# kondratevakate/mri-epilepsy-diagnosis

Measured on AMD Instinct MI355X. Metric: MRI volumes/sec (fwd+bwd) 3D U-Net @160x192x160, higher is better.
Workload: dtype f32; 1 GPU; unet.UNet(c0=8, 3 enc blocks, BN+PReLU, trilinear) fwd+softmax-Dice+bwd+AdamW, batch 2 x 1x160x192x160 fp32 per GPU (BASELINE configs[1]); global_batch=2, parallelism=dp1, launch=eager

## Files before the change

### include/mri3d.h

```cpp
#ifndef MRI3D_H
#define MRI3D_H

#include <stddef.h>
#include <stdint.h>

#ifdef __cplusplus
extern "C" {
#endif

typedef void* mri3d_stream_t;

enum { MRI3D_OK = 0, MRI3D_EINVAL = -1, MRI3D_ENOTSUP = -2, MRI3D_ELAUNCH = -3, MRI3D_EWORKSPACE = -4 };
enum { MRI3D_F32 = 0, MRI3D_BF16 = 1 };
enum { MRI3D_ACT_NONE = 0, MRI3D_ACT_RELU = 1, MRI3D_ACT_LEAKY = 2, MRI3D_ACT_PRELU = 3 };
enum { MRI3D_UP_NEAREST = 0, MRI3D_UP_TRILINEAR = 1 };
enum { MRI3D_PASS_FWD = 0, MRI3D_PASS_DGRAD = 1, MRI3D_PASS_WGRAD = 2 };

int mri3d_version(void);
const char* mri3d_last_error(void);

typedef struct Mri3dConvGeom {
    int32_t n;
    int32_t di, hi, wi, ci;
    int32_t dout, ho, wo, co;
    int32_t kd, kh, kw;
    int32_t sd, sh, sw;
    int32_t pd, ph, pw;
    int32_t dd, dh, dw;
    int32_t x_ld, y_ld;
    int32_t dtype;
} Mri3dConvGeom;

size_t mri3d_conv3d_workspace_bytes(const Mri3dConvGeom* g, int pass);

int mri3d_conv3d_fwd(const Mri3dConvGeom* g, const void* x, const void* w, const void* bias, void* y,
                     void* workspace, size_t ws_bytes, mri3d_stream_t stream);
int32_t mri3d_conv3d_fwd_stats_blocks(const Mri3dConvGeom* g);
int mri3d_conv3d_fwd_stats(const Mri3dConvGeom* g, const void* x, const void* w, const void* bias, void* y,
                           double* stat_partials, void* workspace, size_t ws_bytes, mri3d_stream_t stream);
int mri3d_conv3d_dgrad(const Mri3dConvGeom* g, const void* dy, const void* w, const void* bias, void* dx,
                       void* workspace, size_t ws_bytes, mri3d_stream_t stream);
int mri3d_conv3d_wgrad(const Mri3dConvGeom* g, const void* x, const void* dy, void* dw, void* dbias,
                       void* workspace, size_t ws_bytes, mri3d_stream_t stream);

int mri3d_conv3d_route(const Mri3dConvGeom* g, int32_t pass, int32_t stats, int32_t bias, int32_t split, int32_t second_ld,
                       int32_t align_x, int32_t align_y, char* name, size_t name_bytes);

int32_t mri3d_conv3d_cat_supported(const Mri3dConvGeom* g, int32_t split, int32_t second_ld, int32_t pass);
int32_t mri3d_conv3d_fwd_cat_stats_blocks(const Mri3dConvGeom* g, int32_t split, int32_t second_ld);
int mri3d_conv3d_fwd_cat(const Mri3dConvGeom* g, const void* x, const void* x2, int32_t split, int32_t x2_ld, const void* w,
                         const void* bias, void* y, double* stat_partials, void* workspace, size_t ws_bytes,
                         mri3d_stream_t stream);
int mri3d_conv3d_dgrad_cat(const Mri3dConvGeom* g, const void* dy, const void* w, void* dx, void* dx2, int32_t split,
                           int32_t dx2_ld, void* workspace, size_t ws_bytes, mri3d_stream_t stream);
int mri3d_conv3d_wgrad_cat(const Mri3dConvGeom* g, const void* x, const void* x2, int32_t split, int32_t x2_ld, const void* dy,
                           void* dw, void* dbias, void* workspace, size_t ws_bytes, mri3d_stream_t stream);

int32_t mri3d_conv3d_march_supported(const Mri3dConvGeom* g, int32_t pass);
int32_t mri3d_conv3d_march_stats_blocks(const Mri3dConvGeom* g);
int mri3d_conv3d_fwd_march(const Mri3dConvGeom* g, const void* x, const void* x2, int32_t split, int32_t x2_ld, const void* w,
                           const void* bias, void* y, double* stat_partials, void* workspace, size_t ws_bytes,
                           mri3d_stream_t stream);
int mri3d_conv3d_dgrad_march(const Mri3dConvGeom* g, const void* dy, const void* w, void* dx, void* dx2, int32_t split,
                             int32_t dx2_ld, void* workspace, size_t ws_bytes, mri3d_stream_t stream);

typedef struct Mri3dMarchPlanInfo {
    int32_t chunks, blocks, wgh, wgw, gch, gcw, nseg, seglen, nbuf, grid, whole_chunks, dispatcher;
    int64_t smem_bytes, wp_bytes;
} Mri3dMarchPlanInfo;
int32_t mri3d_conv3d_march_plan_query(const Mri3dConvGeom* g, int32_t pass, int32_t stats, Mri3dMarchPlanInfo* out);

int32_t mri3d_upconv3d_supported(const Mri3dConvGeom* g, int32_t scale);
size_t mri3d_upconv3d_workspace_bytes(const Mri3dConvGeom* g, int32_t scale);
int mri3d_upconv3d_fwd(const Mri3dConvGeom* g, int32_t scale, const void* x, const float* w, const float* bias, void* y,
                       mri3d_stream_t stream);
int mri3d_upconv3d_dgrad(const Mri3dConvGeom* g, int32_t scale, const void* dy, const float* w, void* dx, mri3d_stream_t stream);
int mri3d_upconv3d_wgrad(const Mri3dConvGeom* g, int32_t scale, const void* x, const void* dy, float* dw, float* dbias,
                         void* workspace, size_t ws_bytes, mri3d_stream_t stream);

int32_t mri3d_convpair_supported(const Mri3dConvGeom* first, const Mri3dConvGeom* second);
size_t mri3d_convpair_workspace_bytes(const Mri3dConvGeom* first, const Mri3dConvGeom* second);
int mri3d_convpair_wgrad_first(const Mri3dConvGeom* first, const Mri3dConvGeom* second, const void* x, const void* dy2, const float* w2,
                               float* dw1, float* dbias1, void* workspace, size_t ws_bytes, mri3d_stream_t stream);

typedef struct Mri3dFusedConvPlanInfo {
    int32_t hch, grid, gtrips, trips, per, passes, chunks;
    int64_t slabs, rows;
} Mri3dFusedConvPlanInfo;
int32_t mri3d_upconv3d_plan_query(const Mri3dConvGeom* g, int32_t scale, int32_t pass, Mri3dFusedConvPlanInfo* out);
int32_t mri3d_convpair_plan_query(const Mri3dConvGeom* first, const Mri3dConvGeom* second, Mri3dFusedConvPlanInfo* out);

typedef struct Mri3dNormGeom {
    int32_t n;
    int64_t vox;
    int32_t c;
    int32_t x_ld;
    int32_t y_ld;
    int32_t instance;
    int32_t act;
// ... 31 lines not shown
size_t mri3d_norm_act_pw_workspace_bytes(const Mri3dNormGeom* g, int32_t co);
int mri3d_norm_act_pw_fwd(const Mri3dNormGeom* g, int32_t co, const void* x, const float* mean, const float* invstd,
                          const float* gamma, const float* beta, const float* alpha, const float* w, const float* bias,
                          void* out, mri3d_stream_t stream);
int mri3d_norm_act_pw_bwd(const Mri3dNormGeom* g, int32_t co, int training, const void* x, const void* dout,
                          const float* mean, const float* invstd, const float* gamma, const float* beta, const float* alpha,
                          const float* w, void* dx, float* dgamma, float* dbeta, float* dalpha, float* dw, float* dbias,
                          void* workspace, size_t ws_bytes, mri3d_stream_t stream);

typedef struct Mri3dPoolGeom {
    int32_t n, di, hi, wi, dout, ho, wo, c;
    int32_t kd, kh, kw, sd, sh, sw, pd, ph, pw;
    int32_t x_ld, y_ld;
    int32_t dtype;
} Mri3dPoolGeom;
int mri3d_maxpool3d_fwd(const Mri3dPoolGeom* g, const void* x, void* y, uint8_t* idx, mri3d_stream_t stream);
int mri3d_maxpool3d_bwd(const Mri3dPoolGeom* g, const void* dy, const uint8_t* idx, void* dx, mri3d_stream_t stream);
int mri3d_maxpool3d_bwd_add(const Mri3dPoolGeom* g, const void* dy, const uint8_t* idx, const void* addend,
                            int32_t addend_ld, void* dx, mri3d_stream_t stream);
int mri3d_maxpool3d_route(const Mri3dPoolGeom* g, int32_t pass, int32_t addend_ld, int32_t align_tensors, int32_t align_idx,
                          char* name, size_t name_bytes);

int32_t mri3d_norm_act_pool_supported(const Mri3dNormGeom* g, const Mri3dPoolGeom* pg);
size_t mri3d_norm_act_pool_workspace_bytes(const Mri3dNormGeom* g, const Mri3dPoolGeom* pg);
int mri3d_norm_act_pool_fwd(const Mri3dNormGeom* g, const Mri3dPoolGeom* pg, const void* x, const float* mean,
                            const float* invstd, const float* gamma, const float* beta, const float* alpha, void* skip,
                            void* pooled, uint8_t* idx, mri3d_stream_t stream);
int mri3d_norm_act_pool_bwd(const Mri3dNormGeom* g, const Mri3dPoolGeom* pg, int training, const void* x, const void* dskip,
                            const void* dpool, const uint8_t* idx, const float* mean, const float* invstd, const float* gamma,
                            const float* beta, const float* alpha, void* dx, float* dgamma, float* dbeta, float* dalpha,
                            void* workspace, size_t ws_bytes, mri3d_stream_t stream);

typedef struct Mri3dUpGeom {
    int32_t n, di, hi, wi, dout, ho, wo, c;
    int32_t x_ld, y_ld;
    int32_t mode;
    int32_t align_corners;
    float rd, rh, rw;
    int32_t dtype;
} Mri3dUpGeom;
size_t mri3d_upsample3d_workspace_bytes(const Mri3dUpGeom* g);
int mri3d_upsample3d_fwd(const Mri3dUpGeom* g, const void* x, void* y, mri3d_stream_t stream);
int mri3d_upsample3d_bwd(const Mri3dUpGeom* g, const void* dy, void* dx, void* workspace, size_t ws_bytes,
                         mri3d_stream_t stream);
int mri3d_upsample3d_route(const Mri3dUpGeom* g, int32_t pass, int32_t align, char* name, size_t name_bytes);

typedef struct Mri3dResamplePlanInfo {
    int32_t vec, npv, hch, grid, segs, segl, tiles_h, tiles_w, passes, items, tables;
    int64_t lds_bytes;
} Mri3dResamplePlanInfo;
int32_t mri3d_maxpool3d_plan_query(const Mri3dPoolGeom* g, int32_t pass, int32_t addend_ld, int32_t align_tensors,
                                   int32_t align_idx, Mri3dResamplePlanInfo* out);
int32_t mri3d_upsample3d_plan_query(const Mri3dUpGeom* g, int32_t pass, int32_t align, Mri3dResamplePlanInfo* out);

typedef struct Mri3dDiceGeom {
    int32_t n;
    int64_t vox;
    int32_t c, ct;
    int32_t x_ld, t_ld;
    float eps;
    int32_t dtype;
} Mri3dDiceGeom;
size_t mri3d_softmax_dice_workspace_bytes(const Mri3dDiceGeom* g);
int mri3d_softmax_dice_fwd(const Mri3dDiceGeom* g, const void* logits, const void* target, float* loss,
                           float* stats, void* workspace, size_t ws_bytes, mri3d_stream_t stream);
int mri3d_softmax_dice_bwd(const Mri3dDiceGeom* g, const void* logits, const void* target, const float* stats,
                           const float* dloss, void* dlogits, mri3d_stream_t stream);

int mri3d_argmax_u8(const void* logits, uint8_t* out, int64_t nvox, int32_t c, int32_t ld, int32_t dtype,
                    mri3d_stream_t stream);

size_t mri3d_mask_overlap_workspace_bytes(void);
int mri3d_mask_overlap(const uint8_t* pred, const uint8_t* gt, int64_t nvox, int64_t* counts, void* workspace,
                       size_t ws_bytes, mri3d_stream_t stream);

enum { MRI3D_LABEL_U8 = 0, MRI3D_LABEL_I16 = 1, MRI3D_LABEL_I32 = 2, MRI3D_LABEL_F32 = 3 };

int mri3d_label_remap(const void* in, int32_t in_dtype, void* out, int32_t out_dtype, int64_t n, const uint8_t* lut,
                      int32_t lut_len, int32_t above, int32_t other, mri3d_stream_t stream);

typedef struct Mri3dDiceIndexGeom {
    int32_t n;
    int64_t vox;
    int32_t c;
    int32_t x_ld;
    float eps;
    int32_t dtype;
} Mri3dDiceIndexGeom;
size_t mri3d_softmax_dice_index_workspace_bytes(const Mri3dDiceIndexGeom* g);
int mri3d_softmax_dice_index_fwd(const Mri3dDiceIndexGeom* g, const void* logits, const uint8_t* labels, float* loss,
                                 float* stats, void* workspace, size_t ws_bytes, mri3d_stream_t stream);
int mri3d_softmax_dice_index_bwd(const Mri3dDiceIndexGeom* g, const void* logits, const uint8_t* labels,
                                 const float* stats, const float* dloss, void* dlogits, mri3d_stream_t stream);

size_t mri3d_confusion_workspace_bytes(int32_t c);
int mri3d_confusion_counts(const uint8_t* pred, const uint8_t* gt, int64_t nvox, int32_t c, int64_t* counts,
                           void* workspace, size_t ws_bytes, mri3d_stream_t stream);

size_t mri3d_order_stats_workspace_bytes(void);
int mri3d_order_stats_f32(const float* x, int64_t n, const int64_t* ranks, int32_t nranks, float* out, void* workspace,
                          size_t ws_bytes, mri3d_stream_t stream);
int mri3d_piecewise_linear_f32(const float* x, float* y, int64_t n, const double* edges, const double* slope,
                               const double* intercept, int32_t nseg, mri3d_stream_t stream);
size_t mri3d_znorm_workspace_bytes(void);
int mri3d_znorm_mean_mask_f32(const float* x, float* y, int64_t n, double* stats, void* workspace, size_t ws_bytes,
                              mri3d_stream_t stream);
// ... 85 lines not shown
```

### mri_epilepsy_diagnosis_amd/_lib.py

```python
import ctypes
import os
from ctypes import POINTER, Structure, c_char_p, c_double, c_float, c_int32, c_int64, c_size_t, c_uint8, c_void_p

_HERE = os.path.dirname(os.path.abspath(__file__))
LIB_PATH = os.path.join(_HERE, "libmri3d_hip.so")

F32, BF16 = 0, 1
ACT_NONE, ACT_RELU, ACT_LEAKY, ACT_PRELU = 0, 1, 2, 3
UP_NEAREST, UP_TRILINEAR = 0, 1
PASS_FWD, PASS_DGRAD, PASS_WGRAD = 0, 1, 2
NORM_PASS_STATS, NORM_PASS_FWD, NORM_PASS_BWD = 0, 1, 2
LABEL_U8, LABEL_I16, LABEL_I32, LABEL_F32 = 0, 1, 2, 3
BW_SCOTT, BW_SILVERMAN, BW_FACTOR = 0, 1, 2


class ConvGeom(Structure):
    _fields_ = [(n, c_int32) for n in (
        "n", "di", "hi", "wi", "ci", "dout", "ho", "wo", "co", "kd", "kh", "kw", "sd", "sh", "sw",
        "pd", "ph", "pw", "dd", "dh", "dw", "x_ld", "y_ld", "dtype")]


class NormGeom(Structure):
    _fields_ = [("n", c_int32), ("vox", c_int64), ("c", c_int32), ("x_ld", c_int32), ("y_ld", c_int32),
                ("instance", c_int32), ("act", c_int32), ("alpha_n", c_int32), ("slope", c_float),
                ("eps", c_float), ("group_c", c_int32), ("dtype", c_int32)]


class NormPlanInfo(Structure):
    _fields_ = [(n, c_int32) for n in ("vec", "CL", "VT", "cy", "nblk", "groups")] + [("gvox", c_int64)]


class ResamplePlanInfo(Structure):
    _fields_ = [(n, c_int32) for n in ("vec", "npv", "hch", "grid", "segs", "segl", "tiles_h", "tiles_w", "passes", "items",
                                       "tables")] + [("lds_bytes", c_int64)]


class FusedConvPlanInfo(Structure):
    _fields_ = [(n, c_int32) for n in ("hch", "grid", "gtrips", "trips", "per", "passes", "chunks")] + \
               [("slabs", c_int64), ("rows", c_int64)]


class MarchPlanInfo(Structure):
    _fields_ = [(n, c_int32) for n in ("chunks", "blocks", "wgh", "wgw", "gch", "gcw", "nseg", "seglen", "nbuf", "grid",
                                       "whole_chunks", "dispatcher")] + [("smem_bytes", c_int64), ("wp_bytes", c_int64)]


class PoolGeom(Structure):
    _fields_ = [(n, c_int32) for n in (
        "n", "di", "hi", "wi", "dout", "ho", "wo", "c", "kd", "kh", "kw", "sd", "sh", "sw", "pd", "ph", "pw",
        "x_ld", "y_ld", "dtype")]


class UpGeom(Structure):
    _fields_ = [(n, c_int32) for n in ("n", "di", "hi", "wi", "dout", "ho", "wo", "c", "x_ld", "y_ld", "mode",
                                       "align_corners")] + \
               [("rd", c_float), ("rh", c_float), ("rw", c_float), ("dtype", c_int32)]


class DiceGeom(Structure):
    _fields_ = [("n", c_int32), ("vox", c_int64), ("c", c_int32), ("ct", c_int32), ("x_ld", c_int32),
                ("t_ld", c_int32), ("eps", c_float), ("dtype", c_int32)]


class DiceIndexGeom(Structure):
    _fields_ = [("n", c_int32), ("vox", c_int64), ("c", c_int32), ("x_ld", c_int32), ("eps", c_float), ("dtype", c_int32)]


_P = c_void_p
_FP = c_void_p

SIGNATURES = {
    "mri3d_version": (c_int32, []),
    "mri3d_last_error": (c_char_p, []),
    "mri3d_conv3d_workspace_bytes": (c_size_t, [POINTER(ConvGeom), c_int32]),
    "mri3d_conv3d_fwd": (c_int32, [POINTER(ConvGeom), _P, _P, _P, _P, _P, c_size_t, _P]),
    "mri3d_conv3d_fwd_stats_blocks": (c_int32, [POINTER(ConvGeom)]),
    "mri3d_conv3d_fwd_stats": (c_int32, [POINTER(ConvGeom), _P, _P, _P, _P, _P, _P, c_size_t, _P]),
    "mri3d_conv3d_dgrad": (c_int32, [POINTER(ConvGeom), _P, _P, _P, _P, _P, c_size_t, _P]),
    "mri3d_conv3d_wgrad": (c_int32, [POINTER(ConvGeom), _P, _P, _P, _P, _P, c_size_t, _P]),
    "mri3d_conv3d_route": (c_int32, [POINTER(ConvGeom), c_int32, c_int32, c_int32, c_int32, c_int32, c_int32, c_int32, c_char_p, c_size_t]),
    "mri3d_conv3d_cat_supported": (c_int32, [POINTER(ConvGeom), c_int32, c_int32, c_int32]),
    "mri3d_conv3d_fwd_cat_stats_blocks": (c_int32, [POINTER(ConvGeom), c_int32, c_int32]),
    "mri3d_conv3d_fwd_cat": (c_int32, [POINTER(ConvGeom), _P, _P, c_int32, c_int32, _P, _P, _P, _P, _P, c_size_t, _P]),
    "mri3d_conv3d_dgrad_cat": (c_int32, [POINTER(ConvGeom), _P, _P, _P, _P, c_int32, c_int32, _P, c_size_t, _P]),
    "mri3d_conv3d_wgrad_cat": (c_int32, [POINTER(ConvGeom), _P, _P, c_int32, c_int32, _P, _P, _P, _P, c_size_t, _P]),
    "mri3d_conv3d_march_supported": (c_int32, [POINTER(ConvGeom), c_int32]),
    "mri3d_conv3d_march_stats_blocks": (c_int32, [POINTER(ConvGeom)]),
    "mri3d_conv3d_march_plan_query": (c_int32, [POINTER(ConvGeom), c_int32, c_int32, POINTER(MarchPlanInfo)]),
    "mri3d_conv3d_fwd_march": (c_int32, [POINTER(ConvGeom), _P, _P, c_int32, c_int32, _P, _P, _P, _P, _P, c_size_t, _P]),
    "mri3d_conv3d_dgrad_march": (c_int32, [POINTER(ConvGeom), _P, _P, _P, _P, c_int32, c_int32, _P, c_size_t, _P]),
    "mri3d_upconv3d_supported": (c_int32, [POINTER(ConvGeom), c_int32]),
    "mri3d_upconv3d_workspace_bytes": (c_size_t, [POINTER(ConvGeom), c_int32]),
    "mri3d_upconv3d_fwd": (c_int32, [POINTER(ConvGeom), c_int32, _P, _FP, _FP, _P, _P]),
    "mri3d_upconv3d_dgrad": (c_int32, [POINTER(ConvGeom), c_int32, _P, _FP, _P, _P]),
    "mri3d_upconv3d_wgrad": (c_int32, [POINTER(ConvGeom), c_int32, _P, _P, _FP, _FP, _P, c_size_t, _P]),
    "mri3d_convpair_supported": (c_int32, [POINTER(ConvGeom), POINTER(ConvGeom)]),
    "mri3d_convpair_workspace_bytes": (c_size_t, [POINTER(ConvGeom), POINTER(ConvGeom)]),
    "mri3d_convpair_wgrad_first": (c_int32, [POINTER(ConvGeom), POINTER(ConvGeom), _P, _P, _FP, _FP, _FP, _P, c_size_t, _P]),
    "mri3d_upconv3d_plan_query": (c_int32, [POINTER(ConvGeom), c_int32, c_int32, POINTER(FusedConvPlanInfo)]),
    "mri3d_convpair_plan_query": (c_int32, [POINTER(ConvGeom), POINTER(ConvGeom), POINTER(FusedConvPlanInfo)]),
    "mri3d_norm_workspace_bytes": (c_size_t, [POINTER(NormGeom)]),
    "mri3d_norm_plan_query": (c_int32, [POINTER(NormGeom), c_int32, c_int32, POINTER(NormPlanInfo)]),
    "mri3d_norm_stats": (c_int32, [POINTER(NormGeom), _P, _FP, _FP, _FP, _FP, c_float, _P, c_size_t, _P]),
    "mri3d_norm_stats_from_partials": (c_int32, [POINTER(NormGeom), _P, c_int32, _FP, _FP, _FP, _FP, _FP, c_float, _P]),
    "mri3d_norm_act_fwd": (c_int32, [POINTER(NormGeom), _P, _FP, _FP, _FP, _FP, _FP, _P, _P]),
    "mri3d_norm_act_bwd": (c_int32, [POINTER(NormGeom), c_int32, _P, _P, _FP, _FP, _FP, _FP, _FP, _P, _FP, _FP, _FP,
                                     _P, c_size_t, _P]),
    "mri3d_norm_act_pw_supported": (c_int32, [POINTER(NormGeom), c_int32]),
    "mri3d_norm_act_pw_workspace_bytes": (c_size_t, [POINTER(NormGeom), c_int32]),
    "mri3d_norm_act_pw_fwd": (c_int32, [POINTER(NormGeom), c_int32, _P, _FP, _FP, _FP, _FP, _FP, _FP, _FP, _P, _P]),
    "mri3d_norm_act_pw_bwd": (c_int32, [POINTER(NormGeom), c_int32, c_int32, _P, _P, _FP, _FP, _FP, _FP, _FP, _FP, _P, _FP, _FP,
                                        _FP, _FP, _FP, _P, c_size_t, _P]),
    "mri3d_maxpool3d_fwd": (c_int32, [POINTER(PoolGeom), _P, _P, _P, _P]),
    "mri3d_maxpool3d_bwd": (c_int32, [POINTER(PoolGeom), _P, _P, _P, _P]),
    "mri3d_maxpool3d_bwd_add": (c_int32, [POINTER(PoolGeom), _P, _P, _P, c_int32, _P, _P]),
    "mri3d_maxpool3d_route": (c_int32, [POINTER(PoolGeom), c_int32, c_int32, c_int32, c_int32, c_char_p, c_size_t]),
    "mri3d_maxpool3d_plan_query": (c_int32, [POINTER(PoolGeom), c_int32, c_int32, c_int32, c_int32, POINTER(ResamplePlanInfo)]),
    "mri3d_norm_act_pool_supported": (c_int32, [POINTER(NormGeom), POINTER(PoolGeom)]),
    "mri3d_norm_act_pool_workspace_bytes": (c_size_t, [POINTER(NormGeom), POINTER(PoolGeom)]),
    "mri3d_norm_act_pool_fwd": (c_int32, [POINTER(NormGeom), POINTER(PoolGeom), _P, _FP, _FP, _FP, _FP, _FP, _P, _P, _P, _P]),
    "mri3d_norm_act_pool_bwd": (c_int32, [POINTER(NormGeom), POINTER(PoolGeom), c_int32, _P, _P, _P, _P, _FP, _FP, _FP, _FP,
                                          _FP, _P, _FP, _FP, _FP, _P, c_size_t, _P]),
    "mri3d_upsample3d_workspace_bytes":(c_size_t, [POINTER(UpGeom)]),
    "mri3d_upsample3d_fwd": (c_int32, [POINTER(UpGeom), _P, _P, _P]),
    "mri3d_upsample3d_bwd": (c_int32, [POINTER(UpGeom), _P, _P, _P, c_size_t, _P]),
    "mri3d_upsample3d_route": (c_int32, [POINTER(UpGeom), c_int32, c_int32, c_char_p, c_size_t]),
    "mri3d_upsample3d_plan_query": (c_int32, [POINTER(UpGeom), c_int32, c_int32, POINTER(ResamplePlanInfo)]),
    "mri3d_softmax_dice_workspace_bytes": (c_size_t, [POINTER(DiceGeom)]),
    "mri3d_softmax_dice_fwd": (c_int32, [POINTER(DiceGeom), _P, _P, _FP, _FP, _P, c_size_t, _P]),
    "mri3d_softmax_dice_bwd": (c_int32, [POINTER(DiceGeom), _P, _P, _FP, _FP, _P, _P]),
    "mri3d_argmax_u8": (c_int32, [_P, _P, c_int64, c_int32, c_int32, c_int32, _P]),
    "mri3d_mask_overlap_workspace_bytes": (c_size_t, []),
    "mri3d_mask_overlap": (c_int32, [_P, _P, c_int64, _P, _P, c_size_t, _P]),
    "mri3d_label_remap": (c_int32, [_P, c_int32, _P, c_int32, c_int64, _P, c_int32, c_int32, c_int32, _P]),
    "mri3d_softmax_dice_index_workspace_bytes": (c_size_t, [POINTER(DiceIndexGeom)]),
    "mri3d_softmax_dice_index_fwd": (c_int32, [POINTER(DiceIndexGeom), _P, _P, _FP, _FP, _P, c_size_t, _P]),
    "mri3d_softmax_dice_index_bwd": (c_int32, [POINTER(DiceIndexGeom), _P, _P, _FP, _FP, _P, _P]),
    "mri3d_confusion_workspace_bytes": (c_size_t, [c_int32]),
    "mri3d_confusion_counts": (c_int32, [_P, _P, c_int64, c_int32, _P, _P, c_size_t, _P]),
    "mri3d_order_stats_workspace_bytes": (c_size_t, []),
    "mri3d_order_stats_f32": (c_int32, [_P, c_int64, _P, c_int32, _P, _P, c_size_t, _P]),
    "mri3d_piecewise_linear_f32": (c_int32, [_P, _P, c_int64, _P, _P, _P, c_int32, _P]),
    "mri3d_znorm_workspace_bytes": (c_size_t, []),
    "mri3d_znorm_mean_mask_f32": (c_int32, [_P, _P, c_int64, _P, _P, c_size_t, _P]),
    "mri3d_crop_or_pad_f32": (c_int32, [_P, _P, c_int32, c_int32, c_int32, c_int32, c_int32, c_int32, c_int32, c_float, _P]),
    "mri3d_intensity_workspace_bytes": (c_size_t, [c_int64, c_int32, c_int32]),
    "mri3d_kde_plan": (c_int32, [c_int64, c_int32, c_int32, _P]),
    "mri3d_intensity_moments_f32": (c_int32, [_P, _P, c_int64, c_int32, _P, _P, c_size_t, _P]),
    "mri3d_kde_f32": (c_int32, [_P, _P, c_int64, c_int32, _P, _P, c_int32, c_int32, c_double, _P, _P, _P, c_size_t, _P]),
    "mri3d_surface_distance_workspace_bytes": (c_size_t, [c_int32, c_int32, c_int32]),
    "mri3d_surface_distance": (c_int32, [_P, _P, c_int32, c_int32, c_int32, _P, _P, _P, c_size_t, _P]),
    "mri3d_surface_elements": (c_int32, [_P, _P, c_int32, c_int32, c_int32, _P, _P, _P, _P, c_int64, _P, _P, c_size_t, _P]),
    "mri3d_extract_patches": (c_int32, [_P, c_int32, c_int32, c_int32, c_int32, c_int32, _P, c_int32, c_int32, c_int32,
                                        c_int32, _P, _P]),
    "mri3d_aggregate_patches_u8": (c_int32, [_P, _P, c_int32, c_int32, c_int32, c_int32, c_int32, c_int32, c_int32, _P,
                                             c_int32, c_int32, c_int32, c_int32, _P]),
    "mri3d_aggregate_patches_argmax": (c_int32, [_P, c_int32, c_int32, c_int32, _P, c_int32, c_int32, c_int32, c_int32,
                                                 c_int32, c_int32, c_int32, _P, c_int32, c_int32, c_int32, c_int32, _P]),
    "mri3d_strip_starts_f32": (c_int32, [_FP, c_int32, c_int32, c_int32, c_int32, _P, _P]),
    "mri3d_mirror_patches_f32": (c_int32, [_FP, c_int32, c_int32, c_int32, _P, _P, c_int64, c_int32, c_int32, c_int32, _FP, _P]),
    "mri3d_mirror_patch_labels_u8": (c_int32, [_P, c_int32, c_int32, c_int32, _P, c_int64, c_int32, c_int32, _P, _P]),
    "mri3d_patch_vote_u8": (c_int32, [_P, c_int32, c_int32, _P, _P]),
    "mri3d_paint_patches_u8": (c_int32, [_P, _P, c_int32, c_int32, c_int32, c_int32, c_int32, _P, _P]),
    "mri3d_warp3d": (c_int32, [_FP, _FP, _P, _P, c_int32, c_int32, c_int32, c_int32, c_int32, _FP, _FP, c_int32, c_int32,
                               c_int32, c_float, _FP, _P]),
    "mri3d_bias_field_f32": (c_int32, [_FP, _FP, c_int32, c_int32, c_int32, c_int32, _P, c_int32, _P]),
    "mri3d_kspace_mix_f32": (c_int32, [_FP, _FP, c_int32, c_int32, c_int32, c_int32, c_int32, _FP, _P]),
    "mri3d_copy_channels": (c_int32, [_P, _P, c_int64, c_int32, c_int32, c_int32, c_int32, _P]),
    "mri3d_add_channels": (c_int32, [_P, _P, _P, c_int64, c_int32, c_int32, c_int32, c_int32, c_int32, _P]),
    "mri3d_convert_channels": (c_int32, [_P, c_int32, _P, c_int32, c_int64, c_int32, c_int32, c_int32, _P]),
    "mri3d_bayes_weights_fwd": (c_int32, [_FP, _FP, c_int64, c_int32, c_float, _FP, _FP, _FP, _P]),
    "mri3d_bayes_weights_bwd": (c_int32, [_FP, _FP, c_int64, c_int32, c_float, _FP, _FP, _FP, _FP, _FP, _P]),
    "mri3d_bayes_square": (c_int32, [_P, _P, c_int64, c_int32, c_int32, c_int32, c_int32, _P]),
    "mri3d_bayes_sample_fwd": (c_int32, [_P, _P, _FP, _P, c_int64, c_int32, c_int32, c_int32, c_int32, c_int32, c_int32, _P]),
    "mri3d_bayes_sample_bwd": (c_int32, [_P, _P, _FP, _P, c_int64, c_int32, c_int32, c_int32, c_int32, c_int32, c_int32, _P]),
    "mri3d_bayes_dx": (c_int32, [_P, _P, _P, _P, c_int64, c_int32, c_int32, c_int32, c_int32, c_int32, c_int32, _P]),
    "mri3d_mc_state_bytes": (c_size_t, [c_int64, c_int32]),
    "mri3d_mc_accumulate": (c_int32, [_P, c_int64, c_int32, c_int32, c_int32, c_int32, c_int64, c_int32, _P, c_size_t, _P]),
    "mri3d_mc_finalize": (c_int32, [_P, c_size_t, c_int64, c_int32, c_int32, _FP, _FP, _FP, _FP, _P, _P]),
    "mri3d_adam_step": (c_int32, [_FP, _FP, _FP, _FP, c_int64, c_float, c_float, c_float, c_float, c_float, c_int32,
# ... 32 lines not shown
```

### mri_epilepsy_diagnosis_amd/build.py

```python
import hashlib
import os
import subprocess
import sys
from concurrent.futures import ThreadPoolExecutor

HERE = os.path.dirname(os.path.abspath(__file__))
CSRC = os.path.join(HERE, "csrc")
OBJ = os.path.join(HERE, "csrc", "build")
LIB = os.path.join(HERE, "libmri3d_hip.so")
SOURCES = ["api.hip", "conv_generic.hip", "conv_mfma.hip", "conv_mfma_wgrad.hip", "conv_march.hip", "conv_pointwise.hip", "upconv.hip", "sepconv.hip", "norm.hip", "resample.hip", "loss.hip", "labels.hip", "elementwise.hip", "bayes.hip", "mc_stats.hip", "preprocess.hip", "intensity.hip", "surface.hip", "patches.hip", "detection.hip", "augment.hip", "kspace.hip"]
HIPCC = os.environ.get("HIPCC", "/opt/rocm/bin/hipcc")
FLAGS = ["--offload-arch=gfx950", "-O3", "-fPIC", "-std=c++17", "-Wall", "-Wno-unused-function"]
EXTRA_FLAGS = {"conv_march.hip": ["-mllvm", "-amdgpu-spill-vgpr-to-agpr=0"], "mc_stats.hip": ["-ffp-contract=off"],
               "intensity.hip": ["-ffp-contract=off"]}


def _digest(path):
    h = hashlib.sha256()
    for dep in [path, os.path.join(CSRC, "common.h"), os.path.join(CSRC, "conv_backends.h"), os.path.join(CSRC, "mfma_util.h"), os.path.join(HERE, "..", "include", "mri3d.h")]:
        with open(dep, "rb") as f:
            h.update(f.read())
    h.update(" ".join(FLAGS + EXTRA_FLAGS.get(os.path.basename(path), [])).encode())
    return h.hexdigest()

# ... 9 lines not shown
    r = subprocess.run(cmd, capture_output=True, text=True, timeout=900)
    if r.returncode != 0:
        raise RuntimeError("hipcc failed for %s:\n%s\n%s" % (src, r.stdout, r.stderr))
    if r.stderr.strip():
        sys.stderr.write(r.stderr)
    with open(stamp, "w") as f:
        f.write(dig)
    return obj, True


def build(force=False, jobs=4, verbose=True):
    os.makedirs(OBJ, exist_ok=True)
    if force:
        for f in os.listdir(OBJ):
            os.remove(os.path.join(OBJ, f))
    with ThreadPoolExecutor(max_workers=jobs) as ex:
        results = list(ex.map(_compile, SOURCES))
    objs = [o for o, _ in results]
    changed = any(c for _, c in results)
    if changed or not os.path.exists(LIB):
        cmd = [HIPCC, "--offload-arch=gfx950", "-shared", "-fPIC", "-o", LIB] + objs
        r = subprocess.run(cmd, capture_output=True, text=True)
        if r.returncode != 0:
            raise RuntimeError("link failed:\n%s\n%s" % (r.stdout, r.stderr))
        if verbose:
            print("built", LIB)
    elif verbose:
        print("up to date", LIB)
    return LIB


def build_variant(name, extra_flags, verbose=True):
    obj_dir = os.path.join(CSRC, "build_" + name)
    os.makedirs(obj_dir, exist_ok=True)
    lib = os.path.join(HERE, "libmri3d_hip_%s.so" % name)

    def one(src):
        obj = os.path.join(obj_dir, src.replace(".hip", ".o"))
        r = subprocess.run([HIPCC] + FLAGS + EXTRA_FLAGS.get(src, []) + ["-DMRI3D_TUNING"] + list(extra_flags) + ["-c", os.path.join(CSRC, src), "-o", obj],
                           capture_output=True, text=True, timeout=900)
        if r.returncode != 0:
            raise RuntimeError("hipcc failed for %s:\n%s" % (src, r.stderr[-3000:]))
        return obj
    with ThreadPoolExecutor(max_workers=4) as ex:
        objs = list(ex.map(one, SOURCES))
    r = subprocess.run([HIPCC, "--offload-arch=gfx950", "-shared", "-fPIC", "-o", lib] + objs, capture_output=True, text=True)
    if r.returncode != 0:
        raise RuntimeError("link failed:\n%s" % r.stderr[-3000:])
    if verbose:
        print("built", lib)
    return lib


def build_host_sanitizer(verbose=True):
    root = os.path.join(HERE, "..")
    driver = os.path.join(root, "tests", "native", "host_sanitizer_driver.cpp")
    out_dir = os.path.join(root, "tests", "native", "build")
    os.makedirs(out_dir, exist_ok=True)
    exe = os.path.join(out_dir, "host_sanitizer_driver")
    flags = ["--offload-arch=gfx950", "-fsanitize=address,undefined", "-fno-gpu-sanitize", "-fno-sanitize-recover=undefined", "-fno-omit-frame-pointer",
             "-O1", "-g", "-std=c++17", "-w", "-I", os.path.join(root, "include")]
    h = hashlib.sha256(" ".join(flags).encode())
    inputs = [os.path.join(CSRC, s) for s in SOURCES] + [os.path.join(CSRC, "common.h"), os.path.join(CSRC, "conv_backends.h"), os.path.join(CSRC, "mfma_util.h"), os.path.join(root, "include", "mri3d.h"), driver]
    for f in inputs:
        with open(f, "rb") as fh:
            h.update(fh.read())
    stamp = exe + ".sha"
    if os.path.exists(exe) and os.path.exists(stamp) and open(stamp).read() == h.hexdigest():
        return exe

    def one(src):
        obj = os.path.join(out_dir, os.path.basename(src).rsplit(".", 1)[0] + ".host.o")
        cmd = [HIPCC] + flags + (["-x", "hip"] if src.endswith(".hip") else []) + ["-c", src, "-o", obj]
        r = subprocess.run(cmd, capture_output=True, text=True, timeout=900)
        if r.returncode != 0:
            raise RuntimeError("host sanitizer build failed for %s:\n%s" % (src, r.stderr[-3000:]))
        return obj
    with ThreadPoolExecutor(max_workers=4) as ex:
        objs = list(ex.map(one, [os.path.join(CSRC, s) for s in SOURCES] + [driver]))
    r = subprocess.run([HIPCC, "--offload-arch=gfx950", "-fsanitize=address,undefined", "-fno-gpu-sanitize", "-o", exe] + objs, capture_output=True, text=True, timeout=600)
    if r.returncode != 0:
        raise RuntimeError("host sanitizer link failed:\n%s" % r.stderr[-3000:])
    with open(stamp, "w") as f:
        f.write(h.hexdigest())
    if verbose:
        print("built", exe)
    return exe


if __name__ == "__main__":
    if "--variant" in sys.argv:
        i = sys.argv.index("--variant")
        build_variant(sys.argv[i + 1], sys.argv[i + 2:])
    elif "--host-sanitizer" in sys.argv:
        print(build_host_sanitizer())
    else:
        build(force="--force" in sys.argv)
```

### mri_epilepsy_diagnosis_amd/csrc/api.hip

```cpp
#include "common.h"
#include "conv_backends.h"
#include <string.h>

namespace mri3d {

static thread_local char g_err[512] = "";

void set_error(const char* fmt, ...) {
    va_list ap;
    va_start(ap, fmt);
    vsnprintf(g_err, sizeof(g_err), fmt, ap);
    va_end(ap);
}

static int conv_check(const Mri3dConvGeom* g, const char* who, int first_ci = -1) {
    MRI3D_REQUIRE(g != nullptr, MRI3D_EINVAL, "%s: null geometry", who);
    MRI3D_REQUIRE(g->dtype == MRI3D_F32 || g->dtype == MRI3D_BF16, MRI3D_ENOTSUP, "%s: unknown dtype %d", who, g->dtype);
    MRI3D_REQUIRE(g->n > 0 && g->di > 0 && g->hi > 0 && g->wi > 0 && g->ci > 0 && g->dout > 0 && g->ho > 0 && g->wo > 0 &&
                      g->co > 0,
                  MRI3D_EINVAL, "%s: empty tensor", who);
    MRI3D_REQUIRE(g->kd > 0 && g->kh > 0 && g->kw > 0 && g->sd > 0 && g->sh > 0 && g->sw > 0 && g->dd > 0 && g->dh > 0 &&
                      g->dw > 0 && g->pd >= 0 && g->ph >= 0 && g->pw >= 0,
                  MRI3D_EINVAL, "%s: bad kernel/stride/padding/dilation", who);
    MRI3D_REQUIRE(g->x_ld >= (first_ci >= 0 ? first_ci : g->ci) && g->y_ld >= g->co, MRI3D_EINVAL, "%s: pitch smaller than channel count", who);
// ... 137 lines not shown
    return conv_march_needs(*g, pass == MRI3D_PASS_DGRAD, false, true).grid > 0 ? 1 : 0;
}

extern "C" int32_t mri3d_conv3d_march_stats_blocks(const Mri3dConvGeom* g) {
    if (!g || conv_check(g, "conv3d_march_stats_blocks") != MRI3D_OK) return 0;
    return conv_march_needs(*g, false, true, true).grid;
}

extern "C" int32_t mri3d_conv3d_march_plan_query(const Mri3dConvGeom* g, int32_t pass, int32_t stats, Mri3dMarchPlanInfo* out) {
    MRI3D_REQUIRE(g && out, MRI3D_EINVAL, "conv3d_march_plan_query: null pointer");
    int rc = conv_check(g, "conv3d_march_plan_query");
    if (rc) return rc;
    MRI3D_REQUIRE(pass == MRI3D_PASS_FWD || pass == MRI3D_PASS_DGRAD, MRI3D_EINVAL, "conv3d_march_plan_query: pass %d", pass);
    MRI3D_REQUIRE(!stats || pass == MRI3D_PASS_FWD, MRI3D_EINVAL, "conv3d_march_plan_query: statistics outside the forward");
    Mri3dMarchPlanInfo info;
    MRI3D_REQUIRE(conv_march_plan_info(*g, pass == MRI3D_PASS_DGRAD, stats != 0, info), MRI3D_ENOTSUP,
                  "conv3d_march_plan_query: geometry not served (see mri3d_conv3d_march_supported; statistics: at most 8 output blocks)");
    *out = info;
    return MRI3D_OK;
}

extern "C" int mri3d_conv3d_fwd_march(const Mri3dConvGeom* g, const void* x, const void* x2, int32_t split, int32_t x2_ld,
                                      const void* w, const void* bias, void* y, double* stat_partials, void* workspace,
                                      size_t ws_bytes, mri3d_stream_t stream) {
    int rc = conv_check(g, "conv3d_fwd_march", x2 ? split : -1);
    if (rc) return rc;
    MRI3D_REQUIRE(x && w && y, MRI3D_EINVAL, "conv3d_fwd_march: null pointer");
    MRI3D_REQUIRE(x2 == nullptr || (split > 0 && split < g->ci && x2_ld >= g->ci - split), MRI3D_EINVAL, "conv3d_fwd_march: bad split");
    return conv_march_run(*g, false, true, x, (const float*)w, (const float*)bias, y, workspace, ws_bytes,
                          static_cast<hipStream_t>(stream), stat_partials, ConvSplit{x2, split, x2_ld});
}

extern "C" int mri3d_conv3d_dgrad_march(const Mri3dConvGeom* g, const void* dy, const void* w, void* dx, void* dx2, int32_t split,
                                        int32_t dx2_ld, void* workspace, size_t ws_bytes, mri3d_stream_t stream) {
    int rc = conv_check(g, "conv3d_dgrad_march", dx2 ? split : -1);
    if (rc) return rc;
    MRI3D_REQUIRE(dy && w && dx, MRI3D_EINVAL, "conv3d_dgrad_march: null pointer");
    MRI3D_REQUIRE(dx2 == nullptr || (split > 0 && split < g->ci && dx2_ld >= g->ci - split), MRI3D_EINVAL, "conv3d_dgrad_march: bad split");
    return conv_march_run(*g, true, true, dy, (const float*)w, nullptr, dx, workspace, ws_bytes, static_cast<hipStream_t>(stream),
                          nullptr, ConvSplit{dx2, split, dx2_ld});
}

extern "C" int mri3d_conv3d_wgrad(const Mri3dConvGeom* g, const void* x, const void* dy, void* dw, void* dbias,
                                  void* workspace, size_t ws_bytes, mri3d_stream_t stream) {
    int rc = conv_check(g, "conv3d_wgrad");
    if (rc) return rc;
    MRI3D_REQUIRE(x && dy && dw, MRI3D_EINVAL, "conv3d_wgrad: null pointer");
    hipStream_t s = static_cast<hipStream_t>(stream);
    switch (conv_backend(*g, MRI3D_PASS_WGRAD, false, 0, 0, ptr_align(x, dy, workspace), ptr_align(x))) {
    case ConvBackend::pointwise: return conv_pointwise_wgrad(*g, x, dy, (float*)dw, (float*)dbias, workspace, ws_bytes, s);
    case ConvBackend::mfma: return conv_mfma_wgrad(*g, x, dy, (float*)dw, (float*)dbias, workspace, ws_bytes, s);
    default: return conv_generic_wgrad(*g, x, dy, (float*)dw, (float*)dbias, workspace, ws_bytes, s);
    }
}

extern "C" int mri3d_conv3d_route(const Mri3dConvGeom* g, int32_t pass, int32_t stats, int32_t bias, int32_t split, int32_t second_ld,
                                  int32_t align_x, int32_t align_y, char* name, size_t name_bytes) {
    int rc = conv_check(g, "conv3d_route", split > 0 ? split : -1);
    if (rc) return rc;
    MRI3D_REQUIRE(name != nullptr && name_bytes >= 32, MRI3D_EINVAL, "conv3d_route: name buffer of at least 32 bytes required");
    MRI3D_REQUIRE(pass == MRI3D_PASS_FWD || pass == MRI3D_PASS_DGRAD || pass == MRI3D_PASS_WGRAD, MRI3D_EINVAL, "conv3d_route: unknown pass %d", pass);
    MRI3D_REQUIRE(split >= 0 && (!stats || pass == MRI3D_PASS_FWD), MRI3D_EINVAL, "conv3d_route: negative split, or statistics outside the forward");
    const ConvSplit sp{nullptr, split, second_ld};
    const bool with_bias = bias != 0 && pass != MRI3D_PASS_WGRAD && !(split > 0 && pass == MRI3D_PASS_DGRAD);
    switch (conv_backend(*g, pass, stats != 0, split, second_ld, align_x < align_y ? align_x : align_y, align_x)) {
    case ConvBackend::none: snprintf(name, name_bytes, "none"); break;
    case ConvBackend::generic:
        MRI3D_REQUIRE(conv_generic_route_name(*g, pass, with_bias, align_x, align_y, name, name_bytes), MRI3D_EINVAL,
                      "conv3d_route: name buffer too small");
        break;
    case ConvBackend::pointwise:
        MRI3D_REQUIRE(conv_pointwise_route_name(*g, pass, with_bias, align_x, align_y, name, name_bytes), MRI3D_EINVAL,
                      "conv3d_route: name buffer too small");
        break;
    case ConvBackend::mfma:
        MRI3D_REQUIRE(conv_mfma_route_name(*g, pass, stats != 0, with_bias, sp, name, name_bytes), MRI3D_ENOTSUP,
                      "conv3d_route: the MFMA file names no kernel for a pass it supports");
        break;
    }
    return MRI3D_OK;
}
```

### mri_epilepsy_diagnosis_amd/csrc/conv_backends.h

```cpp
#pragma once
#include "common.h"

namespace mri3d {

struct ConvSplit {
    const void* second = nullptr;
    int split = 0, second_ld = 0;
};

size_t conv_generic_workspace_bytes(const Mri3dConvGeom& g, int pass);
int conv_generic_fwd(const Mri3dConvGeom& g, const void* x, const float* w, const float* bias, void* y, void* ws,
                     size_t ws_bytes, hipStream_t s);
int conv_generic_dgrad(const Mri3dConvGeom& g, const void* dy, const float* w, const float* bias, void* dx, void* ws,
                       size_t ws_bytes, hipStream_t s);
int conv_generic_wgrad(const Mri3dConvGeom& g, const void* x, const void* dy, float* dw, float* dbias, void* ws,
                       size_t ws_bytes, hipStream_t s);
bool conv_generic_route_name(const Mri3dConvGeom& g, int pass, bool bias, int ax, int ay, char* name, size_t name_bytes);

bool conv_mfma_supported(const Mri3dConvGeom& g, int pass);
size_t conv_mfma_workspace_bytes(const Mri3dConvGeom& g, int pass);
int conv_mfma_fwd(const Mri3dConvGeom& g, const void* x, const float* w, const float* bias, void* y, void* ws,
                  size_t ws_bytes, hipStream_t s);
int conv_mfma_dgrad(const Mri3dConvGeom& g, const void* dy, const float* w, const float* bias, void* dx, void* ws,
                    size_t ws_bytes, hipStream_t s);
int conv_mfma_fwd_stat_blocks(const Mri3dConvGeom& g, int split = 0, int second_ld = 0);
bool conv_mfma_cat_supported(const Mri3dConvGeom& g, int split, int second_ld, int pass);
int conv_mfma_fwd_cat(const Mri3dConvGeom& g, const void* x, const void* x2, int split, int x2_ld, const float* w, const float* bias,
                      void* y, double* stat_part, void* ws, size_t ws_bytes, hipStream_t s);
int conv_mfma_dgrad_cat(const Mri3dConvGeom& g, const void* dy, const float* w, void* dx, void* dx2, int split, int dx2_ld, void* ws,
                        size_t ws_bytes, hipStream_t s);
int conv_mfma_fwd_stats(const Mri3dConvGeom& g, const void* x, const float* w, const float* bias, void* y, double* stat_part,
                        void* ws, size_t ws_bytes, hipStream_t s);
bool conv_mfma_route_name(const Mri3dConvGeom& g, int pass, bool stats, bool bias, const ConvSplit& sp, char* name, size_t name_bytes);

bool conv_mfma_wgrad_supported(const Mri3dConvGeom& g, int split = 0, int second_ld = 0);
size_t conv_mfma_wgrad_workspace_bytes(const Mri3dConvGeom& g);
bool conv_mfma_wgrad_route_name(const Mri3dConvGeom& g, char* name, size_t name_bytes);
int conv_mfma_wgrad(const Mri3dConvGeom& g, const void* x, const void* dy, float* dw, float* dbias, void* ws,
                    size_t ws_bytes, hipStream_t s);
int conv_mfma_wgrad_cat(const Mri3dConvGeom& g, const void* x, const void* x2, int split, int x2_ld, const void* dy, float* dw,
                        float* dbias, void* ws, size_t ws_bytes, hipStream_t s);

struct MarchNeeds { int grid; size_t wp_bytes; };
MarchNeeds conv_march_needs(const Mri3dConvGeom& g, bool dgrad, bool stats, bool force);
bool conv_march_plan_info(const Mri3dConvGeom& g, bool dgrad, bool stats, Mri3dMarchPlanInfo& out);
int conv_march_run(const Mri3dConvGeom& g, bool dgrad, bool force, const void* in_v, const float* w, const float* bias, void* out_v,
                   void* ws, size_t ws_bytes, hipStream_t s, double* stat_part, const ConvSplit& sp);

bool conv_pointwise_supported(const Mri3dConvGeom& g, int pass);
size_t conv_pointwise_workspace_bytes(const Mri3dConvGeom& g, int pass);
int conv_pointwise_fwd(const Mri3dConvGeom& g, const void* x, const float* w, const float* bias, void* y, hipStream_t s);
int conv_pointwise_dgrad(const Mri3dConvGeom& g, const void* dy, const float* w, const float* bias, void* dx,
                         hipStream_t s);
int conv_pointwise_wgrad(const Mri3dConvGeom& g, const void* x, const void* dy, float* dw, float* dbias, void* ws,
                         size_t ws_bytes, hipStream_t s);
bool conv_pointwise_route_name(const Mri3dConvGeom& g, int pass, bool bias, int ax, int ay, char* name, size_t name_bytes);

}
```

### mri_epilepsy_diagnosis_amd/csrc/conv_generic.hip

```cpp
#include "common.h"
#include "conv_backends.h"

namespace mri3d {

__device__ __forceinline__ float wave_sum_dpp(float v) {
    v += __builtin_bit_cast(float, __builtin_amdgcn_update_dpp(0, __builtin_bit_cast(int, v), 0xB1, 0xF, 0xF, true));
    v += __builtin_bit_cast(float, __builtin_amdgcn_update_dpp(0, __builtin_bit_cast(int, v), 0x4E, 0xF, 0xF, true));
    v += __builtin_bit_cast(float, __builtin_amdgcn_update_dpp(0, __builtin_bit_cast(int, v), 0x141, 0xF, 0xF, true));
    v += __builtin_bit_cast(float, __builtin_amdgcn_update_dpp(0, __builtin_bit_cast(int, v), 0x140, 0xF, 0xF, true));
    const int vi = __builtin_bit_cast(int, v);
    const float r0 = __builtin_bit_cast(float, __builtin_amdgcn_readlane(vi, 0));
    const float r1 = __builtin_bit_cast(float, __builtin_amdgcn_readlane(vi, 16));
    const float r2 = __builtin_bit_cast(float, __builtin_amdgcn_readlane(vi, 32));
    const float r3 = __builtin_bit_cast(float, __builtin_amdgcn_readlane(vi, 48));
    return (r0 + r1) + (r2 + r3);
}

__global__ void repack_w_kernel(const float* __restrict__ w, float* __restrict__ wp, int Co, int Ci, int taps, int P, int dgrad) {
    const int M = dgrad ? Co : Ci, N = dgrad ? Ci : Co;
    int total = taps * M * P;
    for (int i = blockIdx.x * blockDim.x + threadIdx.x; i < total; i += gridDim.x * blockDim.x) {
        int p = i % P;
        int m = (i / P) % M;
        int tap = i / (P * M);
// ... 847 lines not shown
#pragma unroll
        for (int c = 0; c < CI; ++c) {
            const float vsum = wave_sum_dpp(acc[t][c]);
            if (lane == 0) red[wave][t * CI + c] = vsum;
        }
    {
        const float vsum = wave_sum_dpp(bsum);
        if (lane == 0) red[wave][kSmTaps * CI] = vsum;
    }
    __syncthreads();
    if (tid < taps * CI)
        part[(size_t)blockIdx.x * taps * CI + tid] = (red[0][tid] + red[1][tid]) + (red[2][tid] + red[3][tid]);
    else if (tid == kSmTaps * CI && bias_part)
        bias_part[blockIdx.x] = (red[0][tid] + red[1][tid]) + (red[2][tid] + red[3][tid]);
}

constexpr int kCo1Blocks = 1024;

static bool wgrad_co1_ok(const Mri3dConvGeom& g) {
    static const int off = tuning_knob("MRI3D_CO1_OFF", 0);
    return !off && g.co == 1 && g.kd * g.kh * g.kw <= kSmTaps && (g.ci == 1 || ((g.ci == 4 || g.ci == 8 || g.ci == 16) && g.x_ld % 4 == 0)) &&
           (int64_t)g.dout * g.ho * g.wo < 0x7fffffffLL;
}

constexpr int C1D = 4, C1H = 8, C1WQ = 8;

template <int CO> struct Cin1 { static constexpr int VPT = CO <= 8 ? 4 : 2; };
typedef float f32x2 __attribute__((ext_vector_type(2)));

__device__ __forceinline__ void decode_tile(int t, int tilesD, int tilesH, int tilesW, int TW, int& n, int& d0, int& h0, int& w0) {
    w0 = (t % tilesW) * TW;
    t /= tilesW;
    h0 = (t % tilesH) * C1H;
    t /= tilesH;
    d0 = (t % tilesD) * C1D;
    n = t / tilesD;
}

template <typename T, int TW, int ND, int NTHR = 256>
__device__ __forceinline__ void cin1_stage(float* xs, const T* __restrict__ xn, const Mri3dConvGeom& g, int dlo, int h0,
                                           int w0, int tid) {
    constexpr int PW = TW + 4, NE = ND * (C1H + 2) * (TW + 2);
    for (int e = tid; e < NE; e += NTHR) {
        const int fw = e % (TW + 2), r = e / (TW + 2);
        const int fh = r % (C1H + 2), fd = r / (C1H + 2);
        const int id = dlo + fd, ih = h0 - 1 + fh, iw = w0 - 1 + fw;
        const bool ok = (unsigned)id < (unsigned)g.di && (unsigned)ih < (unsigned)g.hi && (unsigned)iw < (unsigned)g.wi;
        const int cd = min(max(id, 0), g.di - 1), ch = min(max(ih, 0), g.hi - 1), cw = min(max(iw, 0), g.wi - 1);
        const float v = ldf(xn + (((int64_t)cd * g.hi + ch) * g.wi + cw) * g.x_ld);
        xs[(fd * (C1H + 2) + fh) * PW + fw] = ok ? v : 0.f;
    }
}

template <typename T, int CO>
__global__ void __launch_bounds__(256)
conv_cin1_fwd_kernel(Mri3dConvGeom g, const T* __restrict__ x, const float* __restrict__ wp, const float* __restrict__ bias,
                     T* __restrict__ y, int tilesD, int tilesH, int tilesW, int ntiles) {
    constexpr int VPT = Cin1<CO>::VPT, TW = C1WQ * VPT, PW = TW + 4;
    __shared__ __attribute__((aligned(16))) float xs[(C1D + 2) * (C1H + 2) * PW];
    __shared__ __attribute__((aligned(16))) float wsh[27 * CO];
    const int tid = threadIdx.x;
    for (int e = tid; e < 27 * CO; e += 256) wsh[e] = wp[e];
    const int wq = tid % C1WQ, hl = (tid / C1WQ) % C1H, dl = tid / (C1WQ * C1H);
    float bv[CO];
#pragma unroll
    for (int c = 0; c < CO; ++c) bv[c] = bias ? bias[c] : 0.f;
    for (int tile = blockIdx.x; tile < ntiles; tile += gridDim.x) {
        int n, d0, h0, w0;
        decode_tile(tile, tilesD, tilesH, tilesW, TW, n, d0, h0, w0);
        __syncthreads();
        cin1_stage<T, TW, C1D + 2>(xs, x + (int64_t)n * g.di * g.hi * g.wi * g.x_ld, g, d0 - 1, h0, w0, tid);
        __syncthreads();
        f32x2 acc[VPT][CO / 2];
#pragma unroll
        for (int v = 0; v < VPT; ++v)
#pragma unroll
            for (int c = 0; c < CO / 2; ++c) acc[v][c] = f32x2{bv[2 * c], bv[2 * c + 1]};
#pragma unroll
        for (int kd = 0; kd < 3; ++kd)
#pragma unroll
            for (int kh = 0; kh < 3; ++kh) {
                const float* row = xs + ((dl + kd) * (C1H + 2) + hl + kh) * PW + wq * VPT;
                float r[VPT + 2];
#pragma unroll
                for (int i = 0; i < VPT + 2; ++i) r[i] = row[i];
                int woff = (kd * 3 + kh) * 3 * CO;
                asm volatile("" : "+v"(woff));
                __builtin_amdgcn_sched_barrier(0);
                const float* wrow = wsh + woff;
#pragma unroll
                for (int kw = 0; kw < 3; ++kw) {
                    const float* wt = wrow + kw * CO;
#pragma unroll
                    for (int c = 0; c < CO / 2; ++c) {
                        const f32x2 wv = f32x2{wt[2 * c], wt[2 * c + 1]};
#pragma unroll
                        for (int v = 0; v < VPT; ++v)
                            acc[v][c] = __builtin_elementwise_fma(f32x2{r[v + kw], r[v + kw]}, wv, acc[v][c]);
                    }
                }
            }
#pragma unroll
        for (int v = 0; v < VPT; ++v)
#pragma unroll
            for (int c = 0; c < CO / 2; ++c) asm volatile("" : "+v"(acc[v][c]));
        const int od = d0 + dl, oh = h0 + hl;
        if (od < g.dout && oh < g.ho) {
            T* yo = y + ((((int64_t)n * g.dout + od) * g.ho + oh) * g.wo + w0 + wq * VPT) * g.y_ld;
#pragma unroll
            for (int v = 0; v < VPT; ++v)
                if (w0 + wq * VPT + v < g.wo) {
#pragma unroll
                    for (int c = 0; c < CO; c += 4)
                        stf4(yo + (int64_t)v * g.y_ld + c,
                             make_float4(acc[v][c / 2].x, acc[v][c / 2].y, acc[v][c / 2 + 1].x, acc[v][c / 2 + 1].y));
                }
        }
    }
}

template <typename T, int CO>
__global__ void __launch_bounds__(768)
conv_cin1_wgrad_kernel(Mri3dConvGeom g, const T* __restrict__ x, const T* __restrict__ dy, float* __restrict__ part,
                       float* __restrict__ bias_part, int tilesD, int tilesH, int tilesW, int ntiles, int nshares) {
    constexpr int VPT = Cin1<CO>::VPT, TW = C1WQ * VPT, PW = TW + 4, NA = 9 * CO + CO;
    __shared__ __attribute__((aligned(16))) float xs[(C1D + 2) * (C1H + 2) * PW];
    __shared__ float red[12][NA];
    const int kd = __builtin_amdgcn_readfirstlane((int)threadIdx.x >> 8);
    const int tid = threadIdx.x & 255;
    const int per_xcd = gridDim.x / 8;
    const int share = (blockIdx.x % 8) * per_xcd + blockIdx.x / 8;
    const int wq = tid % C1WQ, hl = (tid / C1WQ) % C1H, dl = tid / (C1WQ * C1H);
    f32x2 acc[3][3][CO / 2];
    float bsum[CO];
#pragma unroll
    for (int a = 0; a < 3; ++a)
#pragma unroll
        for (int b = 0; b < 3; ++b)
#pragma unroll
            for (int c = 0; c < CO / 2; ++c) acc[a][b][c] = f32x2{0.f, 0.f};
#pragma unroll
    for (int c = 0; c < CO; ++c) bsum[c] = 0.f;
    for (int tile = share; tile < ntiles; tile += nshares) {
        int n, d0, h0, w0;
        decode_tile(tile, tilesD, tilesH, tilesW, TW, n, d0, h0, w0);
        __syncthreads();
        cin1_stage<T, TW, C1D + 2, 768>(xs, x + (int64_t)n * g.di * g.hi * g.wi * g.x_ld, g, d0 - 1, h0, w0, (int)threadIdx.x);
        const int od = d0 + dl, oh = h0 + hl;
        f32x2 gy[VPT][CO / 2];
#pragma unroll
        for (int v = 0; v < VPT; ++v) {
            const int ow = w0 + wq * VPT + v;
            const bool ok = od < g.dout && oh < g.ho && ow < g.wo;
            const T* dp = dy + ((((int64_t)n * g.dout + min(od, g.dout - 1)) * g.ho + min(oh, g.ho - 1)) * g.wo +
                                min(ow, g.wo - 1)) * g.y_ld;
#pragma unroll
            for (int c = 0; c < CO; c += 4) {
                const float4 q = ldf4(dp + c);
                gy[v][c / 2] = f32x2{ok ? q.x : 0.f, ok ? q.y : 0.f};
                gy[v][c / 2 + 1] = f32x2{ok ? q.z : 0.f, ok ? q.w : 0.f};
            }
        }
        __syncthreads();
#pragma unroll
        for (int kh = 0; kh < 3; ++kh) {
            const float* row = xs + ((dl + kd) * (C1H + 2) + hl + kh) * PW + wq * VPT;
            float r[VPT + 2];
#pragma unroll
            for (int i = 0; i < VPT + 2; ++i) r[i] = row[i];
#pragma unroll
            for (int kw = 0; kw < 3; ++kw)
#pragma unroll
                for (int v = 0; v < VPT; ++v)
#pragma unroll
                    for (int c = 0; c < CO / 2; ++c)
                        acc[kh][kw][c] = __builtin_elementwise_fma(f32x2{r[v + kw], r[v + kw]}, gy[v][c], acc[kh][kw][c]);
        }
        if (kd == 1) {
#pragma unroll
            for (int v = 0; v < VPT; ++v)
#pragma unroll
                for (int c = 0; c < CO / 2; ++c) { bsum[2 * c] += gy[v][c].x; bsum[2 * c + 1] += gy[v][c].y; }
        }
    }
    const int lane = tid & 63, wave = (int)threadIdx.x >> 6;
#pragma unroll
    for (int a = 0; a < 3; ++a)
#pragma unroll
        for (int b = 0; b < 3; ++b)
#pragma unroll
            for (int c = 0; c < CO; ++c) {
                const float vsum = wave_sum_dpp((c & 1) ? acc[a][b][c / 2].y : acc[a][b][c / 2].x);
                if (lane == 0) red[wave][(a * 3 + b) * CO + c] = vsum;
            }
#pragma unroll
    for (int c = 0; c < CO; ++c) {
        const float vsum = wave_sum_dpp(bsum[c]);
        if (lane == 0) red[wave][9 * CO + c] = vsum;
    }
    __syncthreads();
    const int w0_ = 4 * kd;
    if (tid < 9 * CO) {
        const float t4 = (red[w0_][tid] + red[w0_ + 1][tid]) + (red[w0_ + 2][tid] + red[w0_ + 3][tid]);
        part[((size_t)share * 27 + kd * 9 + tid / CO) * CO + tid % CO] = t4;
    } else if (tid < NA && kd == 1 && bias_part) {
        const int c = tid - 9 * CO;
        bias_part[(size_t)share * CO + c] = (red[w0_][tid] + red[w0_ + 1][tid]) + (red[w0_ + 2][tid] + red[w0_ + 3][tid]);
    }
}

template <typename T>
__global__ void __launch_bounds__(256)
conv_c1c1_stencil_kernel(Mri3dConvGeom g, const T* __restrict__ x, int x_ld, const float* __restrict__ w, const float* __restrict__ bias,
                         int flip, T* __restrict__ y, int y_ld, int tilesD, int tilesH, int tilesW, int ntiles) {
    constexpr int VPT = 4, TW = C1WQ * VPT, PW = TW + 4;
    __shared__ __attribute__((aligned(16))) float xs[(C1D + 2) * (C1H + 2) * PW];
    const int tid = threadIdx.x;
    const int wq = tid % C1WQ, hl = (tid / C1WQ) % C1H, dl = tid / (C1WQ * C1H);
    float wt[27];
#pragma unroll
    for (int t = 0; t < 27; ++t) wt[t] = w[flip ? 26 - t : t];
    const float b0 = bias ? bias[0] : 0.f;
    Mri3dConvGeom gs = g;
    gs.x_ld = x_ld;
    for (int tile = blockIdx.x; tile < ntiles; tile += gridDim.x) {
        int n, d0, h0, w0;
        decode_tile(tile, tilesD, tilesH, tilesW, TW, n, d0, h0, w0);
        __syncthreads();
        cin1_stage<T, TW, C1D + 2>(xs, x + (int64_t)n * g.di * g.hi * g.wi * x_ld, gs, d0 - 1, h0, w0, tid);
        __syncthreads();
        float acc[VPT];
#pragma unroll
        for (int v = 0; v < VPT; ++v) acc[v] = b0;
#pragma unroll
        for (int kd = 0; kd < 3; ++kd)
#pragma unroll
            for (int kh = 0; kh < 3; ++kh) {
                const float* row = xs + ((dl + kd) * (C1H + 2) + hl + kh) * PW + wq * VPT;
                float r[VPT + 2];
#pragma unroll
                for (int i = 0; i < VPT + 2; ++i) r[i] = row[i];
#pragma unroll
                for (int kw = 0; kw < 3; ++kw)
#pragma unroll
                    for (int v = 0; v < VPT; ++v) acc[v] = fmaf(r[v + kw], wt[(kd * 3 + kh) * 3 + kw], acc[v]);
            }
#pragma unroll
        for (int v = 0; v < VPT; ++v) asm volatile("" : "+v"(acc[v]));
        const int od = d0 + dl, oh = h0 + hl;
        if (od < g.di && oh < g.hi) {
            T* yo = y + ((((int64_t)n * g.di + od) * g.hi + oh) * g.wi + w0 + wq * VPT) * y_ld;
#pragma unroll
            for (int v = 0; v < VPT; ++v)
                if (w0 + wq * VPT + v < g.wi) stf(yo + (int64_t)v * y_ld, acc[v]);
        }
    }
}

template <typename T>
__global__ void __launch_bounds__(256)
// ... 600 lines not shown
        MRI3D_DISPATCH_DTYPE(g.dtype, T, {
            switch (p.ci_inst) {
                case 1: MRI3D_CO1(1); break;
                case 4: MRI3D_CO1(4); break;
                case 8: MRI3D_CO1(8); break;
                default: MRI3D_CO1(16); break;
            }
        });
#undef MRI3D_CO1
        break;
    }
    case GenKernel::quads: {
        what = "conv3d_wgrad(quads)";
#define MRI3D_WGQ(NTv, CIVv)                                                                                           \
    hipLaunchKernelGGL((conv_wgrad_quads_kernel<T, NTv, CIVv>), dim3(nb), dim3(256), 0, s, g, (const T*)x, (const T*)dy,  \
                       part, bias_part, p.quads.QI, p.quads.QO, p.quads.hch, p.CiP, p.CoP)
        MRI3D_DISPATCH_DTYPE(g.dtype, T, {
            if (p.civ == 1) MRI3D_WGQ(8, 1);
            else if (p.nt == 4) MRI3D_WGQ(4, 4);
            else if (p.nt == 6) MRI3D_WGQ(6, 4);
            else MRI3D_WGQ(8, 4);
        });
#undef MRI3D_WGQ
        break;
    }
    case GenKernel::small: {
        what = "conv3d_wgrad(small)";
        MRI3D_DISPATCH_DTYPE(g.dtype, T, {
            hipLaunchKernelGGL(conv_wgrad_small_kernel<T>, dim3(nb, p.small.gy, p.small.gz), dim3(256), 0, s, g, (const T*)x,
                               (const T*)dy, part, bias_part, p.small.CiL, p.CiP, p.CoP);
        });
        break;
    }
    case GenKernel::lds: {
        const auto& q = p.lds;
        MRI3D_REQUIRE(q.smem <= 160 * 1024, MRI3D_ENOTSUP, "conv3d_wgrad: Ci=%d Co=%d needs %zu B of LDS", g.ci, g.co, q.smem);
        MRI3D_DISPATCH_DTYPE(g.dtype, T, {
            static const hipError_t attr_ = hipFuncSetAttribute(reinterpret_cast<const void*>(conv_wgrad_generic_kernel<T>),
                                                                hipFuncAttributeMaxDynamicSharedMemorySize, 160 * 1024);
            (void)attr_;
            hipLaunchKernelGGL(conv_wgrad_generic_kernel<T>, dim3(nb, taps, q.gz), dim3(256), q.smem, s, g, (const T*)x,
                               (const T*)dy, part, bias_part, q.Ci4, q.Co4, q.nitems, q.vsplit);
        });
        break;
    }
    case GenKernel::taps: case GenKernel::gather: case GenKernel::strided_taps: case GenKernel::strided:
        MRI3D_REQUIRE(false, MRI3D_EINVAL, "conv3d_wgrad: no weight-gradient kernel in the plan");
    }
    hipLaunchKernelGGL(wgrad_reduce_kernel, dim3(cdiv(g.co * g.ci * taps + g.co, 8)), dim3(256), 0, s, part, bias_part, dw, dbias, nb,
                       taps, g.ci, g.co, p.CiP, p.CoP);
    return check_launch(what);
}

}
```

### mri_epilepsy_diagnosis_amd/csrc/resample.hip

```cpp
#include "common.h"
#include <limits.h>
#include <algorithm>
#include <stdlib.h>
#include <type_traits>

namespace mri3d {

template <int VEC>
struct V {
    float v[VEC];
    template <typename T>
    __device__ __forceinline__ void load(const T* p) {
        if constexpr (VEC == 8) {
            const bf16x8_t t = *reinterpret_cast<const bf16x8_t*>(p);
#pragma unroll
            for (int j = 0; j < 8; ++j) v[j] = (float)t[j];
        } else if constexpr (VEC == 4) {
            float4 t = ldf4(p);
            v[0] = t.x; v[1] = t.y; v[2] = t.z; v[3] = t.w;
        } else {
            v[0] = ldf(p);
        }
    }
    template <typename T>
// ... 562 lines not shown
        for (int f = f0; f <= f1; ++f) {
            if (f < f1) fetch(f + 1);
            const float4* base = pbuf[f & 1] + ((2 * ihl) * MFW + 2 * iwl) * MCQ + q;
            float4 sf = make_float4(0.f, 0.f, 0.f, 0.f);
#pragma unroll
            for (int bb = 0; bb < 4; ++bb) {
                float4 r = make_float4(0.f, 0.f, 0.f, 0.f);
#pragma unroll
                for (int cc = 0; cc < 4; ++cc) {
                    const float4 gv = base[(bb * MFW + cc) * MCQ];
                    r.x = fmaf(ww[cc], gv.x, r.x);
                    r.y = fmaf(ww[cc], gv.y, r.y);
                    r.z = fmaf(ww[cc], gv.z, r.z);
                    r.w = fmaf(ww[cc], gv.w, r.w);
                }
                sf.x = fmaf(wh[bb], r.x, sf.x);
                sf.y = fmaf(wh[bb], r.y, sf.y);
                sf.z = fmaf(wh[bb], r.z, sf.z);
                sf.w = fmaf(wh[bb], r.w, sf.w);
            }
            const int i = f >> 1;
            float wdi[4];
            up2_axis_weights(i, g.di, wdi);
            if (f & 1) {
                if (i >= d0) { accA.x = fmaf(wdi[2], sf.x, accA.x); accA.y = fmaf(wdi[2], sf.y, accA.y);
                               accA.z = fmaf(wdi[2], sf.z, accA.z); accA.w = fmaf(wdi[2], sf.w, accA.w); }
                float wn[4];
                up2_axis_weights(i + 1, g.di, wn);
                if (i >= d0) { accB.x = wn[0] * sf.x; accB.y = wn[0] * sf.y; accB.z = wn[0] * sf.z; accB.w = wn[0] * sf.w; }
                else { accA.x = wn[0] * sf.x; accA.y = wn[0] * sf.y; accA.z = wn[0] * sf.z; accA.w = wn[0] * sf.w; }
            } else {
                if (i > d0) {
                    float wp[4];
                    up2_axis_weights(i - 1, g.di, wp);
                    accA.x = fmaf(wp[3], sf.x, accA.x); accA.y = fmaf(wp[3], sf.y, accA.y);
                    accA.z = fmaf(wp[3], sf.z, accA.z); accA.w = fmaf(wp[3], sf.w, accA.w);
                    if (vok) stf4(dxo + (int64_t)(i - 1) * xplane, accA);
                    accA = accB;
                }
                if (i < d1) { accA.x = fmaf(wdi[1], sf.x, accA.x); accA.y = fmaf(wdi[1], sf.y, accA.y);
                              accA.z = fmaf(wdi[1], sf.z, accA.z); accA.w = fmaf(wdi[1], sf.w, accA.w); }
            }
            if (f < f1) stash((f + 1) & 1);
            __syncthreads();
        }
        if (d1 == g.di && vok) stf4(dxo + (int64_t)(d1 - 1) * xplane, accA);
    }
}

constexpr int UTH = 4, UTW = 16;
constexpr int UHH = UTH + 2, UHW = UTW + 2, UHV = UHH * UHW;
constexpr int UMD = 16;

template <typename T, int VEC, int NPV>
__global__ void __launch_bounds__(256)
upsample2x_fwd_march_kernel(Mri3dUpGeom g, const T* __restrict__ x, T* __restrict__ y, int segsD, int segl, int tilesH,
                            int tilesW, int cpasses, int nitems) {
    constexpr int PCH = VEC * NPV;
    constexpr int NST = (UHV * NPV + 255) / 256;
    __shared__ __attribute__((aligned(16))) float cbuf[2][UHV * NPV * VEC];
    const int tid = threadIdx.x;
    const int per_xcd = (nitems + 7) / 8;
    for (int b = blockIdx.x; b < per_xcd * 8; b += gridDim.x) {
        const int item = (b % 8) * per_xcd + b / 8;
        if (item >= nitems) continue;
        int t = item;
        const int c0 = (t % cpasses) * PCH;
        t /= cpasses;
        const int w0 = (t % tilesW) * UTW;
        t /= tilesW;
        const int h0 = (t % tilesH) * UTH;
        t /= tilesH;
        const int d0 = (t % segsD) * segl;
        const int n = t / segsD;
        const int d1 = min(d0 + segl, g.di);
        const T* xn = x + (int64_t)n * g.di * g.hi * g.wi * g.x_ld + c0;
        const int xplane = g.hi * g.wi * g.x_ld;
        int soff[NST];
#pragma unroll
        for (int j = 0; j < NST; ++j) {
            const int idx = min(j * 256 + tid, UHV * NPV - 1);
            const int pc = idx % NPV, hv = idx / NPV;
            const int fw = hv % UHW, fh = hv / UHW;
            const int ch = min(max(h0 - 1 + fh, 0), g.hi - 1), cw = min(max(w0 - 1 + fw, 0), g.wi - 1);
            soff[j] = (ch * g.wi + cw) * g.x_ld + (c0 + pc * VEC < g.c ? pc * VEC : 0);
        }
        V<VEC> sv[NST];
        auto fetch = [&](int c) {
            const T* pl = xn + (int64_t)min(max(c, 0), g.di - 1) * xplane;
#pragma unroll
            for (int j = 0; j < NST; ++j) sv[j].load(pl + soff[j]);
        };
        auto stash = [&](int buf) {
#pragma unroll
            for (int j = 0; j < NST; ++j) {
                const int idx = j * 256 + tid;
                if (j < NST - 1 || idx < UHV * NPV) {
#pragma unroll
                    for (int e = 0; e < VEC; e += 4)
                        *reinterpret_cast<float4*>(&cbuf[buf][idx * VEC + e]) = make_float4(sv[j].v[e], sv[j].v[e + 1], sv[j].v[e + 2], sv[j].v[e + 3]);
                }
            }
        };
        int ia[NPV], ib[NPV], ic[NPV], id[NPV], yoff[NPV];
        unsigned okm = 0;
#pragma unroll
        for (int k = 0; k < NPV; ++k) {
            const int it = k * 256 + tid;
            const int pc = it % NPV, pos = it / NPV;
            const int fwl = pos % (2 * UTW), fhl = pos / (2 * UTW);
            const int hw0 = (fwl >> 1) + 1, hw1 = hw0 + ((fwl & 1) ? 1 : -1), hh0 = (fhl >> 1) + 1, hh1 = hh0 + ((fhl & 1) ? 1 : -1);
            ia[k] = ((hh0 * UHW + hw0) * NPV + pc) * VEC;
            ib[k] = ((hh0 * UHW + hw1) * NPV + pc) * VEC;
            ic[k] = ((hh1 * UHW + hw0) * NPV + pc) * VEC;
            id[k] = ((hh1 * UHW + hw1) * NPV + pc) * VEC;
            const int oh = 2 * h0 + fhl, ow = 2 * w0 + fwl;
            const bool ok = oh < g.ho && ow < g.wo && c0 + pc * VEC < g.c;
            okm |= ok ? (1u << k) : 0u;
            yoff[k] = ok ? (oh * g.wo + ow) * g.y_ld + c0 + pc * VEC : 0;
        }
        T* yn = y + (int64_t)n * g.dout * g.ho * g.wo * g.y_ld;
        const int64_t yplane = (int64_t)g.ho * g.wo * g.y_ld;

        __syncthreads();
        fetch(d0 - 1);
        stash(0);
        __syncthreads();
        V<VEC> pp[NPV];
        for (int c = d0 - 1; c <= d1; ++c) {
            const int buf = (c - (d0 - 1)) & 1;
            if (c < d1) fetch(c + 1);
#pragma unroll
            for (int k = 0; k < NPV; ++k) {
                V<VEC> pc_;
#pragma unroll
                for (int e = 0; e < VEC; e += 4) {
                    const float4 a = *reinterpret_cast<const float4*>(&cbuf[buf][ia[k] + e]);
                    const float4 bq = *reinterpret_cast<const float4*>(&cbuf[buf][ib[k] + e]);
                    const float4 cq = *reinterpret_cast<const float4*>(&cbuf[buf][ic[k] + e]);
                    const float4 dq = *reinterpret_cast<const float4*>(&cbuf[buf][id[k] + e]);
                    pc_.v[e + 0] = 0.75f * fmaf(0.75f, a.x, 0.25f * bq.x) + 0.25f * fmaf(0.75f, cq.x, 0.25f * dq.x);
                    pc_.v[e + 1] = 0.75f * fmaf(0.75f, a.y, 0.25f * bq.y) + 0.25f * fmaf(0.75f, cq.y, 0.25f * dq.y);
                    pc_.v[e + 2] = 0.75f * fmaf(0.75f, a.z, 0.25f * bq.z) + 0.25f * fmaf(0.75f, cq.z, 0.25f * dq.z);
                    pc_.v[e + 3] = 0.75f * fmaf(0.75f, a.w, 0.25f * bq.w) + 0.25f * fmaf(0.75f, cq.w, 0.25f * dq.w);
                }
                if (c >= d0 && ((okm >> k) & 1u)) {
                    V<VEC> o;
                    if (c > d0) {
#pragma unroll
                        for (int e = 0; e < VEC; ++e) o.v[e] = fmaf(0.75f, pp[k].v[e], 0.25f * pc_.v[e]);
                        o.store(yn + (int64_t)(2 * c - 1) * yplane + yoff[k]);
                    }
                    if (c < d1) {
#pragma unroll
                        for (int e = 0; e < VEC; ++e) o.v[e] = fmaf(0.75f, pc_.v[e], 0.25f * pp[k].v[e]);
                        o.store(yn + (int64_t)(2 * c) * yplane + yoff[k]);
                    }
                }
                pp[k] = pc_;
            }
            if (c < d1) stash(buf ^ 1);
            __syncthreads();
        }
    }
}

enum class ResampleKernel { maxpool_fwd, maxpool2_fwd, maxpool_bwd, up_fwd, up2x_fwd_march, up_bwd, up_nearest_int_bwd, up2x_bwd_tile, up2x_bwd_march };

struct ResamplePlan {
    ResampleKernel kern;
    int vec = 1;
    int npv = 0;
    int hch = 0;
    int grid = 0;
    int segs = 0, segl = 0, tilesH = 0, tilesW = 0, passes = 0;
    int items = 0;
    size_t smem = 0;
    bool tables = false;
    char name[40];
};

static const char* type_name(int dtype) { return dtype == MRI3D_BF16 ? "bf16" : "f32"; }

static ResamplePlan pool_fwd_plan(const Mri3dPoolGeom& g, int align, int align_idx) {
    const PoolFwdLanes l = pool_fwd_lanes(g, {g.x_ld, g.y_ld}, {align}, align_idx);
    ResamplePlan p;
    p.kern = l.lines ? ResampleKernel::maxpool2_fwd : ResampleKernel::maxpool_fwd;
    p.vec = l.vec, p.hch = l.hch, p.grid = l.grid;
    snprintf(p.name, sizeof(p.name), "%s<%s,%d>", l.lines ? "maxpool2_fwd" : "maxpool_fwd", type_name(g.dtype), p.vec);
    return p;
}

static ResamplePlan pool_bwd_plan(const Mri3dPoolGeom& g, int align, int align_idx, bool addend, int a_ld, int align_addend) {
    ResamplePlan p;
    p.kern = ResampleKernel::maxpool_bwd;
    p.vec = pool_vec(g.dtype, g.c, {g.x_ld, g.y_ld, addend ? a_ld : 0}, {align, addend ? align_addend : 16}, align_idx);
    slab_plan(g.n * g.di, g.hi, g.wi, g.c / p.vec, p.hch, p.grid);
    snprintf(p.name, sizeof(p.name), "maxpool_bwd<%s,%d>%s", type_name(g.dtype), p.vec, addend ? "+add" : "");
    return p;
}

static bool up_generic_only() {
    static const int generic = tuning_knob("MRI3D_UP_GENERIC", 0);
    return generic != 0;
}

static int up_vec(const Mri3dUpGeom& g, int align) {
    return g.c % 4 == 0 && g.x_ld % 4 == 0 && g.y_ld % 4 == 0 && align_vec4(g.dtype, align) ? 4 : 1;
}

static bool up2x_fast_ok(const Mri3dUpGeom& g, int align) {
    return g.mode == MRI3D_UP_TRILINEAR && !g.align_corners && g.dout == 2 * g.di && g.ho == 2 * g.hi && g.wo == 2 * g.wi &&
           g.rd == 0.5f && g.rh == 0.5f && g.rw == 0.5f && up_vec(g, align) == 4;
}

static ResamplePlan up_fwd_plan(const Mri3dUpGeom& g, int align) {
    ResamplePlan p;
// ... 11 lines not shown
            p.kern = ResampleKernel::up2x_fwd_march;
            p.vec = vec, p.npv = npv, p.segs = segsD, p.segl = segl, p.tilesH = mtilesH, p.tilesW = mtilesW, p.passes = mpasses;
            p.items = (int)items;
            p.grid = (int)std::min<int64_t>((items + 7) / 8 * 8, 256 * 4 * 8);
            snprintf(p.name, sizeof(p.name), "upsample2x_fwd_march<%s,%d,%d>", type_name(g.dtype), vec, npv);
            return p;
        }
    }
    p.kern = ResampleKernel::up_fwd;
    p.vec = up_vec(g, align);
    slab_plan(g.n * g.dout, g.ho, g.wo, g.c / p.vec, p.hch, p.grid);
    snprintf(p.name, sizeof(p.name), "upsample_fwd<%s,%d>", type_name(g.dtype), p.vec);
    return p;
}

static ResamplePlan up_bwd_plan(const Mri3dUpGeom& g, int align) {
    ResamplePlan p;
    if (!up_generic_only() && up2x_fast_ok(g, align)) {
        if (g.c % 16 == 0) {
            const int segsD = cdiv(g.di, MD), tilesH = cdiv(g.hi, MTH), tilesW = cdiv(g.wi, MTW), cpasses = g.c / 16;
            const int64_t items = (int64_t)g.n * segsD * cpasses * tilesH * tilesW;
            if (items <= 0x7ffffff0 && (int64_t)g.ho * g.wo * g.y_ld <= 0x7fffffff) {
                p.kern = ResampleKernel::up2x_bwd_march;
                p.vec = 4, p.segs = segsD, p.tilesH = tilesH, p.tilesW = tilesW, p.passes = cpasses, p.items = (int)items;
                p.grid = (int)std::min<int64_t>((items + 7) / 8 * 8, 256 * 3 * 8);
                snprintf(p.name, sizeof(p.name), "upsample2x_bwd_march<%s>", type_name(g.dtype));
                return p;
            }
        }
        const int tilesD = cdiv(g.di, TTD), tilesH = cdiv(g.hi, TTH), tilesW = cdiv(g.wi, TTW);
        const int64_t nt = (int64_t)g.n * tilesD * tilesH * tilesW;
        if (nt <= 0x7fffffff) {
            p.kern = ResampleKernel::up2x_bwd_tile;
            p.vec = 4, p.segs = tilesD, p.tilesH = tilesH, p.tilesW = tilesW, p.items = (int)nt, p.smem = kUp2TileLds;
            p.grid = (int)std::min<int64_t>(nt, 2048);
            snprintf(p.name, sizeof(p.name), "upsample2x_bwd<%s>", type_name(g.dtype));
            return p;
        }
    }
    p.vec = up_vec(g, align);
    slab_plan(g.n * g.di, g.hi, g.wi, g.c / p.vec, p.hch, p.grid);
    const int sc = g.di > 0 ? g.dout / g.di : 0;
    if (!up_generic_only() && g.mode == MRI3D_UP_NEAREST && p.vec == 4 && (sc == 2 || sc == 4) && g.dout == sc * g.di &&
        g.ho == sc * g.hi && g.wo == sc * g.wi) {
        p.kern = ResampleKernel::up_nearest_int_bwd;
        p.npv = sc;
        snprintf(p.name, sizeof(p.name), "upsample_nearest_int_bwd<%s,%d>", type_name(g.dtype), sc);
        return p;
    }
    p.kern = ResampleKernel::up_bwd;
    p.tables = true;
    snprintf(p.name, sizeof(p.name), "tables+upsample_bwd<%s,%d>", type_name(g.dtype), p.vec);
    return p;
}

template <auto kern, typename... Args>
static void launch(const ResamplePlan& p, hipStream_t s, Args... args) {
    if (p.smem != 0) {
        static const hipError_t attr = hipFuncSetAttribute(reinterpret_cast<const void*>(kern), hipFuncAttributeMaxDynamicSharedMemorySize, (int)p.smem);
        (void)attr;
    }
    hipLaunchKernelGGL(kern, dim3(p.grid), dim3(256), p.smem, s, args...);
}

template <int... Vs, typename F>
static void with_int(int v, F f) {
    (void)((v == Vs && (f(std::integral_constant<int, Vs>{}), true)) || ...);
}

template <typename T, int VEC> constexpr bool has_vec = VEC < 8 || sizeof(T) == 2;

}

using namespace mri3d;

static int pool_check(const Mri3dPoolGeom* g, const char* who) {
    MRI3D_REQUIRE(g != nullptr, MRI3D_EINVAL, "%s: null geometry", who);
    MRI3D_REQUIRE(g->dtype == MRI3D_F32 || g->dtype == MRI3D_BF16, MRI3D_ENOTSUP, "%s: unknown dtype %d", who, g->dtype);
    MRI3D_REQUIRE(g->n > 0 && g->c > 0 && g->di > 0 && g->hi > 0 && g->wi > 0 && g->dout > 0 && g->ho > 0 && g->wo > 0,
                  MRI3D_EINVAL, "%s: empty tensor", who);
    MRI3D_REQUIRE(g->kd * g->kh * g->kw <= 256 && g->kd > 0 && g->kh > 0 && g->kw > 0, MRI3D_ENOTSUP,
                  "%s: window volume must be <= 256", who);
    MRI3D_REQUIRE(g->sd > 0 && g->sh > 0 && g->sw > 0 && g->x_ld >= g->c && g->y_ld >= g->c, MRI3D_EINVAL,
                  "%s: bad stride/pitch", who);
    MRI3D_REQUIRE((g->dout - 1) * g->sd - g->pd < g->di && (g->ho - 1) * g->sh - g->ph < g->hi &&
                      (g->wo - 1) * g->sw - g->pw < g->wi && 2 * g->pd <= g->kd && 2 * g->ph <= g->kh && 2 * g->pw <= g->kw,
                  MRI3D_EINVAL, "%s: output dims inconsistent with input", who);
    return MRI3D_OK;
}

static int pool_bwd_check(const Mri3dPoolGeom* g, bool addend, int32_t a_ld, const char* who) {
    if (int rc = pool_check(g, who)) return rc;
    MRI3D_REQUIRE(!addend || a_ld >= g->c, MRI3D_EINVAL, "%s: addend pitch %d < %d channels", who, a_ld, g->c);
    return MRI3D_OK;
}

extern "C" int mri3d_maxpool3d_fwd(const Mri3dPoolGeom* g, const void* x, void* y, uint8_t* idx,
                                   mri3d_stream_t stream) {
    if (int rc = pool_check(g, "maxpool3d_fwd")) return rc;
    MRI3D_REQUIRE(x && y && idx, MRI3D_EINVAL, "maxpool3d_fwd: null pointer");
    const ResamplePlan p = pool_fwd_plan(*g, ptr_align(x, y), ptr_align(idx));
    hipStream_t s = static_cast<hipStream_t>(stream);
    MRI3D_DISPATCH_DTYPE(g->dtype, T, {
        if (p.kern == ResampleKernel::maxpool2_fwd)
            with_int<4, 8>(p.vec, [&](auto V) {
                if constexpr (has_vec<T, V.value>) launch<maxpool2_fwd_kernel<T, V.value>>(p, s, *g, (const T*)x, (T*)y, idx, p.hch);
// ... 101 lines not shown
                        launch<upsample2x_fwd_march_kernel<T, VEC, N.value>>(p, s, *g, (const T*)x, (T*)y, p.segs, p.segl, p.tilesH, p.tilesW,
                                                                              p.passes, p.items);
                });
            });
        else
            with_int<1, 4>(p.vec, [&](auto V) { launch<upsample_fwd_kernel<T, V.value>>(p, s, *g, (const T*)x, (T*)y, p.hch); });
    });
    return check_launch(p.name);
}

extern "C" int mri3d_upsample3d_bwd(const Mri3dUpGeom* g, const void* dy, void* dx, void* workspace, size_t ws_bytes,
                                    mri3d_stream_t stream) {
    if (int rc = up_check(g, "upsample3d_bwd")) return rc;
    MRI3D_REQUIRE(dy && dx, MRI3D_EINVAL, "upsample3d_bwd: null pointer");
    MRI3D_REQUIRE(workspace && ws_bytes >= mri3d_upsample3d_workspace_bytes(g), MRI3D_EWORKSPACE,
                  "upsample3d_bwd: workspace %zu < %zu", ws_bytes, mri3d_upsample3d_workspace_bytes(g));
    const ResamplePlan p = up_bwd_plan(*g, ptr_align(dx, dy));
    hipStream_t s = static_cast<hipStream_t>(stream);
    int* tab = static_cast<int*>(workspace);
    if (p.tables) hipLaunchKernelGGL(upsample_tables_kernel, dim3(3), dim3(256), 0, s, *g, tab);
    MRI3D_DISPATCH_DTYPE(g->dtype, T, {
        switch (p.kern) {
        case ResampleKernel::up2x_bwd_march:
            launch<upsample2x_bwd_march_kernel<T>>(p, s, *g, (const T*)dy, (T*)dx, p.segs, p.tilesH, p.tilesW, p.passes, p.items);
            break;
        case ResampleKernel::up2x_bwd_tile:
            launch<upsample2x_bwd_kernel<T>>(p, s, *g, (const T*)dy, (T*)dx, p.segs, p.tilesH, p.tilesW, p.items);
            break;
        case ResampleKernel::up_nearest_int_bwd:
            with_int<2, 4>(p.npv, [&](auto S) { launch<upsample_nearest_int_bwd_kernel<T, S.value>>(p, s, *g, (const T*)dy, (T*)dx, p.hch); });
            break;
        default:
            with_int<1, 4>(p.vec, [&](auto V) { launch<upsample_bwd_kernel<T, V.value>>(p, s, *g, (const T*)dy, (T*)dx, (const int*)tab, p.hch); });
        }
    });
    return check_launch(p.name);
}

extern "C" int mri3d_upsample3d_route(const Mri3dUpGeom* g, int32_t pass, int32_t align, char* name, size_t name_bytes) {
    if (int rc = route_args_check(pass, name, name_bytes, "upsample3d_route")) return rc;
    if (int rc = up_check(g, "upsample3d_route")) return rc;
    const ResamplePlan p = pass == MRI3D_PASS_FWD ? up_fwd_plan(*g, align) : up_bwd_plan(*g, align);
    snprintf(name, name_bytes, "%s", p.name);
    return MRI3D_OK;
}

extern "C" int32_t mri3d_upsample3d_plan_query(const Mri3dUpGeom* g, int32_t pass, int32_t align, Mri3dResamplePlanInfo* out) {
    MRI3D_REQUIRE(out != nullptr, MRI3D_EINVAL, "upsample3d_plan_query: null result");
    MRI3D_REQUIRE(pass == MRI3D_PASS_FWD || pass == MRI3D_PASS_DGRAD, MRI3D_EINVAL, "upsample3d_plan_query: unknown pass %d", pass);
    if (int rc = up_check(g, "upsample3d_plan_query")) return rc;
    plan_info(pass == MRI3D_PASS_FWD ? up_fwd_plan(*g, align) : up_bwd_plan(*g, align), out);
    return MRI3D_OK;
}
```

### mri_epilepsy_diagnosis_amd/nn.py

```python
import math

import torch
import torch.nn as tnn

from . import ops


class Conv3d(tnn.Conv3d):
    def forward(self, x):
        if self.padding_mode != "zeros" or self.groups != 1 or isinstance(self.padding, str):
            raise NotImplementedError("mri3d Conv3d supports padding_mode='zeros', groups=1, numeric padding")
        return ops.conv3d(x, self.weight, self.bias, self.stride, self.padding, self.dilation)


class ConvTranspose3d(tnn.ConvTranspose3d):
    def forward(self, x, output_size=None):
        if output_size is not None or self.groups != 1 or self.padding_mode != "zeros":
            raise NotImplementedError("mri3d ConvTranspose3d supports groups=1, zero padding, no output_size")
        return ops.conv_transpose3d(x, self.weight, self.bias, self.stride, self.padding, self.output_padding,
                                    self.dilation)


class BayesConv3d(tnn.Module):

# ... 89 lines not shown
    if isinstance(norm, tnn.GroupNorm):
        return ops.norm_act(x, norm.weight, norm.bias, alpha, None, None, "group", 0.1, norm.eps, kind, slope, out,
                            norm.num_channels // norm.num_groups)
    raise NotImplementedError("unsupported normalisation module %r" % (norm,))


def _plain_pointwise(head):
    return (isinstance(head, Conv3d) and tuple(head.kernel_size) == (1, 1, 1) and tuple(head.stride) == (1, 1, 1)
            and tuple(head.dilation) == (1, 1, 1) and head.groups == 1 and head.padding_mode == "zeros"
            and not isinstance(head.padding, str) and tuple(head.padding) == (0, 0, 0))


def _local_stats_spec(norm, act):
    kind, alpha, slope = _act_spec(act)
    if norm is None:
        return "none", (None, None, alpha, None, None, "none", 0.1, 0.0), kind, alpha, slope
    if not isinstance(norm, tnn.modules.batchnorm._BatchNorm) or norm.momentum is None:
        return None
    mode, args = _batchnorm_spec(norm, alpha)
    return None if mode == "sync" else (mode, args, kind, alpha, slope)


def _fused_tail(norm, act, supported, asked, run, given):
    spec = _local_stats_spec(norm, act)
    if spec is None:
        return None
    mode, args, kind, alpha, slope = spec
    if not supported(*asked, mode, kind, alpha):
        return None
    _count_batch(norm)
    return run(*given, *args, act=kind, slope=slope)


def fused_norm_act_head(norm, act, x, head):
    if not _plain_pointwise(head):
        return None
    cast = ops.autocast_dtype()
    if cast is not None and x.dtype != cast:
        return None
    return _fused_tail(norm, act, ops.norm_act_pointwise_supported, (x, head.weight), ops.norm_act_pointwise,
                       (x, head.weight, head.bias))


def fused_norm_act_pool(norm, act, x, pool):
    if (not isinstance(pool, tnn.MaxPool3d) or pool.ceil_mode or pool.return_indices or pool.dilation not in (1, (1, 1, 1))
            or not x.is_cuda):
        return None
    if x.dtype != torch.float32:
        return None
    return _fused_tail(norm, act, ops.norm_act_pool_supported, (x, pool.kernel_size, pool.stride, pool.padding), ops.norm_act_pool,
                       (x,))


def conv_norm_act(conv, norm, act, x, out=None, head=None, pool=None):
    wants = (isinstance(norm, tnn.modules.batchnorm._BatchNorm) and (norm.training or norm.running_mean is None)
             and ops.sync_batchnorm_reducer() is None and isinstance(conv, Conv3d) and conv.padding_mode == "zeros"
             and conv.groups == 1 and not isinstance(conv.padding, str))
    if isinstance(x, (tuple, list)):
        xa, xb = x
        plain = (isinstance(conv, Conv3d) and conv.padding_mode == "zeros" and conv.groups == 1 and not isinstance(conv.padding, str)
                 and tuple(conv.stride) == (1, 1, 1) and tuple(conv.dilation) == (1, 1, 1))
        if plain:
            y = ops.conv3d_cat(xa, xb, conv.weight, conv.bias, conv.padding, bn_stats=wants)
        else:
            y = conv(ops.cat_channels([xa, xb]))
    elif wants:
        y = ops.conv3d(x, conv.weight, conv.bias, conv.stride, conv.padding, conv.dilation, bn_stats=True)
    else:
        y = conv(x)
    if head is not None:
        logits = fused_norm_act_head(norm, act, y, head) if out is None else None
        return logits if logits is not None else head(fused_norm_act(norm, act, y, out))
    if pool is not None:
        both = fused_norm_act_pool(norm, act, y, pool) if out is None else None
        return both if both is not None else pool.forward_with_skip(fused_norm_act(norm, act, y, out))
    return fused_norm_act(norm, act, y, out)


class GroupNorm(tnn.GroupNorm):
    def forward(self, x):
        return fused_norm_act(self, None, x)


class BatchNorm3d(tnn.BatchNorm3d):
    def forward(self, x):
        return fused_norm_act(self, None, x)


class InstanceNorm3d(tnn.InstanceNorm3d):
    def forward(self, x):
        return fused_norm_act(self, None, x)


class PReLU(tnn.PReLU):
    def forward(self, x):
        if x.dim() != 5:
            return super().forward(x)
        return fused_norm_act(None, self, x)


class ReLU(tnn.ReLU):
    def forward(self, x):
        if x.dim() != 5:
            return super().forward(x)
        return fused_norm_act(None, self, x)


class LeakyReLU(tnn.LeakyReLU):
    def forward(self, x):
        if x.dim() != 5:
            return super().forward(x)
        return fused_norm_act(None, self, x)


class MaxPool3d(tnn.MaxPool3d):
    def forward(self, x):
        if self.ceil_mode or self.return_indices or self.dilation not in (1, (1, 1, 1)):
            raise NotImplementedError("mri3d MaxPool3d supports floor mode, dilation 1, no indices")
        return ops.max_pool3d(x, self.kernel_size, self.stride, self.padding)

    def forward_with_skip(self, x):
        if self.ceil_mode or self.return_indices or self.dilation not in (1, (1, 1, 1)):
            raise NotImplementedError("mri3d MaxPool3d supports floor mode, dilation 1, no indices")
        return ops.max_pool3d_skip(x, self.kernel_size, self.stride, self.padding)


def _pair(v):
    return (v, v) if isinstance(v, int) else tuple(v)
# ... 96 lines not shown
```

### mri_epilepsy_diagnosis_amd/ops.py

```python
import collections
import ctypes
import math

import torch

from . import _lib
from ._lib import (ACT_LEAKY, ACT_NONE, ACT_PRELU, ACT_RELU, BF16, F32, NORM_PASS_BWD, NORM_PASS_FWD, NORM_PASS_STATS, PASS_DGRAD,
                   PASS_FWD, PASS_WGRAD, UP_NEAREST, UP_TRILINEAR, ConvGeom, DiceGeom, NormGeom, NormPlanInfo, PoolGeom, UpGeom,
                   check)

CL3D = torch.channels_last_3d



def _require_device(*ts):
    for t in ts:
        if t is None:
            continue
        if not t.is_cuda:
            raise RuntimeError(
                "mri_epilepsy_diagnosis_amd ops run only on a ROCm device tensor (got %s); there is no CPU fallback"
                % t.device)
        if t.dtype not in (torch.float32, torch.bfloat16):
            raise RuntimeError("mri_epilepsy_diagnosis_amd ops: only float32 / bfloat16 tensors are supported, got %s"
# ... 269 lines not shown
    ho = (hi + 2 * ph - dh * (kh - 1) - 1) // sh + 1
    wo = (wi + 2 * pw - dw * (kw - 1) - 1) // sw + 1
    if do <= 0 or ho <= 0 or wo <= 0:
        raise RuntimeError("Kernel size can't be greater than actual input size")
    return ConvGeom(n, di, hi, wi, ci, do, ho, wo, co, kd, kh, kw, sd, sh, sw, pd, ph, pw, dd, dh, dw,
                    ci if x_ld is None else x_ld, co if y_ld is None else y_ld, dtype)


def _ptr_align(*ts):
    bits = 16
    for t in ts:
        if t is not None:
            bits |= t.data_ptr()
    return bits & -bits


def conv_route(g, pass_, stats=False, bias=False, split=0, second_ld=0, align=16, x_align=None, y_align=None):
    name = ctypes.create_string_buffer(64)
    xa, ya = align if x_align is None else x_align, align if y_align is None else y_align
    check(_lib.lib().mri3d_conv3d_route(ctypes.byref(g), pass_, int(bool(stats)), int(bool(bias)), split, second_ld, xa, ya, name, 64),
          "conv3d_route")
    return name.value.decode()


def pool_route(g, pass_, addend_ld=0, align=16, idx_align=16):
    name = ctypes.create_string_buffer(64)
    check(_lib.lib().mri3d_maxpool3d_route(ctypes.byref(g), pass_, addend_ld, align, idx_align, name, 64), "maxpool3d_route")
    return name.value.decode()


def upsample_route(g, pass_, align=16):
    name = ctypes.create_string_buffer(64)
    check(_lib.lib().mri3d_upsample3d_route(ctypes.byref(g), pass_, align, name, 64), "upsample3d_route")
    return name.value.decode()


RESAMPLE_PLAN_FIELDS = ("vec", "npv", "hch", "grid", "segs", "segl", "tiles_h", "tiles_w", "passes", "items", "tables", "lds_bytes")


def _resample_plan_dict(info):
    return {f: int(getattr(info, f)) for f in RESAMPLE_PLAN_FIELDS}


def pool_plan(g, pass_, addend_ld=0, align=16, idx_align=16):
    info = _lib.ResamplePlanInfo()
    check(_lib.lib().mri3d_maxpool3d_plan_query(ctypes.byref(g), pass_, addend_ld, align, idx_align, ctypes.byref(info)),
          "maxpool3d_plan_query")
    return _resample_plan_dict(info)


def upsample_plan(g, pass_, align=16):
    info = _lib.ResamplePlanInfo()
    check(_lib.lib().mri3d_upsample3d_plan_query(ctypes.byref(g), pass_, align, ctypes.byref(info)), "upsample3d_plan_query")
    return _resample_plan_dict(info)


FUSEDCONV_PLAN_FIELDS = ("hch", "grid", "gtrips", "trips", "per", "passes", "chunks", "slabs", "rows")


def upconv_plan(g, scale, pass_):
    info = _lib.FusedConvPlanInfo()
    check(_lib.lib().mri3d_upconv3d_plan_query(ctypes.byref(g), scale, pass_, ctypes.byref(info)), "upconv3d_plan_query")
    return {f: int(getattr(info, f)) for f in FUSEDCONV_PLAN_FIELDS}


def conv_pair_plan(first, second):
    info = _lib.FusedConvPlanInfo()
    check(_lib.lib().mri3d_convpair_plan_query(ctypes.byref(first), ctypes.byref(second), ctypes.byref(info)), "convpair_plan_query")
    return {f: int(getattr(info, f)) for f in FUSEDCONV_PLAN_FIELDS}


MARCH_PLAN_FIELDS = ("chunks", "blocks", "wgh", "wgw", "gch", "gcw", "nseg", "seglen", "nbuf", "grid", "whole_chunks", "dispatcher",
                     "smem_bytes", "wp_bytes")


def conv_march_plan(g, pass_, stats=False):
    info = _lib.MarchPlanInfo()
    check(_lib.lib().mri3d_conv3d_march_plan_query(ctypes.byref(g), pass_, 1 if stats else 0, ctypes.byref(info)),
          "conv3d_march_plan_query")
    return {f: int(getattr(info, f)) for f in MARCH_PLAN_FIELDS}


def norm_plan(g, pass_, align=16):
    info = NormPlanInfo()
    check(_lib.lib().mri3d_norm_plan_query(ctypes.byref(g), pass_, align, ctypes.byref(info)), "norm_plan_query")
    return (info.vec, info.CL, info.VT, info.cy, info.nblk, info.groups, info.gvox)


def _stuffed_wgrad_ok(g):
    return ((g.kd, g.kh, g.kw) == (3, 3, 3) and (g.sd, g.sh, g.sw) == (2, 2, 2) and (g.pd, g.ph, g.pw) == (1, 1, 1)
            and (g.dd, g.dh, g.dw) == (1, 1, 1) and g.ci % 8 == 0 and g.co % 4 == 0 and g.x_ld % 4 == 0)


_ONE = (1, 1, 1)
_ConvPasses = collections.namedtuple("_ConvPasses", "fwd dgrad wgrad stuffed layer")


def _conv_passes(xshape, wshape, stride, padding, dilation, dtype=F32, x_ld=None, dy_ld=None, dx_ld=None):
    fwd = _conv_geom(xshape, wshape, stride, padding, dilation, x_ld=x_ld, dtype=dtype)
    dgrad = _conv_geom(xshape, wshape, stride, padding, dilation, x_ld=dx_ld, y_ld=dy_ld, dtype=dtype)
    wgrad = _conv_geom(xshape, wshape, stride, padding, dilation, x_ld=fwd.x_ld, y_ld=dy_ld, dtype=dtype)
    stuffed = _conv_geom(xshape, wshape, _ONE, _ONE, _ONE, x_ld=fwd.x_ld, dtype=dtype) if _stuffed_wgrad_ok(fwd) else None
    return _ConvPasses(fwd, dgrad, wgrad, stuffed, (tuple(xshape), tuple(wshape), stride, padding, dilation, dtype, x_ld, dx_ld))


def _for_gradient_pitch(p, dy_ld):
# ... 228 lines not shown
        L = _lib.lib()
        xa, a_ld = _nd(xa)
        xb, b_ld = _nd(xb)
        w = weight.contiguous()
        p = _cat_passes(xa, xb, w.shape, a_ld)
        g, ca = p.fwd, xa.shape[1]
        y = _new((g.n, g.co, g.dout, g.ho, g.wo), xa)
        ws_bytes = L.mri3d_conv3d_workspace_bytes(ctypes.byref(g), PASS_FWD)
        part = None
        if stats_holder is not None:
            part = _stats_partials(stats_holder, L.mri3d_conv3d_fwd_cat_stats_blocks(ctypes.byref(g), ca, b_ld), g, xa, bias)
        _launch(L.mri3d_conv3d_fwd_cat, lambda: _conv_tag("fwd", g) + " cat" + (" +bn-stats" if part is not None else ""),
                lambda: _conv_work(g, "fwd"), ws_bytes, xa.device, g, xa, xb, ca, b_ld, w, bias, y, part)
        ctx.save_for_backward(xa, xb, w)
        ctx.passes, ctx.b_ld, ctx.params = p, b_ld, (weight, bias)
        return y

    @staticmethod
    def backward(ctx, dy):
        xa, xb, w = ctx.saved_tensors
        dy, y_ld = _nd(dy)
        p = _for_gradient_pitch(ctx.passes, y_ld)
        ca, cb = xa.shape[1], xb.shape[1]
        dxa = dxb = None
        if ctx.needs_input_grad[0] or ctx.needs_input_grad[1]:
            dxa, dxb = _new(xa.shape, xa), _new(xb.shape, xb)
            _conv_launch(_lib.lib().mri3d_conv3d_dgrad_cat, PASS_DGRAD, p.dgrad, dy.device, dy, w, dxa, dxb, ca, cb, suffix=" cat")
        dw, db = _conv_param_grads(ctx, 2, ctx.params, lambda dw, db: _conv_wgrad(p.wgrad, xa, dy, w, db is not None, dw, db,
                                                                                 split=(xb, ca, ctx.b_ld)))
        return dxa, dxb, dw, db, None


def conv3d_cat(xa, xb, weight, bias=None, padding=1, bn_stats=False):
    xa, xb = _autocast_in(xa), _autocast_in(xb)
    ok = (xa.is_cuda and xa.dim() == 5 and xb.shape[0] == xa.shape[0] and xb.shape[2:] == xa.shape[2:] and xa.dtype == xb.dtype
          and tuple(weight.shape[2:]) == (3, 3, 3) and _triple(padding) == (1, 1, 1) and weight.shape[1] == xa.shape[1] + xb.shape[1])
    if ok:
        L = _lib.lib()
        a_nd, a_ld = _nd(xa)
        b_nd, b_ld = _nd(xb)
        ca, cb = xa.shape[1], xb.shape[1]
        p = _cat_passes(a_nd, b_nd, weight.shape, a_ld)
        ok = (a_nd.data_ptr() % 16 == 0 and b_nd.data_ptr() % 16 == 0
              and L.mri3d_conv3d_cat_supported(ctypes.byref(p.fwd), ca, b_ld, PASS_FWD)
              and L.mri3d_conv3d_cat_supported(ctypes.byref(p.fwd), ca, b_ld, PASS_WGRAD)
              and L.mri3d_conv3d_cat_supported(ctypes.byref(p.dgrad), ca, cb, PASS_DGRAD))
    if not ok:
        return conv3d(cat_channels([xa, xb]), weight, bias, 1, padding, 1, bn_stats=bn_stats)
    return _apply_with_bn_stats(_Conv3dCatFn, bn_stats, xa, xb, weight, bias)


def conv3d(x, weight, bias=None, stride=1, padding=0, dilation=1, bn_stats=False):
    return _apply_with_bn_stats(_Conv3dFn, bn_stats, _autocast_in(x), weight, bias, _triple(stride), _triple(padding), _triple(dilation))




class _BayesWeightsFn(torch.autograd.Function):

    @staticmethod
    def forward(ctx, mu, logsigma, evaluate, threshold):
        _require_param(mu, logsigma)
        if mu.shape != logsigma.shape:
            raise RuntimeError("bayes_conv3d: mu_weight %s and logsigma_weight %s differ in shape" % (tuple(mu.shape), tuple(logsigma.shape)))
        mu, logsigma = mu.contiguous(), logsigma.contiguous()
        w_var, log_alpha = torch.empty_like(mu), torch.empty_like(mu)
        w_mean = torch.empty_like(mu) if evaluate else None
        check(_lib.lib().mri3d_bayes_weights_fwd(_ptr(mu), _ptr(logsigma), mu.numel(), int(evaluate), float(threshold), _ptr(w_mean),
                                                 _ptr(w_var), _ptr(log_alpha), _stream()), "bayes_weights_fwd")
        ctx.save_for_backward(mu, logsigma)
        ctx.evaluate, ctx.threshold = bool(evaluate), float(threshold)
        ctx.set_materialize_grads(False)
        return (w_mean, w_var, log_alpha) if evaluate else (w_var, log_alpha)

    @staticmethod
    def backward(ctx, *grads):
        mu, logsigma = ctx.saved_tensors
        d_w_mean, d_w_var, d_log_alpha = grads if ctx.evaluate else (None,) + grads
        d_w_mean, d_w_var, d_log_alpha = (None if g is None else g.contiguous() for g in (d_w_mean, d_w_var, d_log_alpha))
        dmu, dls = torch.empty_like(mu), torch.empty_like(mu)
        check(_lib.lib().mri3d_bayes_weights_bwd(_ptr(mu), _ptr(logsigma), mu.numel(), int(ctx.evaluate), ctx.threshold, _ptr(d_w_mean),
                                                 _ptr(d_w_var), _ptr(d_log_alpha), _ptr(dmu), _ptr(dls), _stream()),
              "bayes_weights_bwd")
        return dmu, dls, None, None


def _stream_work(n_tensors, like, eps_numel=0):
    return {"flops": 0.0, "bytes": _esz(like) * n_tensors * like.numel() + 4.0 * eps_numel}


def _bayes_square(x, x_ld):
    n, c, d, h, w = x.shape
    x2 = _new(x.shape, x)
    _launch(_lib.lib().mri3d_bayes_square, lambda: "bayes_square %d @%dx%dx%d n%d" % (c, d, h, w, n), lambda: _stream_work(2, x), None, None,
            x, x2, n * d * h * w, c, x_ld, c, _dt(x))
    return x2


class _BayesConv3dFn(torch.autograd.Function):

    @staticmethod
    def forward(ctx, x, w_mean, w_var, mu_bias, logsigma_bias, eps, stride, padding, dilation):
        _require_device(x)
        _require_param(w_mean, w_var, mu_bias, logsigma_bias, eps)
        L = _lib.lib()
        x, x_ld = _nd(x)
# ... 274 lines not shown
            raise RuntimeError("%s backward: gradient dtype %s does not match activation dtype %s" % (who, t.dtype, x.dtype))
    if g0.x_ld != g0.c:
        x = x.contiguous(memory_format=CL3D)
    return x


class _NormActFn(torch.autograd.Function):

    @staticmethod
    def forward(ctx, x, gamma, beta, alpha, running_mean, running_var, stats_mode, momentum, eps, act, slope, out, group_c=0,
                fused_stats=None):
        _require_device(x)
        _require_param(gamma, beta, alpha)
        ctx.params = (gamma, beta, alpha)
        L = _lib.lib()
        x, x_ld = _nd(x)
        n, c, d, h, w = x.shape
        act_code = _ACT_CODES[act]
        instance = 1 if stats_mode in ("instance", "group") else 0
        if stats_mode == "group" and (group_c <= 0 or c % group_c):
            raise RuntimeError("group norm: channels per group %d must divide C=%d" % (group_c, c))
        group_c = group_c if stats_mode == "group" else 0
        if out is None:
            y, y_ld, y_off = _new(x.shape, x), c, 0
        else:
            buf, y_off = out
            y_ld = _pitch_of(buf)
            if (y_ld != buf.shape[1] or tuple(buf.shape[2:]) != (d, h, w) or buf.shape[0] != n or y_off + c > buf.shape[1]
                    or buf.dtype != x.dtype):
                raise RuntimeError("norm_act(out=): buffer %s cannot hold a %s slice at channel %d"
                                   % (tuple(buf.shape), tuple(x.shape), y_off))
            y = _slice_view(buf, y_off, c)
        g = _norm_geom(x, x_ld, y_ld, act_code, alpha, slope, eps, instance, group_c)
        ctx.training_stats = stats_mode in ("batch", "instance", "group")
        ctx.sync = _sync_bn_reducer if stats_mode == "sync" else None
        if stats_mode == "sync":
            if ctx.sync is None:
                raise RuntimeError("norm_act(stats_mode='sync') needs ops.set_sync_batchnorm(reducer)")
            mean, invstd, ctx.sync_count = _sync_statistics(ctx.sync, g, x, running_mean, running_var, momentum, eps)
        else:
            mode = "batch" if ctx.training_stats else (stats_mode if stats_mode == "running" else "none")
            mean, invstd = _norm_statistics("norm_act", g, x, n if instance else 1, mode, None if instance else running_mean,
                                            None if instance else running_var, momentum, eps, fused_stats)
        with _timed(lambda: "norm_act_fwd c%d vox%d n%d" % (c, g.vox, n), lambda: {"flops": 0.0, "bytes": 2 * _esz(x) * x.numel()}):
            check(L.mri3d_norm_act_fwd(ctypes.byref(g), _ptr(x), _ptr(mean), _ptr(invstd), _ptr(gamma), _ptr(beta),
                                       _ptr(alpha) if act_code == ACT_PRELU else None, _ptr(y), _stream()),
                  "norm_act_fwd")
        ctx.save_for_backward(x, mean, invstd, gamma, beta, alpha)
        ctx.geom = g
        return y

    @staticmethod
    def backward(ctx, dy):
        L = _lib.lib()
        x, mean, invstd, gamma, beta, alpha = ctx.saved_tensors
        g0 = ctx.geom
        dy, dy_ld = _nd(dy)
        x = _backward_x("norm_act", x, g0, dy)
        dx = _new(x.shape, x)
        g = _repitched(g0, g0.c, dy_ld)
        prelu = g.act == ACT_PRELU
        sinks, grads = _grad_slots(ctx, (gamma, beta, alpha if prelu else None))
        dgamma_k, dbeta_k, dalpha = grads
        sync = ctx.sync
        if sync is not None:
            dbeta_k = dbeta_k if dbeta_k is not None else torch.empty(g.c, dtype=torch.float32, device=x.device)
            dgamma_k = dgamma_k if dgamma_k is not None else torch.empty(g.c, dtype=torch.float32, device=x.device)
        ws = _workspace(L.mri3d_norm_workspace_bytes(ctypes.byref(g)), x.device)
        with _timed(lambda: "norm_act_bwd c%d vox%d n%d" % (g.c, g.vox, g.n), lambda: {"flops": 0.0, "bytes": 5 * _esz(x) * x.numel()}):
            check(L.mri3d_norm_act_bwd(ctypes.byref(g), 1 if ctx.training_stats else 0, _ptr(x), _ptr(dy), _ptr(mean),
                                       _ptr(invstd), _ptr(gamma), _ptr(beta), _ptr(alpha) if prelu else None, _ptr(dx),
                                       _ptr(dgamma_k), _ptr(dbeta_k), _ptr(dalpha), _ptr(ws), ws.numel(), _stream()),
                  "norm_act_bwd")
        if sync is not None:
            _sync_correct_dx(sync, g, x, mean, invstd, gamma, dbeta_k, dgamma_k, ctx.sync_count, dx)
        return (dx, *_grad_slots_done(ctx, grads, sinks), None, None, None, None, None, None, None, None, None, None)


def norm_act(x, gamma=None, beta=None, alpha=None, running_mean=None, running_var=None, stats_mode="batch",
             momentum=0.1, eps=1e-5, act=None, slope=0.01, out=None, group_c=0):
    fused = _fused_stats_of(x, stats_mode, momentum)
    return _NormActFn.apply(x, gamma, beta, alpha, running_mean, running_var, stats_mode, momentum, eps, act, slope, out,
                            group_c, fused)


def _fusable_x_ld(x, stats_mode, act):
    if stats_mode not in ("batch", "running", "none") or act not in _ACT_CODES:
        return None
    if not (x.dim() == 5 and x.dtype in (torch.float32, torch.bfloat16)):
        return None
    x_ld = _pitch_of(x)
    if x_ld is None:
        return x.shape[1]
    return None if x.data_ptr() % (4 * x.element_size()) else x_ld


def norm_act_pointwise_supported(x, weight, stats_mode="batch", act=None, alpha=None):
    x_ld = _fusable_x_ld(x, stats_mode, act) if x.is_cuda else None
    if x_ld is None:
        return False
    if weight.dim() != 5 or tuple(weight.shape[2:]) != (1, 1, 1) or weight.shape[1] != x.shape[1] or weight.dtype != torch.float32:
        return False
    g = _norm_geom(x, x_ld, weight.shape[0], _ACT_CODES[act], alpha, 0.0, 0.0)
    return bool(_lib.lib().mri3d_norm_act_pw_supported(ctypes.byref(g), weight.shape[0]))


class _NormActPointwiseFn(torch.autograd.Function):

    @staticmethod
    def forward(ctx, x, gamma, beta, alpha, weight, bias, running_mean, running_var, stats_mode, momentum, eps, act, slope,
                fused_stats=None):
        _require_device(x)
        _require_param(gamma, beta, alpha, weight, bias)
        ctx.params = (gamma, beta, alpha, weight, bias)
        L = _lib.lib()
        x, x_ld = _nd(x)
        n, c, d, h, w = x.shape
        co = weight.shape[0]
        act_code = _ACT_CODES[act]
        wm = weight.contiguous()
        g = _norm_geom(x, x_ld, co, act_code, alpha, slope, eps)
        if not L.mri3d_norm_act_pw_supported(ctypes.byref(g), co):
            raise RuntimeError("norm_act_pointwise: c=%d co=%d pitch %d is not served (ask norm_act_pointwise_supported first)"
                               % (c, co, x_ld))
        mean, invstd = _norm_statistics("norm_act_pointwise", g, x, 1, stats_mode, running_mean, running_var, momentum, eps,
                                        fused_stats)
        out = _new((n, co, d, h, w), x)
        with _timed(lambda: "norm_act_pw_fwd c%d->%d vox%d n%d" % (c, co, g.vox, n),
                    lambda: {"flops": 2.0 * co * c * n * g.vox, "bytes": _esz(x) * (x.numel() + out.numel())}):
# ... 88 lines not shown
        ctx.pooled_shape = tuple(pooled.shape)
        ctx.training_stats = stats_mode == "batch"
        ctx.set_materialize_grads(False)
        return pooled, skip

    @staticmethod
    def backward(ctx, dpool, dskip):
        L = _lib.lib()
        if dpool is None and dskip is None:
            return (None,) * 12
        x, idx, mean, invstd, gamma, beta, alpha = ctx.saved_tensors
        g0 = ctx.geom
        n, c, d, h, w = x.shape
        s_ld = p_ld = c
        for name, t, shape in (("pooled", dpool, ctx.pooled_shape), ("skip", dskip, tuple(x.shape))):
            if t is not None and tuple(t.shape) != shape:
                raise RuntimeError("norm_act_pool backward: %s gradient %s does not match %s" % (name, tuple(t.shape), shape))
        if dskip is not None:
            dskip, s_ld = _nd(dskip)
            if s_ld % 4 or dskip.data_ptr() % (4 * dskip.element_size()):
                dskip, s_ld = dskip.contiguous(memory_format=CL3D), c
        if dpool is not None:
            dpool, p_ld = _nd(dpool)
            if p_ld % 4 or dpool.data_ptr() % (4 * dpool.element_size()):
                dpool, p_ld = dpool.contiguous(memory_format=CL3D), c
        x = _backward_x("norm_act_pool", x, g0, dpool, dskip)
        two = (2, 2, 2)
        g = _repitched(g0, c, s_ld)
        pg, _ = _pool_geom(x, s_ld, p_ld, two, two, (0, 0, 0))
        prelu = g.act == ACT_PRELU
        sinks, grads = _grad_slots(ctx, (gamma, beta, alpha if prelu else None))
        dx = _new(x.shape, x) if ctx.needs_input_grad[0] else None
        ws = _workspace(L.mri3d_norm_act_pool_workspace_bytes(ctypes.byref(g), ctypes.byref(pg)), x.device)
        passes = 2 if ctx.training_stats else 1
        npool = idx.numel()
        with _timed(lambda: "norm_act_pool_bwd c%d" % c,
                    lambda: {"flops": 0.0,
                             "bytes": passes * (_esz(x) * (x.numel() + (x.numel() if dskip is not None else 0))
                                                + ((_esz(x) + 1) * npool if dpool is not None else 0))
                                      + (_esz(x) * x.numel() if dx is not None else 0)}):
            check(L.mri3d_norm_act_pool_bwd(ctypes.byref(g), ctypes.byref(pg), 1 if ctx.training_stats else 0, _ptr(x),
                                            _ptr(dskip), _ptr(dpool), _ptr(idx), _ptr(mean), _ptr(invstd), _ptr(gamma),
                                            _ptr(beta), _ptr(alpha) if prelu else None, _ptr(dx), _ptr(grads[0]), _ptr(grads[1]),
                                            _ptr(grads[2]), _ptr(ws), ws.numel(), _stream()), "norm_act_pool_bwd")
        return (dx, *_grad_slots_done(ctx, grads, sinks), None, None, None, None, None, None, None, None)


def norm_act_pool(x, gamma=None, beta=None, alpha=None, running_mean=None, running_var=None, stats_mode="batch",
                  momentum=0.1, eps=1e-5, act=None, slope=0.01):
    fused = _fused_stats_of(x, stats_mode, momentum)
    return _NormActPoolFn.apply(x, gamma, beta, alpha, running_mean, running_var, stats_mode, momentum, eps, act, slope, fused)


def activation(x, act, alpha=None, slope=0.01):
    return norm_act(x, None, None, alpha, None, None, "none", 0.1, 0.0, act, slope)


class _ScaleInstanceFn(torch.autograd.Function):

    @staticmethod
    def forward(ctx, x, scale):
        _require_device(x)
        _require_param(scale)
        L = _lib.lib()
        x = _cl(x)
        n, c, d, h, w = x.shape
        g = NormGeom(n, d * h * w, c, c, c, 1, ACT_NONE, 1, 0.0, 0.0, 0, _dt(x))
        scale = scale.reshape(n * c).contiguous()
        zeros = torch.zeros_like(scale)
        y = _new(x.shape, x)
        check(L.mri3d_norm_act_fwd(ctypes.byref(g), _ptr(x), _ptr(zeros), _ptr(scale), None, None, None, _ptr(y),
                                   _stream()), "norm_act_fwd")
        ctx.save_for_backward(scale, zeros)
        ctx.geom = g
        return y

    @staticmethod
    def backward(ctx, dy):
        L = _lib.lib()
        scale, zeros = ctx.saved_tensors
        g = ctx.geom
        dy = _cl(dy)
        dx = _new(dy.shape, dy)
        check(L.mri3d_norm_act_fwd(ctypes.byref(g), _ptr(dy), _ptr(zeros), _ptr(scale), None, None, None, _ptr(dx),
                                   _stream()), "norm_act_fwd")
        return dx, None


def dropout3d(x, p, training):
    if not training or p == 0.0:
        return x
    n, c = x.shape[0], x.shape[1]
    keep = torch.empty(n, c, device=x.device, dtype=torch.float32).bernoulli_(1.0 - p)
    return _ScaleInstanceFn.apply(x, keep / (1.0 - p))




def _pool_out(i, k, s, p, ceil_mode):
    if ceil_mode:
        o = -(-(i + 2 * p - k) // s) + 1
        if (o - 1) * s >= i + p:
            o -= 1
        return o
    return (i + 2 * p - k) // s + 1

# ... 18 lines not shown

    @staticmethod
    def backward(ctx, dy):
        return _pool_backward(ctx, dy)


def _pool_backward(ctx, dy, dskip=None, ds_ld=0):
    (idx,) = ctx.saved_tensors
    dy, dy_ld = _nd(dy)
    dx = _new(ctx.xshape, dy)
    g = _repitched(ctx.geom, ctx.geom.c, dy_ld, _dt(dy))
    if dskip is None:
        _launch(_lib.lib().mri3d_maxpool3d_bwd, lambda: "maxpool_bwd c%d" % g.c,
                lambda: {"flops": 0.0, "bytes": _esz(dy) * dx.numel() + (_esz(dy) + 1) * dy.numel()}, None, dy.device, g, dy, idx, dx)
    else:
        _launch(_lib.lib().mri3d_maxpool3d_bwd_add, lambda: "maxpool_bwd+skip c%d" % g.c,
                lambda: {"flops": 0.0, "bytes": _esz(dy) * 2 * dx.numel() + (_esz(dy) + 1) * dy.numel()}, None, dy.device,
                g, dy, idx, dskip, ds_ld, dx)
    return dx, None, None, None


class _MaxPoolSkipFn(torch.autograd.Function):

    @staticmethod
    def forward(ctx, x, kernel, stride, padding):
        y = _MaxPool3dFn.forward(ctx, x, kernel, stride, padding)
        return y, x.view_as(x)

    @staticmethod
    def backward(ctx, dy, dskip):
        if dskip is None:
            return _MaxPool3dFn.backward(ctx, dy)
        if dy is None:
            return dskip, None, None, None
        dskip, ds_ld = _nd(dskip)
        if tuple(dskip.shape) != ctx.xshape or dskip.dtype != dy.dtype:
            raise RuntimeError("max_pool3d_skip backward: skip gradient %s %s does not match the input %s %s"
                               % (tuple(dskip.shape), dskip.dtype, ctx.xshape, dy.dtype))
        return _pool_backward(ctx, dy, dskip, ds_ld)


def max_pool3d_skip(x, kernel_size, stride=None, padding=0):
    k = _triple(kernel_size)
    s = _triple(stride) if stride is not None else k
    return _MaxPoolSkipFn.apply(x, k, s, _triple(padding))


def max_pool3d(x, kernel_size, stride=None, padding=0):
    k = _triple(kernel_size)
    s = _triple(stride) if stride is not None else k
    return _MaxPool3dFn.apply(x, k, s, _triple(padding))




class _Upsample3dFn(torch.autograd.Function):
    @staticmethod
    def forward(ctx, x, out_size, mode, align_corners, ratios, out):
        _require_device(x)
        x, x_ld = _nd(x)
        n, c, d, h, w = x.shape
        do, ho, wo = out_size
        if out is None:
            y, y_ld = _new((n, c, do, ho, wo), x), c
        else:
            buf, y_off = out
            y_ld = _pitch_of(buf)
            if (y_ld != buf.shape[1] or tuple(buf.shape[2:]) != (do, ho, wo) or buf.shape[0] != n
                    or y_off + c > buf.shape[1] or buf.dtype != x.dtype):
                raise RuntimeError("upsample3d(out=): buffer %s cannot hold a %s slice at channel %d"
                                   % (tuple(buf.shape), (n, c, do, ho, wo), y_off))
            y = _slice_view(buf, y_off, c)
        g = UpGeom(n, d, h, w, do, ho, wo, c, x_ld, y_ld, mode, 1 if align_corners else 0, ratios[0], ratios[1], ratios[2],
                   _dt(x))
        _launch(_lib.lib().mri3d_upsample3d_fwd, lambda: "upsample_fwd c%d" % c,
                lambda: {"flops": 0.0, "bytes": _esz(x) * (x.numel() + y.numel())}, None, x.device, g, x, y)
        ctx.geom = g
        ctx.xshape = tuple(x.shape)
        return y

    @staticmethod
    def backward(ctx, dy):
        L = _lib.lib()
        dy, dy_ld = _nd(dy)
        dx = _new(ctx.xshape, dy)
        g = _repitched(ctx.geom, ctx.geom.c, dy_ld, _dt(dy))
        _launch(L.mri3d_upsample3d_bwd, lambda: "upsample_bwd c%d" % g.c, lambda: {"flops": 0.0, "bytes": _esz(dy) * (dx.numel() + dy.numel())},
                L.mri3d_upsample3d_workspace_bytes(ctypes.byref(g)), dy.device, g, dy, dx)
        return dx, None, None, None, None, None


def upsample3d(x, size=None, scale_factor=None, mode="nearest", align_corners=None, out=None):
    if mode == "linear":
        mode = "trilinear"
    if mode not in ("nearest", "trilinear"):
        raise NotImplementedError("upsample3d: mode %r is not supported" % (mode,))
    if mode == "nearest" and align_corners is not None:
        raise ValueError("align_corners option can only be set with the interpolating modes")
    in_sz = tuple(x.shape[2:])
    if (size is None) == (scale_factor is None):
        raise ValueError("exactly one of size or scale_factor must be given")
    if size is not None:
        out_sz = _triple(size)
        sf = None
    else:
        sf = tuple(float(s) for s in (scale_factor if isinstance(scale_factor, (tuple, list)) else (scale_factor,) * 3))
        out_sz = tuple(int(math.floor(float(i) * s)) for i, s in zip(in_sz, sf))
    ac = bool(align_corners)
    ratios = []
    for a in range(3):
        i, o = in_sz[a], out_sz[a]
        if mode == "trilinear" and ac:
            r = (i - 1) / (o - 1) if o > 1 else 0.0
        elif sf is not None:
            r = 1.0 / sf[a]
        else:
            r = i / o
        ratios.append(float(r))
    code = UP_NEAREST if mode == "nearest" else UP_TRILINEAR
    return _Upsample3dFn.apply(x, out_sz, code, ac, tuple(ratios), out)


class _UpConv3dFn(torch.autograd.Function):

    @staticmethod
    def forward(ctx, x, weight, bias, scale, padding):
        _require_device(x)
        _require_param(weight, bias)
        x, x_ld = _nd(x)
        w = weight.contiguous()
        p = _upconv_passes(x.shape, w.shape, scale, padding, _dt(x), x_ld)
        g = p.fwd
        y = _new((g.n, g.co, g.dout, g.ho, g.wo), x)
        _launch(_lib.lib().mri3d_upconv3d_fwd, lambda: _conv_tag("fwd", g) + " of nearest x%d" % scale,
                lambda: {"flops": _conv_work(g, "fwd")["flops"], "bytes": _esz(x) * (x.numel() + y.numel())},
                None, None, g, scale, x, w, bias, y)
        ctx.save_for_backward(x, w)
        ctx.passes, ctx.scale, ctx.params = p, scale, (weight, bias)
        return y

    @staticmethod
    def backward(ctx, dy):
# ... 429 lines not shown
```

### mri_epilepsy_diagnosis_amd/unet/unet.py

```python
import torch
import torch.nn as tnn

from .. import nn as mnn
from .. import ops

_UPSAMPLING = {"nearest": "nearest", "linear": "trilinear", "trilinear": "trilinear"}


class ConvolutionalBlock(tnn.Module):
    def __init__(self, dimensions, in_channels, out_channels, normalization=None, kernel_size=3, activation="ReLU",
                 preactivation=False, padding=0, padding_mode="zeros", dilation=None, dropout=0):
        super().__init__()
        if dimensions != 3:
            raise NotImplementedError("only the 3-D U-Net of the reference is implemented")
        if preactivation or padding_mode != "zeros" or dropout:
            raise NotImplementedError("preactivation / non-zero padding_mode / dropout are not used by the reference")
        dilation = 1 if dilation is None else dilation
        if padding:
            total = kernel_size + 2 * (dilation - 1) - 1
            padding = total // 2
        conv = mnn.Conv3d(in_channels, out_channels, kernel_size, padding=padding, dilation=dilation)
        norm = None
        if normalization is not None:
            norm = {"batch": mnn.BatchNorm3d, "instance": mnn.InstanceNorm3d}[normalization.lower()](out_channels)
        act = None
        if activation is not None:
            act = {"PReLU": mnn.PReLU, "ReLU": mnn.ReLU, "LeakyReLU": mnn.LeakyReLU}[activation]()
        self.conv_layer = conv
        self.norm_layer = norm
        self.activation_layer = act
        self.dropout_layer = None
        self.block = tnn.Sequential(*[m for m in (conv, norm, act) if m is not None])

    def forward(self, x, out=None, head=None, pool=None):
        return mnn.conv_norm_act(self.conv_layer, self.norm_layer, self.activation_layer, x, out, head, pool)


class EncodingBlock(tnn.Module):
    def __init__(self, in_channels, out_channels_first, dimensions, normalization, pooling_type, preactivation=False,
                 is_first_block=False, residual=False, padding=0, padding_mode="zeros", activation="ReLU",
                 dilation=None, dropout=0):
        super().__init__()
        if residual:
            raise NotImplementedError("residual encoding blocks are not used by the reference")
        self.conv1 = ConvolutionalBlock(dimensions, in_channels, out_channels_first,
                                        normalization=None if is_first_block else normalization,
                                        padding=padding, activation=activation, dilation=dilation)
        out_channels_second = 2 * out_channels_first
        self.conv2 = ConvolutionalBlock(dimensions, out_channels_first, out_channels_second, normalization=normalization,
                                        padding=padding, activation=activation, dilation=dilation)
        self.downsample = None
        if pooling_type is not None:
            if pooling_type != "max":
                raise NotImplementedError("only max pooling is used by the reference")
            self.downsample = mnn.MaxPool3d(kernel_size=2)

    def forward(self, x, skip_out=None, head=None, fused_pool=True):
        if self.downsample is None:
            return self.conv2(self.conv1(x), skip_out, head)
        if fused_pool and skip_out is None and isinstance(self.downsample, mnn.MaxPool3d):
            return self.conv2(self.conv1(x), pool=self.downsample)
        x = self.conv2(self.conv1(x), skip_out)
        return self.downsample.forward_with_skip(x)

    @property
    def out_channels(self):
        return self.conv2.conv_layer.out_channels


class Encoder(tnn.Module):
    def __init__(self, in_channels, out_channels_first, dimensions, pooling_type, num_encoding_blocks, normalization,
                 padding=0, activation="ReLU", initial_dilation=None):
        super().__init__()
        self.encoding_blocks = tnn.ModuleList()
        self.dilation = initial_dilation
        first = True
        for _ in range(num_encoding_blocks):
            blk = EncodingBlock(in_channels, out_channels_first, dimensions, normalization, pooling_type,
                                is_first_block=first, padding=padding, activation=activation, dilation=self.dilation)
            first = False
            self.encoding_blocks.append(blk)
            in_channels = 2 * out_channels_first
            out_channels_first = in_channels
            if self.dilation is not None:
                self.dilation *= 2

    def forward(self, x, cat_bufs=None, fused_pool=True):
        skips = []
        for i, blk in enumerate(self.encoding_blocks):
            x, skip = blk(x, None if cat_bufs is None else (cat_bufs[i], 0), fused_pool=fused_pool)
            skips.append(skip)
        return skips, x

    @property
    def out_channels(self):
        return self.encoding_blocks[-1].out_channels


class DecodingBlock(tnn.Module):
    def __init__(self, in_channels_skip_connection, dimensions, upsampling_type, normalization, padding=0,
                 activation="ReLU", dilation=None):
        super().__init__()
        if upsampling_type == "conv":
            c = 2 * in_channels_skip_connection
            self.upsample = mnn.ConvTranspose3d(c, c, kernel_size=2, stride=2)
        else:
            mode = _UPSAMPLING[upsampling_type]
            self.upsample = mnn.Upsample(scale_factor=2, mode=mode, align_corners=False if mode == "trilinear" else None)
        in_first = in_channels_skip_connection * 3
        self.conv1 = ConvolutionalBlock(dimensions, in_first, in_channels_skip_connection, normalization=normalization,
                                        padding=padding, activation=activation, dilation=dilation)
        self.conv2 = ConvolutionalBlock(dimensions, in_channels_skip_connection, in_channels_skip_connection,
                                        normalization=normalization, padding=padding, activation=activation,
                                        dilation=dilation)

    def forward(self, skip, x, cat_buf=None, head=None):
        if cat_buf is not None and isinstance(self.upsample, mnn.Upsample):
            up = ops.upsample3d(x, self.upsample.size, self.upsample.scale_factor, self.upsample.mode,
                                self.upsample.align_corners, out=(cat_buf, skip.shape[1]))
            return self.conv2(self.conv1(ops.join_channels(cat_buf, [skip, up])), head=head)
        x = self.upsample(x)
        if skip.shape[2:] != x.shape[2:]:
            raise NotImplementedError("padding=False (centre-cropped skips) is not used by the reference")
        return self.conv2(self.conv1((skip, x)), head=head)


class Decoder(tnn.Module):
    def __init__(self, in_channels_skip_connection, dimensions, upsampling_type, num_decoding_blocks, normalization,
                 padding=0, activation="ReLU", initial_dilation=None):
        super().__init__()
        self.decoding_blocks = tnn.ModuleList()
        self.dilation = initial_dilation
        for _ in range(num_decoding_blocks):
            self.decoding_blocks.append(DecodingBlock(in_channels_skip_connection, dimensions, upsampling_type,
                                                      normalization, padding=padding, activation=activation,
                                                      dilation=self.dilation))
            in_channels_skip_connection //= 2
            if self.dilation is not None:
                self.dilation //= 2

    def forward(self, skips, x, cat_bufs=None, head=None):
        last = min(len(skips), len(self.decoding_blocks)) - 1
        for j, (skip, blk) in enumerate(zip(reversed(skips), self.decoding_blocks)):
            x = blk(skip, x, None if cat_bufs is None else cat_bufs[len(skips) - 1 - j], head if j == last else None)
        return x


class UNet(tnn.Module):
    def __init__(self, in_channels=1, out_classes=2, dimensions=2, num_encoding_blocks=5, out_channels_first_layer=64,
                 normalization=None, pooling_type="max", upsampling_type="conv", preactivation=False, residual=False,
                 padding=0, padding_mode="zeros", activation="ReLU", initial_dilation=None, dropout=0,
                 monte_carlo_dropout=0):
        super().__init__()
        if dimensions != 3:
            raise NotImplementedError("only dimensions=3 (the reference's configuration) is implemented")
        if preactivation or residual or dropout or padding_mode != "zeros":
            raise NotImplementedError("option not used by the reference and not implemented")
        if not padding:
            raise NotImplementedError("padding=False (valid convolutions + cropped skips) is not used by the reference")
        depth = num_encoding_blocks - 1
        self.encoder = Encoder(in_channels, out_channels_first_layer, dimensions, pooling_type, depth, normalization,
                               padding=padding, activation=activation, initial_dilation=initial_dilation)
        c = self.encoder.out_channels if depth > 0 else in_channels
        first = c if depth > 0 else out_channels_first_layer
        self.bottom_block = EncodingBlock(c, first, dimensions, normalization, pooling_type=None, padding=padding,
                                          activation=activation, dilation=self.encoder.dilation,
                                          is_first_block=depth == 0)
        skip_channels = out_channels_first_layer * 2 ** depth
        self.decoder = Decoder(skip_channels, dimensions, upsampling_type, depth, normalization, padding=padding,
                               activation=activation, initial_dilation=self.encoder.dilation)
        self.monte_carlo_layer = mnn.Dropout3d(p=monte_carlo_dropout) if monte_carlo_dropout else None
        self.shared_concat_buffers = False
        self.fused_head = True
        self.fused_pool = True
        self.classifier = ConvolutionalBlock(dimensions, 2 * out_channels_first_layer, out_classes, kernel_size=1,
                                             activation=None)

    def forward(self, x):
        cat_bufs = None
        if self.shared_concat_buffers and x.is_cuda and len(self.encoder.encoding_blocks) and all(
                isinstance(b.upsample, mnn.Upsample) for b in self.decoder.decoding_blocks):
            cat_bufs = []
            n, sp = x.shape[0], tuple(x.shape[2:])
            for blk in self.encoder.encoding_blocks:
                if any(s % 2 for s in sp):
                    cat_bufs = None
                    break
                cat_bufs.append(ops.new_cat_buffer(n, 3 * blk.out_channels, sp, x))
                sp = tuple(s // 2 for s in sp)
        clf = self.classifier
        mc = self.monte_carlo_layer
        mc = mc if (mc is not None and mc.training and mc.p > 0) else None
        head = clf.conv_layer if (self.fused_head and mc is None and x.is_cuda and clf.norm_layer is None
                                  and clf.activation_layer is None and clf.dropout_layer is None) else None
        skips, enc = self.encoder(x, cat_bufs, self.fused_pool)
        if not skips:
            x = self.bottom_block(enc, head=head)
        else:
            x = self.decoder(skips, self.bottom_block(enc), cat_bufs, head)
        if head is not None:
            return x
        return self.classifier(x if mc is None else mc(x))
```

Before: 68.86 volumes/s.

## Fuse norm+PReLU with trilinear upsample and add cin1 conv+PReLU kernels

Adds a fused BatchNorm-apply + activation + 2x trilinear upsample kernel, so decoder blocks emit the upsampled tensor directly instead of writing the normalized activation and then upsampling it in a separate pass. The decoder consumes the upsampled output without going through the concat-buffer path. It also adds a first-layer conv (single input channel) kernel that applies PReLU in its epilogue and computes the PReLU alpha gradient inside wgrad, but that path is disabled by default. Both aim to cut full-resolution memory traffic and kernel launches, at the cost of more specialised code paths and a recomputation-based backward.

```diff
diff --git a/include/mri3d.h b/include/mri3d.h
--- a/include/mri3d.h
+++ b/include/mri3d.h
@@ -45,6 +45,18 @@
 
 int mri3d_conv3d_route(const Mri3dConvGeom* g, int32_t pass, int32_t stats, int32_t bias, int32_t split, int32_t second_ld,
                        int32_t align_x, int32_t align_y, char* name, size_t name_bytes);
+
+typedef struct Mri3dCin1PreluPlanInfo {
+    int32_t tiles_d, tiles_h, tiles_w, tiles, grid, shares;
+    int64_t ws_bytes;
+} Mri3dCin1PreluPlanInfo;
+int32_t mri3d_conv3d_cin1_prelu_supported(const Mri3dConvGeom* g, int32_t alpha_n);
+int32_t mri3d_conv3d_cin1_prelu_plan_query(const Mri3dConvGeom* g, int32_t alpha_n, int32_t pass, Mri3dCin1PreluPlanInfo* out);
+int mri3d_conv3d_cin1_prelu_fwd(const Mri3dConvGeom* g, const void* x, const void* w, const void* bias, const float* alpha,
+                                int32_t alpha_n, void* y, void* a, void* workspace, size_t ws_bytes, mri3d_stream_t stream);
+int mri3d_conv3d_cin1_prelu_wgrad(const Mri3dConvGeom* g, const void* x, const void* y, const void* da, const float* alpha,
+                                  int32_t alpha_n, void* dw, void* dbias, float* dalpha, void* workspace, size_t ws_bytes,
+                                  mri3d_stream_t stream);
 
 int32_t mri3d_conv3d_cat_supported(const Mri3dConvGeom* g, int32_t split, int32_t second_ld, int32_t pass);
 int32_t mri3d_conv3d_fwd_cat_stats_blocks(const Mri3dConvGeom* g, int32_t split, int32_t second_ld);
@@ -182,6 +194,11 @@
 int32_t mri3d_maxpool3d_plan_query(const Mri3dPoolGeom* g, int32_t pass, int32_t addend_ld, int32_t align_tensors,
                                    int32_t align_idx, Mri3dResamplePlanInfo* out);
 int32_t mri3d_upsample3d_plan_query(const Mri3dUpGeom* g, int32_t pass, int32_t align, Mri3dResamplePlanInfo* out);
+
+int32_t mri3d_norm_act_upsample_supported(const Mri3dNormGeom* g, const Mri3dUpGeom* ug);
+int32_t mri3d_norm_act_upsample_plan_query(const Mri3dNormGeom* g, const Mri3dUpGeom* ug, Mri3dResamplePlanInfo* out);
+int mri3d_norm_act_upsample_fwd(const Mri3dNormGeom* g, const Mri3dUpGeom* ug, const void* x, const float* mean, const float* invstd,
+                                const float* gamma, const float* beta, const float* alpha, void* y, mri3d_stream_t stream);
 
 typedef struct Mri3dDiceGeom {
     int32_t n;
diff --git a/mri_epilepsy_diagnosis_amd/_lib.py b/mri_epilepsy_diagnosis_amd/_lib.py
--- a/mri_epilepsy_diagnosis_amd/_lib.py
+++ b/mri_epilepsy_diagnosis_amd/_lib.py
@@ -38,6 +38,10 @@
 class FusedConvPlanInfo(Structure):
     _fields_ = [(n, c_int32) for n in ("hch", "grid", "gtrips", "trips", "per", "passes", "chunks")] + \
                [("slabs", c_int64), ("rows", c_int64)]
+
+
+class Cin1PreluPlanInfo(Structure):
+    _fields_ = [(n, c_int32) for n in ("tiles_d", "tiles_h", "tiles_w", "tiles", "grid", "shares")] + [("ws_bytes", c_int64)]
 
 
 class MarchPlanInfo(Structure):
@@ -79,6 +83,10 @@
     "mri3d_conv3d_dgrad": (c_int32, [POINTER(ConvGeom), _P, _P, _P, _P, _P, c_size_t, _P]),
     "mri3d_conv3d_wgrad": (c_int32, [POINTER(ConvGeom), _P, _P, _P, _P, _P, c_size_t, _P]),
     "mri3d_conv3d_route": (c_int32, [POINTER(ConvGeom), c_int32, c_int32, c_int32, c_int32, c_int32, c_int32, c_int32, c_char_p, c_size_t]),
+    "mri3d_conv3d_cin1_prelu_supported": (c_int32, [POINTER(ConvGeom), c_int32]),
+    "mri3d_conv3d_cin1_prelu_plan_query": (c_int32, [POINTER(ConvGeom), c_int32, c_int32, POINTER(Cin1PreluPlanInfo)]),
+    "mri3d_conv3d_cin1_prelu_fwd": (c_int32, [POINTER(ConvGeom), _P, _P, _P, _FP, c_int32, _P, _P, _P, c_size_t, _P]),
+    "mri3d_conv3d_cin1_prelu_wgrad": (c_int32, [POINTER(ConvGeom), _P, _P, _P, _FP, c_int32, _P, _P, _FP, _P, c_size_t, _P]),
     "mri3d_conv3d_cat_supported": (c_int32, [POINTER(ConvGeom), c_int32, c_int32, c_int32]),
     "mri3d_conv3d_fwd_cat_stats_blocks": (c_int32, [POINTER(ConvGeom), c_int32, c_int32]),
     "mri3d_conv3d_fwd_cat": (c_int32, [POINTER(ConvGeom), _P, _P, c_int32, c_int32, _P, _P, _P, _P, _P, c_size_t, _P]),
@@ -126,6 +134,9 @@
     "mri3d_upsample3d_bwd": (c_int32, [POINTER(UpGeom), _P, _P, _P, c_size_t, _P]),
     "mri3d_upsample3d_route": (c_int32, [POINTER(UpGeom), c_int32, c_int32, c_char_p, c_size_t]),
     "mri3d_upsample3d_plan_query": (c_int32, [POINTER(UpGeom), c_int32, c_int32, POINTER(ResamplePlanInfo)]),
+    "mri3d_norm_act_upsample_supported": (c_int32, [POINTER(NormGeom), POINTER(UpGeom)]),
+    "mri3d_norm_act_upsample_plan_query": (c_int32, [POINTER(NormGeom), POINTER(UpGeom), POINTER(ResamplePlanInfo)]),
+    "mri3d_norm_act_upsample_fwd": (c_int32, [POINTER(NormGeom), POINTER(UpGeom), _P, _FP, _FP, _FP, _FP, _FP, _P, _P]),
     "mri3d_softmax_dice_workspace_bytes": (c_size_t, [POINTER(DiceGeom)]),
     "mri3d_softmax_dice_fwd": (c_int32, [POINTER(DiceGeom), _P, _P, _FP, _FP, _P, c_size_t, _P]),
     "mri3d_softmax_dice_bwd": (c_int32, [POINTER(DiceGeom), _P, _P, _FP, _FP, _P, _P]),
diff --git a/mri_epilepsy_diagnosis_amd/build.py b/mri_epilepsy_diagnosis_amd/build.py
--- a/mri_epilepsy_diagnosis_amd/build.py
+++ b/mri_epilepsy_diagnosis_amd/build.py
@@ -85,12 +85,12 @@
     return lib
 
 
-def build_host_sanitizer(verbose=True):
+def build_host_sanitizer(verbose=True, driver="host_sanitizer_driver.cpp"):
     root = os.path.join(HERE, "..")
-    driver = os.path.join(root, "tests", "native", "host_sanitizer_driver.cpp")
+    driver = os.path.join(root, "tests", "native", driver)
     out_dir = os.path.join(root, "tests", "native", "build")
     os.makedirs(out_dir, exist_ok=True)
-    exe = os.path.join(out_dir, "host_sanitizer_driver")
+    exe = os.path.join(out_dir, os.path.basename(driver).rsplit(".", 1)[0])
     flags = ["--offload-arch=gfx950", "-fsanitize=address,undefined", "-fno-gpu-sanitize", "-fno-sanitize-recover=undefined", "-fno-omit-frame-pointer",
              "-O1", "-g", "-std=c++17", "-w", "-I", os.path.join(root, "include")]
     h = hashlib.sha256(" ".join(flags).encode())
@@ -102,12 +102,22 @@
     if os.path.exists(exe) and os.path.exists(stamp) and open(stamp).read() == h.hexdigest():
         return exe
 
+    headers = [f for f in inputs if f.endswith(".h")]
+
     def one(src):
         obj = os.path.join(out_dir, os.path.basename(src).rsplit(".", 1)[0] + ".host.o")
+        oh = hashlib.sha256(" ".join(flags).encode())
+        for f in [src] + headers:
+            with open(f, "rb") as fh:
+                oh.update(fh.read())
+        if os.path.exists(obj) and os.path.exists(obj + ".sha") and open(obj + ".sha").read() == oh.hexdigest():
+            return obj
         cmd = [HIPCC] + flags + (["-x", "hip"] if src.endswith(".hip") else []) + ["-c", src, "-o", obj]
         r = subprocess.run(cmd, capture_output=True, text=True, timeout=900)
         if r.returncode != 0:
             raise RuntimeError("host sanitizer build failed for %s:\n%s" % (src, r.stderr[-3000:]))
+        with open(obj + ".sha", "w") as f:
+            f.write(oh.hexdigest())
         return obj
     with ThreadPoolExecutor(max_workers=4) as ex:
         objs = list(ex.map(one, [os.path.join(CSRC, s) for s in SOURCES] + [driver]))
diff --git a/mri_epilepsy_diagnosis_amd/csrc/api.hip b/mri_epilepsy_diagnosis_amd/csrc/api.hip
--- a/mri_epilepsy_diagnosis_amd/csrc/api.hip
+++ b/mri_epilepsy_diagnosis_amd/csrc/api.hip
@@ -213,6 +213,41 @@
     case ConvBackend::mfma: return conv_mfma_wgrad(*g, x, dy, (float*)dw, (float*)dbias, workspace, ws_bytes, s);
     default: return conv_generic_wgrad(*g, x, dy, (float*)dw, (float*)dbias, workspace, ws_bytes, s);
     }
+}
+
+extern "C" int32_t mri3d_conv3d_cin1_prelu_supported(const Mri3dConvGeom* g, int32_t alpha_n) {
+    Mri3dCin1PreluPlanInfo info;
+    return (g != nullptr && conv_check(g, "conv3d_cin1_prelu_supported") == MRI3D_OK &&
+            conv_cin1_prelu_plan_info(*g, alpha_n, MRI3D_PASS_FWD, info) && conv_cin1_prelu_plan_info(*g, alpha_n, MRI3D_PASS_WGRAD, info)) ? 1 : 0;
+}
+
+extern "C" int32_t mri3d_conv3d_cin1_prelu_plan_query(const Mri3dConvGeom* g, int32_t alpha_n, int32_t pass, Mri3dCin1PreluPlanInfo* out) {
+    int rc = conv_check(g, "conv3d_cin1_prelu_plan_query");
+    if (rc) return rc;
+    MRI3D_REQUIRE(out != nullptr, MRI3D_EINVAL, "conv3d_cin1_prelu_plan_query: null result");
+    MRI3D_REQUIRE(pass == MRI3D_PASS_FWD || pass == MRI3D_PASS_WGRAD, MRI3D_EINVAL, "conv3d_cin1_prelu_plan_query: unknown pass %d", pass);
+    MRI3D_REQUIRE(conv_cin1_prelu_plan_info(*g, alpha_n, pass, *out), MRI3D_ENOTSUP,
+                  "conv3d_cin1_prelu_plan_query: ci=%d co=%d alpha_n=%d not served", g->ci, g->co, alpha_n);
+    return MRI3D_OK;
+}
+
+extern "C" int mri3d_conv3d_cin1_prelu_fwd(const Mri3dConvGeom* g, const void* x, const void* w, const void* bias, const float* alpha,
+                                           int32_t alpha_n, void* y, void* a, void* workspace, size_t ws_bytes, mri3d_stream_t stream) {
+    int rc = conv_check(g, "conv3d_cin1_prelu_fwd");
+    if (rc) return rc;
+    MRI3D_REQUIRE(x && w && alpha && y && a, MRI3D_EINVAL, "conv3d_cin1_prelu_fwd: null pointer");
+    return conv_cin1_prelu_fwd(*g, x, (const float*)w, (const float*)bias, alpha, alpha_n, y, a, workspace, ws_bytes,
+                               static_cast<hipStream_t>(stream));
+}
+
+extern "C" int mri3d_conv3d_cin1_prelu_wgrad(const Mri3dConvGeom* g, const void* x, const void* y, const void* da, const float* alpha,
+                                             int32_t alpha_n, void* dw, void* dbias, float* dalpha, void* workspace, size_t ws_bytes,
+                                             mri3d_stream_t stream) {
+    int rc = conv_check(g, "conv3d_cin1_prelu_wgrad");
+    if (rc) return rc;
+    MRI3D_REQUIRE(x && y && da && alpha && dw, MRI3D_EINVAL, "conv3d_cin1_prelu_wgrad: null pointer");
+    return conv_cin1_prelu_wgrad(*g, x, y, da, alpha, alpha_n, (float*)dw, (float*)dbias, dalpha, workspace, ws_bytes,
+                                 static_cast<hipStream_t>(stream));
 }
 
 extern "C" int mri3d_conv3d_route(const Mri3dConvGeom* g, int32_t pass, int32_t stats, int32_t bias, int32_t split, int32_t second_ld,
diff --git a/mri_epilepsy_diagnosis_amd/csrc/conv_backends.h b/mri_epilepsy_diagnosis_amd/csrc/conv_backends.h
--- a/mri_epilepsy_diagnosis_amd/csrc/conv_backends.h
+++ b/mri_epilepsy_diagnosis_amd/csrc/conv_backends.h
@@ -16,6 +16,11 @@
 int conv_generic_wgrad(const Mri3dConvGeom& g, const void* x, const void* dy, float* dw, float* dbias, void* ws,
                        size_t ws_bytes, hipStream_t s);
 bool conv_generic_route_name(const Mri3dConvGeom& g, int pass, bool bias, int ax, int ay, char* name, size_t name_bytes);
+bool conv_cin1_prelu_plan_info(const Mri3dConvGeom& g, int alpha_n, int pass, Mri3dCin1PreluPlanInfo& out);
+int conv_cin1_prelu_fwd(const Mri3dConvGeom& g, const void* x, const float* w, const float* bias, const float* alpha, int alpha_n,
+                        void* y, void* a, void* ws, size_t ws_bytes, hipStream_t s);
+int conv_cin1_prelu_wgrad(const Mri3dConvGeom& g, const void* x, const void* y, const void* da, const float* alpha, int alpha_n,
+                          float* dw, float* dbias, float* dalpha, void* ws, size_t ws_bytes, hipStream_t s);
 
 bool conv_mfma_supported(const Mri3dConvGeom& g, int pass);
 size_t conv_mfma_workspace_bytes(const Mri3dConvGeom& g, int pass);
diff --git a/mri_epilepsy_diagnosis_amd/csrc/conv_generic.hip b/mri_epilepsy_diagnosis_amd/csrc/conv_generic.hip
--- a/mri_epilepsy_diagnosis_amd/csrc/conv_generic.hip
+++ b/mri_epilepsy_diagnosis_amd/csrc/conv_generic.hip
@@ -923,10 +923,19 @@
     }
 }
 
-template <typename T, int CO>
-__global__ void __launch_bounds__(256)
-conv_cin1_fwd_kernel(Mri3dConvGeom g, const T* __restrict__ x, const float* __restrict__ wp, const float* __restrict__ bias,
-                     T* __restrict__ y, int tilesD, int tilesH, int tilesW, int ntiles) {
+template <typename T>
+struct Cin1Prelu {
+    T* act;
+    const T* y;
+    double* dal_part;
+    const float* alpha;
+    int alpha_n;
+};
+
+template <typename T, int CO, bool PRELU>
+__device__ __forceinline__ void
+conv_cin1_fwd_body(const Mri3dConvGeom& g, const T* __restrict__ x, const float* __restrict__ wp, const float* __restrict__ bias,
+                   T* __restrict__ y, int tilesD, int tilesH, int tilesW, int ntiles, const Cin1Prelu<T>& pr) {
     constexpr int VPT = Cin1<CO>::VPT, TW = C1WQ * VPT, PW = TW + 4;
     __shared__ __attribute__((aligned(16))) float xs[(C1D + 2) * (C1H + 2) * PW];
     __shared__ __attribute__((aligned(16))) float wsh[27 * CO];
@@ -936,6 +945,11 @@
     float bv[CO];
 #pragma unroll
     for (int c = 0; c < CO; ++c) bv[c] = bias ? bias[c] : 0.f;
+    float al[PRELU ? CO : 1];
+    if constexpr (PRELU) {
+#pragma unroll
+        for (int c = 0; c < CO; ++c) al[c] = pr.alpha[pr.alpha_n == 1 ? 0 : c];
+    }
     for (int tile = blockIdx.x; tile < ntiles; tile += gridDim.x) {
         int n, d0, h0, w0;
         decode_tile(tile, tilesD, tilesH, tilesW, TW, n, d0, h0, w0);
@@ -977,7 +991,8 @@
             for (int c = 0; c < CO / 2; ++c) asm volatile("" : "+v"(acc[v][c]));
         const int od = d0 + dl, oh = h0 + hl;
         if (od < g.dout && oh < g.ho) {
-            T* yo = y + ((((int64_t)n * g.dout + od) * g.ho + oh) * g.wo + w0 + wq * VPT) * g.y_ld;
+            const int64_t off = ((((int64_t)n * g.dout + od) * g.ho + oh) * g.wo + w0 + wq * VPT) * g.y_ld;
+            T* yo = y + off;
 #pragma unroll
             for (int v = 0; v < VPT; ++v)
                 if (w0 + wq * VPT + v < g.wo) {
@@ -985,15 +1000,38 @@
                     for (int c = 0; c < CO; c += 4)
                         stf4(yo + (int64_t)v * g.y_ld + c,
                              make_float4(acc[v][c / 2].x, acc[v][c / 2].y, acc[v][c / 2 + 1].x, acc[v][c / 2 + 1].y));
+                    if constexpr (PRELU) {
+#pragma unroll
+                        for (int c = 0; c < CO; c += 4)
+                            stf4(pr.act + off + (int64_t)v * g.y_ld + c,
+                                 make_float4(apply_act(fmaf(acc[v][c / 2].x, 1.f, 0.f), MRI3D_ACT_PRELU, al[c]),
+                                             apply_act(fmaf(acc[v][c / 2].y, 1.f, 0.f), MRI3D_ACT_PRELU, al[c + 1]),
+                                             apply_act(fmaf(acc[v][c / 2 + 1].x, 1.f, 0.f), MRI3D_ACT_PRELU, al[c + 2]),
+                                             apply_act(fmaf(acc[v][c / 2 + 1].y, 1.f, 0.f), MRI3D_ACT_PRELU, al[c + 3])));
+                    }
                 }
         }
     }
 }
 
 template <typename T, int CO>
-__global__ void __launch_bounds__(768)
-conv_cin1_wgrad_kernel(Mri3dConvGeom g, const T* __restrict__ x, const T* __restrict__ dy, float* __restrict__ part,
-                       float* __restrict__ bias_part, int tilesD, int tilesH, int tilesW, int ntiles, int nshares) {
+__global__ void __launch_bounds__(256)
+conv_cin1_fwd_kernel(Mri3dConvGeom g, const T* __restrict__ x, const float* __restrict__ wp, const float* __restrict__ bias,
+                     T* __restrict__ y, int tilesD, int tilesH, int tilesW, int ntiles) {
+    conv_cin1_fwd_body<T, CO, false>(g, x, wp, bias, y, tilesD, tilesH, tilesW, ntiles, Cin1Prelu<T>{});
+}
+
+template <typename T, int CO>
+__global__ void __launch_bounds__(256)
+conv_cin1_prelu_fwd_kernel(Mri3dConvGeom g, const T* __restrict__ x, const float* __restrict__ wp, const float* __restrict__ bias,
+                           T* __restrict__ y, int tilesD, int tilesH, int tilesW, int ntiles, Cin1Prelu<T> pr) {
+    conv_cin1_fwd_body<T, CO, true>(g, x, wp, bias, y, tilesD, tilesH, tilesW, ntiles, pr);
+}
+
+template <typename T, int CO, bool PRELU>
+__device__ __forceinline__ void
+conv_cin1_wgrad_body(const Mri3dConvGeom& g, const T* __restrict__ x, const T* __restrict__ dy, float* __restrict__ part,
+                     float* __restrict__ bias_part, int tilesD, int tilesH, int tilesW, int ntiles, int nshares, const Cin1Prelu<T>& pr) {
     constexpr int VPT = Cin1<CO>::VPT, TW = C1WQ * VPT, PW = TW + 4, NA = 9 * CO + CO;
     __shared__ __attribute__((aligned(16))) float xs[(C1D + 2) * (C1H + 2) * PW];
     __shared__ float red[12][NA];
@@ -1012,6 +1050,12 @@
             for (int c = 0; c < CO / 2; ++c) acc[a][b][c] = f32x2{0.f, 0.f};
 #pragma unroll
     for (int c = 0; c < CO; ++c) bsum[c] = 0.f;
+    float al[PRELU ? CO : 1];
+    double dal[PRELU ? CO : 1];
+    if constexpr (PRELU) {
+#pragma unroll
+        for (int c = 0; c < CO; ++c) { al[c] = pr.alpha[pr.alpha_n == 1 ? 0 : c]; dal[c] = 0.0; }
+    }
     for (int tile = share; tile < ntiles; tile += nshares) {
         int n, d0, h0, w0;
         decode_tile(tile, tilesD, tilesH, tilesW, TW, n, d0, h0, w0);
@@ -1023,11 +1067,25 @@
         for (int v = 0; v < VPT; ++v) {
             const int ow = w0 + wq * VPT + v;
             const bool ok = od < g.dout && oh < g.ho && ow < g.wo;
-            const T* dp = dy + ((((int64_t)n * g.dout + min(od, g.dout - 1)) * g.ho + min(oh, g.ho - 1)) * g.wo +
-                                min(ow, g.wo - 1)) * g.y_ld;
+            const int64_t off = ((((int64_t)n * g.dout + min(od, g.dout - 1)) * g.ho + min(oh, g.ho - 1)) * g.wo +
+                                 min(ow, g.wo - 1)) * g.y_ld;
+            const T* dp = dy + off;
 #pragma unroll
             for (int c = 0; c < CO; c += 4) {
-                const float4 q = ldf4(dp + c);
+                float4 q = ldf4(dp + c);
+                if constexpr (PRELU) {
+                    const float4 yq = ldf4(pr.y + off + c);
+                    const float gq[4] = {q.x, q.y, q.z, q.w}, yv[4] = {yq.x, yq.y, yq.z, yq.w};
+                    float dq[4];
+#pragma unroll
+                    for (int j = 0; j < 4; ++j) {
+                        const float u = fmaf(1.f, yv[j], 0.f);
+                        const bool pos = u > 0.f;
+                        dq[j] = 1.f * (pos ? gq[j] : gq[j] * al[c + j]);
+                        if (kd == 1) dal[c + j] += (ok && !pos) ? (double)gq[j] * (double)u : 0.0;
+                    }
+                    q = make_float4(dq[0], dq[1], dq[2], dq[3]);
+                }
                 gy[v][c / 2] = f32x2{ok ? q.x : 0.f, ok ? q.y : 0.f};
                 gy[v][c / 2 + 1] = f32x2{ok ? q.z : 0.f, ok ? q.w : 0.f};
             }
@@ -1077,6 +1135,58 @@
     } else if (tid < NA && kd == 1 && bias_part) {
         const int c = tid - 9 * CO;
         bias_part[(size_t)share * CO + c] = (red[w0_][tid] + red[w0_ + 1][tid]) + (red[w0_ + 2][tid] + red[w0_ + 3][tid]);
+    }
+    if constexpr (PRELU) {
+        __shared__ double dred[4][CO];
+        if (kd == 1) {
+#pragma unroll
+            for (int c = 0; c < CO; ++c) {
+                const double vsum = wave_sum_d(dal[c]);
+                if (lane == 0) dred[wave - 4][c] = vsum;
+            }
+        }
+        __syncthreads();
+        if (kd == 1 && tid < CO) pr.dal_part[(size_t)share * CO + tid] = (dred[0][tid] + dred[1][tid]) + (dred[2][tid] + dred[3][tid]);
+    }
+}
+
+template <typename T, int CO>
+__global__ void __launch_bounds__(768)
+conv_cin1_wgrad_kernel(Mri3dConvGeom g, const T* __restrict__ x, const T* __restrict__ dy, float* __restrict__ part,
+                       float* __restrict__ bias_part, int tilesD, int tilesH, int tilesW, int ntiles, int nshares) {
+    conv_cin1_wgrad_body<T, CO, false>(g, x, dy, part, bias_part, tilesD, tilesH, tilesW, ntiles, nshares, Cin1Prelu<T>{});
+}
+
+template <typename T, int CO>
+__global__ void __launch_bounds__(768)
+conv_cin1_prelu_wgrad_kernel(Mri3dConvGeom g, const T* __restrict__ x, const T* __restrict__ da, float* __restrict__ part,
+                             float* __restrict__ bias_part, int tilesD, int tilesH, int tilesW, int ntiles, int nshares,
+                             Cin1Prelu<T> pr) {
+    conv_cin1_wgrad_body<T, CO, true>(g, x, da, part, bias_part, tilesD, tilesH, tilesW, ntiles, nshares, pr);
+}
+
+template <int CO>
+__global__ void __launch_bounds__(256)
+cin1_dalpha_reduce_kernel(const double* __restrict__ dal_part, float* __restrict__ dalpha, int nshares, int alpha_n) {
+    constexpr int QL = 256 / CO;
+    __shared__ double r[QL][CO];
+    __shared__ double tot[CO];
+    const int c = threadIdx.x % CO, q = threadIdx.x / CO;
+    double a = 0.0;
+    for (int sh = q; sh < nshares; sh += QL) a += dal_part[(size_t)sh * CO + c];
+    r[q][c] = a;
+    __syncthreads();
+    if (q == 0) {
+        a = 0.0;
+        for (int i = 0; i < QL; ++i) a += r[i][c];
+        tot[c] = a;
+        if (alpha_n > 1) dalpha[c] = (float)a;
+    }
+    __syncthreads();
+    if (threadIdx.x == 0 && alpha_n == 1) {
+        a = 0.0;
+        for (int i = 0; i < CO; ++i) a += tot[i];
+        dalpha[0] = (float)a;
     }
 }
 
@@ -1783,4 +1893,71 @@
     return check_launch(what);
 }
 
-}
+struct Cin1PreluPlan {
+    C1Tiles t;
+    int grid = 0, shares = 0;
+    size_t part_floats = 0, dal_off = 0, ws_bytes = 0;
+};
+
+static bool cin1_prelu_plan(const Mri3dConvGeom& g, int alpha_n, int pass, Cin1PreluPlan& p) {
+    if (g.dtype != MRI3D_F32 || !cin1_ok(g) || g.co != 8 || (alpha_n != 1 && alpha_n != g.co)) return false;
+    p.t = cin1_tiles(g);
+    if (pass == MRI3D_PASS_FWD) {
+        const GenericPlan q = generic_fwd_plan(g, 16, 16);
+        if (q.kernel != GenKernel::cin1) return false;
+        p.grid = std::min((int)p.t.ntiles, 256 * 8), p.ws_bytes = q.ws_bytes;
+        return true;
+    }
+    if (pass != MRI3D_PASS_WGRAD) return false;
+    const GenericPlan q = generic_wgrad_plan(g, 16, 16);
+    if (q.kernel != GenKernel::cin1) return false;
+    p.grid = p.shares = q.slots, p.part_floats = q.part_floats;
+    p.dal_off = align_up(q.ws_bytes, 8);
+    p.ws_bytes = p.dal_off + (size_t)p.shares * g.co * sizeof(double);
+    return true;
+}
+
+bool conv_cin1_prelu_plan_info(const Mri3dConvGeom& g, int alpha_n, int pass, Mri3dCin1PreluPlanInfo& out) {
+    Cin1PreluPlan p;
+    if (!cin1_prelu_plan(g, alpha_n, pass, p)) return false;
+    out.tiles_d = p.t.tilesD, out.tiles_h = p.t.tilesH, out.tiles_w = p.t.tilesW, out.tiles = (int32_t)p.t.ntiles;
+    out.grid = p.grid, out.shares = p.shares, out.ws_bytes = (int64_t)p.ws_bytes;
+    return true;
+}
+
+int conv_cin1_prelu_fwd(const Mri3dConvGeom& g, const void* x, const float* w, const float* bias, const float* alpha, int alpha_n,
+                        void* y, void* a, void* ws, size_t ws_bytes, hipStream_t s) {
+    Cin1PreluPlan p;
+    MRI3D_REQUIRE(cin1_prelu_plan(g, alpha_n, MRI3D_PASS_FWD, p), MRI3D_ENOTSUP, "conv3d_cin1_prelu_fwd: ci=%d co=%d alpha_n=%d not served",
+                  g.ci, g.co, alpha_n);
+    MRI3D_REQUIRE(aligned_vec4(g.dtype, y, a), MRI3D_EINVAL, "conv3d_cin1_prelu_fwd: y and a must be aligned to 4 elements");
+    MRI3D_REQUIRE(ws != nullptr && ws_bytes >= p.ws_bytes, MRI3D_EWORKSPACE, "conv3d_cin1_prelu_fwd: workspace %zu < %zu", ws_bytes, p.ws_bytes);
+    float* wp = static_cast<float*>(ws);
+    hipLaunchKernelGGL(repack_w_kernel, dim3(1), dim3(256), 0, s, w, wp, g.co, 1, 27, g.co, 0);
+    const Cin1Prelu<float> pr{(float*)a, nullptr, nullptr, alpha, alpha_n};
+    hipLaunchKernelGGL((conv_cin1_prelu_fwd_kernel<float, 8>), dim3(p.grid), dim3(256), 0, s, g, (const float*)x, wp, bias, (float*)y,
+                       p.t.tilesD, p.t.tilesH, p.t.tilesW, (int)p.t.ntiles, pr);
+    return check_launch("conv3d_cin1_prelu_fwd");
+}
+
+int conv_cin1_prelu_wgrad(const Mri3dConvGeom& g, const void* x, const void* y, const void* da, const float* alpha, int alpha_n,
+                          float* dw, float* dbias, float* dalpha, void* ws, size_t ws_bytes, hipStream_t s) {
+    Cin1PreluPlan p;
+    MRI3D_REQUIRE(cin1_prelu_plan(g, alpha_n, MRI3D_PASS_WGRAD, p), MRI3D_ENOTSUP,
+                  "conv3d_cin1_prelu_wgrad: ci=%d co=%d alpha_n=%d not served", g.ci, g.co, alpha_n);
+    MRI3D_REQUIRE(aligned_vec4(g.dtype, y, da), MRI3D_EINVAL, "conv3d_cin1_prelu_wgrad: y and da must be aligned to 4 elements");
+    MRI3D_REQUIRE(ws != nullptr && ws_bytes >= p.ws_bytes && (reinterpret_cast<uintptr_t>(ws) & 7) == 0, MRI3D_EWORKSPACE,
+                  "conv3d_cin1_prelu_wgrad: workspace %zu < %zu, or not 8-byte aligned", ws_bytes, p.ws_bytes);
+    float* part = static_cast<float*>(ws);
+    float* bias_part = dbias ? part + p.part_floats : nullptr;
+    double* dal_part = reinterpret_cast<double*>(static_cast<char*>(ws) + p.dal_off);
+    const Cin1Prelu<float> pr{nullptr, (const float*)y, dal_part, alpha, alpha_n};
+    hipLaunchKernelGGL((conv_cin1_prelu_wgrad_kernel<float, 8>), dim3(p.grid), dim3(768), 0, s, g, (const float*)x, (const float*)da, part,
+                       bias_part, p.t.tilesD, p.t.tilesH, p.t.tilesW, (int)p.t.ntiles, p.shares, pr);
+    hipLaunchKernelGGL(wgrad_reduce_kernel, dim3(cdiv(g.co * 27 + g.co, 8)), dim3(256), 0, s, part, bias_part, dw, dbias, p.shares, 27, 1,
+                       g.co, 1, g.co);
+    if (dalpha) hipLaunchKernelGGL(cin1_dalpha_reduce_kernel<8>, dim3(1), dim3(256), 0, s, dal_part, dalpha, p.shares, alpha_n);
+    return check_launch("conv3d_cin1_prelu_wgrad");
+}
+
+}
diff --git a/mri_epilepsy_diagnosis_amd/csrc/resample.hip b/mri_epilepsy_diagnosis_amd/csrc/resample.hip
--- a/mri_epilepsy_diagnosis_amd/csrc/resample.hip
+++ b/mri_epilepsy_diagnosis_amd/csrc/resample.hip
@@ -638,10 +638,17 @@
 constexpr int UHH = UTH + 2, UHW = UTW + 2, UHV = UHH * UHW;
 constexpr int UMD = 16;
 
-template <typename T, int VEC, int NPV>
-__global__ void __launch_bounds__(256)
-upsample2x_fwd_march_kernel(Mri3dUpGeom g, const T* __restrict__ x, T* __restrict__ y, int segsD, int segl, int tilesH,
-                            int tilesW, int cpasses, int nitems) {
+struct UpNormAct {
+    const float *mean, *invstd, *gamma, *beta, *alpha;
+    int alpha_n, act;
+    float slope;
+};
+
+template <typename T, int VEC, int NPV, bool NA>
+__device__ __forceinline__ void
+upsample2x_fwd_march_body(const Mri3dUpGeom& g, const T* __restrict__ x, T* __restrict__ y, int segsD, int segl, int tilesH,
+                          int tilesW, int cpasses, int nitems, const UpNormAct& na) {
+    static_assert(256 % NPV == 0, "a lane stages the same piece of every voxel it stages");
     constexpr int PCH = VEC * NPV;
     constexpr int NST = (UHV * NPV + 255) / 256;
     __shared__ __attribute__((aligned(16))) float cbuf[2][UHV * NPV * VEC];
@@ -671,6 +678,21 @@
             const int ch = min(max(h0 - 1 + fh, 0), g.hi - 1), cw = min(max(w0 - 1 + fw, 0), g.wi - 1);
             soff[j] = (ch * g.wi + cw) * g.x_ld + (c0 + pc * VEC < g.c ? pc * VEC : 0);
         }
+        float sc[NA ? VEC : 1], sh[NA ? VEC : 1], al[NA ? VEC : 1];
+        if constexpr (NA) {
+            const int pcs = tid % NPV, cb = c0 + (c0 + pcs * VEC < g.c ? pcs * VEC : 0);
+#pragma unroll
+            for (int e = 0; e < VEC; ++e) {
+                const int c = cb + e;
+                const float gm = na.gamma ? na.gamma[c] : 1.f;
+                const float bt = na.beta ? na.beta[c] : 0.f;
+                const float mu = na.mean ? na.mean[c] : 0.f;
+                const float is = na.invstd ? na.invstd[c] : 1.f;
+                sc[e] = gm * is;
+                sh[e] = bt - mu * sc[e];
+                al[e] = (na.act == MRI3D_ACT_PRELU) ? na.alpha[na.alpha_n == 1 ? 0 : c] : na.slope;
+            }
+        }
         V<VEC> sv[NST];
         auto fetch = [&](int c) {
             const T* pl = xn + (int64_t)min(max(c, 0), g.di - 1) * xplane;
@@ -682,6 +704,10 @@
             for (int j = 0; j < NST; ++j) {
                 const int idx = j * 256 + tid;
                 if (j < NST - 1 || idx < UHV * NPV) {
+                    if constexpr (NA) {
+#pragma unroll
+                        for (int e = 0; e < VEC; ++e) sv[j].v[e] = apply_act(fmaf(sv[j].v[e], sc[e], sh[e]), na.act, al[e]);
+                    }
 #pragma unroll
                     for (int e = 0; e < VEC; e += 4)
                         *reinterpret_cast<float4*>(&cbuf[buf][idx * VEC + e]) = make_float4(sv[j].v[e], sv[j].v[e + 1], sv[j].v[e + 2], sv[j].v[e + 3]);
@@ -749,6 +775,20 @@
             __syncthreads();
         }
     }
+}
+
+template <typename T, int VEC, int NPV>
+__global__ void __launch_bounds__(256)
+upsample2x_fwd_march_kernel(Mri3dUpGeom g, const T* __restrict__ x, T* __restrict__ y, int segsD, int segl, int tilesH,
+                            int tilesW, int cpasses, int nitems) {
+    upsample2x_fwd_march_body<T, VEC, NPV, false>(g, x, y, segsD, segl, tilesH, tilesW, cpasses, nitems, UpNormAct{});
+}
+
+template <typename T, int VEC, int NPV>
+__global__ void __launch_bounds__(256)
+norm_act_upsample2x_fwd_march_kernel(Mri3dUpGeom g, const T* __restrict__ x, T* __restrict__ y, int segsD, int segl, int tilesH,
+                                     int tilesW, int cpasses, int nitems, UpNormAct na) {
+    upsample2x_fwd_march_body<T, VEC, NPV, true>(g, x, y, segsD, segl, tilesH, tilesW, cpasses, nitems, na);
 }
 
 enum class ResampleKernel { maxpool_fwd, maxpool2_fwd, maxpool_bwd, up_fwd, up2x_fwd_march, up_bwd, up_nearest_int_bwd, up2x_bwd_tile, up2x_bwd_march };
@@ -866,6 +906,17 @@
     p.tables = true;
     snprintf(p.name, sizeof(p.name), "tables+upsample_bwd<%s,%d>", type_name(g.dtype), p.vec);
     return p;
+}
+
+static bool na_up_plan(const Mri3dNormGeom& g, const Mri3dUpGeom& ug, ResamplePlan& p) {
+    if (g.dtype != MRI3D_F32 || ug.dtype != MRI3D_F32 || g.instance != 0 || g.group_c != 0) return false;
+    if (g.act < MRI3D_ACT_NONE || g.act > MRI3D_ACT_PRELU || (g.act == MRI3D_ACT_PRELU && g.alpha_n != 1 && g.alpha_n != g.c)) return false;
+    if (ug.n <= 0 || ug.c <= 0 || ug.di <= 0 || ug.hi <= 0 || ug.wi <= 0 || ug.x_ld < ug.c || ug.y_ld < ug.c) return false;
+    if (g.n != ug.n || g.c != ug.c || g.x_ld != ug.x_ld || g.vox != (int64_t)ug.di * ug.hi * ug.wi) return false;
+    p = up_fwd_plan(ug, 16);
+    if (p.kern != ResampleKernel::up2x_fwd_march) return false;
+    snprintf(p.name, sizeof(p.name), "norm_act_upsample2x_fwd_march<f32,%d,%d>", p.vec, p.npv);
+    return true;
 }
 
 template <auto kern, typename... Args>
@@ -1073,3 +1124,38 @@
     plan_info(pass == MRI3D_PASS_FWD ? up_fwd_plan(*g, align) : up_bwd_plan(*g, align), out);
     return MRI3D_OK;
 }
+
+extern "C" int32_t mri3d_norm_act_upsample_supported(const Mri3dNormGeom* g, const Mri3dUpGeom* ug) {
+    ResamplePlan p;
+    return (g != nullptr && ug != nullptr && na_up_plan(*g, *ug, p)) ? 1 : 0;
+}
+
+extern "C" int32_t mri3d_norm_act_upsample_plan_query(const Mri3dNormGeom* g, const Mri3dUpGeom* ug, Mri3dResamplePlanInfo* out) {
+    MRI3D_REQUIRE(g != nullptr && ug != nullptr, MRI3D_EINVAL, "norm_act_upsample_plan_query: null geometry");
+    MRI3D_REQUIRE(out != nullptr, MRI3D_EINVAL, "norm_act_upsample_plan_query: null result");
+    ResamplePlan p;
+    MRI3D_REQUIRE(na_up_plan(*g, *ug, p), MRI3D_ENOTSUP, "norm_act_upsample_plan_query: c=%d x_ld=%d instance=%d %dx%dx%d -> %dx%dx%d not served",
+                  g->c, g->x_ld, g->instance, ug->di, ug->hi, ug->wi, ug->dout, ug->ho, ug->wo);
+    plan_info(p, out);
+    return MRI3D_OK;
+}
+
+extern "C" int mri3d_norm_act_upsample_fwd(const Mri3dNormGeom* g, const Mri3dUpGeom* ug, const void* x, const float* mean,
+                                           const float* invstd, const float* gamma, const float* beta, const float* alpha, void* y,
+                                           mri3d_stream_t stream) {
+    MRI3D_REQUIRE(g != nullptr && ug != nullptr, MRI3D_EINVAL, "norm_act_upsample_fwd: null geometry");
+    ResamplePlan p;
+    MRI3D_REQUIRE(na_up_plan(*g, *ug, p), MRI3D_ENOTSUP, "norm_act_upsample_fwd: c=%d x_ld=%d instance=%d %dx%dx%d -> %dx%dx%d not served",
+                  g->c, g->x_ld, g->instance, ug->di, ug->hi, ug->wi, ug->dout, ug->ho, ug->wo);
+    MRI3D_REQUIRE(x && y, MRI3D_EINVAL, "norm_act_upsample_fwd: null pointer");
+    MRI3D_REQUIRE((mean == nullptr) == (invstd == nullptr), MRI3D_EINVAL, "norm_act_upsample_fwd: mean/invstd must both be set");
+    MRI3D_REQUIRE(g->act != MRI3D_ACT_PRELU || alpha, MRI3D_EINVAL, "norm_act_upsample_fwd: PReLU needs alpha");
+    MRI3D_REQUIRE(aligned_vec4(g->dtype, x, y), MRI3D_EINVAL, "norm_act_upsample_fwd: x and y must be aligned to 4 elements");
+    hipStream_t s = static_cast<hipStream_t>(stream);
+    const UpNormAct na{mean, invstd, gamma, beta, alpha, g->alpha_n, g->act, g->slope};
+    with_int<1, 2, 4, 8>(p.npv, [&](auto N) {
+        launch<norm_act_upsample2x_fwd_march_kernel<float, 4, N.value>>(p, s, *ug, (const float*)x, (float*)y, p.segs, p.segl, p.tilesH,
+                                                                         p.tilesW, p.passes, p.items, na);
+    });
+    return check_launch(p.name);
+}
diff --git a/mri_epilepsy_diagnosis_amd/nn.py b/mri_epilepsy_diagnosis_amd/nn.py
--- a/mri_epilepsy_diagnosis_amd/nn.py
+++ b/mri_epilepsy_diagnosis_amd/nn.py
@@ -165,7 +165,31 @@
                        (x,))
 
 
-def conv_norm_act(conv, norm, act, x, out=None, head=None, pool=None):
+def fused_norm_act_upsample(norm, act, x, upsample):
+    if (not isinstance(upsample, tnn.Upsample) or upsample.mode not in ("trilinear", "linear") or upsample.align_corners
+            or upsample.size is not None or upsample.scale_factor not in (2, 2.0, (2, 2, 2), (2.0, 2.0, 2.0)) or not x.is_cuda):
+        return None
+    if x.dtype != torch.float32 or ops.autocast_dtype() is not None:
+        return None
+    return _fused_tail(norm, act, ops.norm_act_upsample_supported, (x,), ops.norm_act_upsample, (x,))
+
+
+def fused_conv_prelu(conv, act, x):
+    if not (isinstance(conv, Conv3d) and isinstance(act, tnn.PReLU) and torch.is_tensor(x)):
+        return None
+    if (conv.padding_mode != "zeros" or conv.groups != 1 or isinstance(conv.padding, str) or tuple(conv.stride) != (1, 1, 1)
+            or tuple(conv.dilation) != (1, 1, 1)):
+        return None
+    if not ops.conv3d_prelu_supported(x, conv.weight, act.weight, conv.stride, conv.padding, conv.dilation):
+        return None
+    return ops.conv3d_prelu(x, conv.weight, conv.bias, act.weight, conv.padding)
+
+
+def conv_norm_act(conv, norm, act, x, out=None, head=None, pool=None, upsample=None, fused_act=False):
+    if fused_act and norm is None and out is None and head is None and pool is None and upsample is None:
+        a = fused_conv_prelu(conv, act, x)
+        if a is not None:
+            return a
     wants = (isinstance(norm, tnn.modules.batchnorm._BatchNorm) and (norm.training or norm.running_mean is None)
              and ops.sync_batchnorm_reducer() is None and isinstance(conv, Conv3d) and conv.padding_mode == "zeros"
              and conv.groups == 1 and not isinstance(conv.padding, str))
@@ -187,6 +211,9 @@
     if pool is not None:
         both = fused_norm_act_pool(norm, act, y, pool) if out is None else None
         return both if both is not None else pool.forward_with_skip(fused_norm_act(norm, act, y, out))
+    if upsample is not None:
+        up = fused_norm_act_upsample(norm, act, y, upsample) if out is None else None
+        return up if up is not None else upsample(fused_norm_act(norm, act, y, out))
     return fused_norm_act(norm, act, y, out)
 
 
diff --git a/mri_epilepsy_diagnosis_amd/ops.py b/mri_epilepsy_diagnosis_amd/ops.py
--- a/mri_epilepsy_diagnosis_amd/ops.py
+++ b/mri_epilepsy_diagnosis_amd/ops.py
@@ -345,6 +345,13 @@
 def upsample_plan(g, pass_, align=16):
     info = _lib.ResamplePlanInfo()
     check(_lib.lib().mri3d_upsample3d_plan_query(ctypes.byref(g), pass_, align, ctypes.byref(info)), "upsample3d_plan_query")
+    return _resample_plan_dict(info)
+
+
+def norm_act_upsample_plan(g, ug):
+    info = _lib.ResamplePlanInfo()
+    check(_lib.lib().mri3d_norm_act_upsample_plan_query(ctypes.byref(g), ctypes.byref(ug), ctypes.byref(info)),
+          "norm_act_upsample_plan_query")
     return _resample_plan_dict(info)
 
 
@@ -679,6 +686,75 @@
 
 def conv3d(x, weight, bias=None, stride=1, padding=0, dilation=1, bn_stats=False):
     return _apply_with_bn_stats(_Conv3dFn, bn_stats, _autocast_in(x), weight, bias, _triple(stride), _triple(padding), _triple(dilation))
+
+
+CIN1_PRELU_PLAN_FIELDS = ("tiles_d", "tiles_h", "tiles_w", "tiles", "grid", "shares", "ws_bytes")
+
+
+def conv_cin1_prelu_plan(g, alpha_n, pass_):
+    info = _lib.Cin1PreluPlanInfo()
+    check(_lib.lib().mri3d_conv3d_cin1_prelu_plan_query(ctypes.byref(g), alpha_n, pass_, ctypes.byref(info)),
+          "conv3d_cin1_prelu_plan_query")
+    return {f: int(getattr(info, f)) for f in CIN1_PRELU_PLAN_FIELDS}
+
+
+def conv3d_prelu_supported(x, weight, alpha, stride=1, padding=0, dilation=1):
+    if not (x.is_cuda and x.dim() == 5 and x.dtype == torch.float32 and weight.dim() == 5 and weight.dtype == torch.float32):
+        return False
+    if (x.requires_grad and torch.is_grad_enabled()) or _autocast_dtype is not None or alpha is None or alpha.dtype != torch.float32:
+        return False
+    if x.shape[1] != weight.shape[1] or any(k > i + 2 * p for k, i, p in zip(weight.shape[2:], x.shape[2:], _triple(padding))):
+        return False
+    x_ld = _pitch_of(x)
+    g = _conv_geom(x.shape, weight.shape, _triple(stride), _triple(padding), _triple(dilation), x_ld=x_ld if x_ld is not None else x.shape[1])
+    return bool(_lib.lib().mri3d_conv3d_cin1_prelu_supported(ctypes.byref(g), alpha.numel()))
+
+
+class _Conv3dPreluFn(torch.autograd.Function):
+
+    @staticmethod
+    def forward(ctx, x, weight, bias, alpha, padding):
+        _require_device(x)
+        _require_param(weight, bias, alpha)
+        L = _lib.lib()
+        x, x_ld = _nd(x)
+        w = weight.contiguous()
+        g = _conv_geom(x.shape, w.shape, _ONE, padding, _ONE, x_ld=x_ld)
+        plan = conv_cin1_prelu_plan(g, alpha.numel(), PASS_FWD)
+        y = _new((g.n, g.co, g.dout, g.ho, g.wo), x)
+        a = _new(y.shape, x)
+        ws = _workspace(plan["ws_bytes"], x.device)
+        with _timed(lambda: _conv_tag("fwd", g) + " +prelu", lambda: _conv_work(g, "fwd")):
+            check(L.mri3d_conv3d_cin1_prelu_fwd(ctypes.byref(g), _ptr(x), _ptr(w), _ptr(bias), _ptr(alpha), alpha.numel(), _ptr(y), _ptr(a),
+                                                _ptr(ws), ws.numel(), _stream()), "conv3d_cin1_prelu_fwd")
+        ctx.save_for_backward(x, y, w, alpha)
+        ctx.geom, ctx.params = g, (weight, bias, alpha)
+        return a
+
+    @staticmethod
+    def backward(ctx, da):
+        L = _lib.lib()
+        x, y, w, alpha = ctx.saved_tensors
+        g = ctx.geom
+        if not any(p is not None and ctx.needs_input_grad[1 + i] for i, p in enumerate(ctx.params)):
+            return None, None, None, None, None
+        if da.dtype != y.dtype:
+            raise RuntimeError("conv3d_prelu backward: gradient dtype %s does not match activation dtype %s" % (da.dtype, y.dtype))
+        da, da_ld = _nd(da)
+        if da_ld != g.y_ld or da.data_ptr() % 16:
+            da = da.contiguous(memory_format=CL3D)
+        sinks, grads = _grad_slots(ctx, ctx.params, 1, ctx.params, all_written=True)
+        plan = conv_cin1_prelu_plan(g, alpha.numel(), PASS_WGRAD)
+        ws = _workspace(plan["ws_bytes"], x.device)
+        with _timed(lambda: _conv_tag("wgrad", g) + " +prelu", lambda: _conv_work(g, "wgrad")):
+            check(L.mri3d_conv3d_cin1_prelu_wgrad(ctypes.byref(g), _ptr(x), _ptr(y), _ptr(da), _ptr(alpha), alpha.numel(), _ptr(grads[0]),
+                                                  _ptr(grads[1]), _ptr(grads[2]), _ptr(ws), ws.numel(), _stream()),
+                  "conv3d_cin1_prelu_wgrad")
+        return (None, *_grad_slots_done(ctx, grads, sinks, 1, ctx.params), None)
+
+
+def conv3d_prelu(x, weight, bias, alpha, padding=1):
+    return _Conv3dPreluFn.apply(x, weight, bias, alpha, _triple(padding))
 
 
 
@@ -1059,29 +1135,34 @@
 
     @staticmethod
     def backward(ctx, dy):
-        L = _lib.lib()
-        x, mean, invstd, gamma, beta, alpha = ctx.saved_tensors
-        g0 = ctx.geom
-        dy, dy_ld = _nd(dy)
-        x = _backward_x("norm_act", x, g0, dy)
-        dx = _new(x.shape, x)
-        g = _repitched(g0, g0.c, dy_ld)
-        prelu = g.act == ACT_PRELU
-        sinks, grads = _grad_slots(ctx, (gamma, beta, alpha if prelu else None))
-        dgamma_k, dbeta_k, dalpha = grads
-        sync = ctx.sync
-        if sync is not None:
-            dbeta_k = dbeta_k if dbeta_k is not None else torch.empty(g.c, dtype=torch.float32, device=x.device)
-            dgamma_k = dgamma_k if dgamma_k is not None else torch.empty(g.c, dtype=torch.float32, device=x.device)
-        ws = _workspace(L.mri3d_norm_workspace_bytes(ctypes.byref(g)), x.device)
-        with _timed(lambda: "norm_act_bwd c%d vox%d n%d" % (g.c, g.vox, g.n), lambda: {"flops": 0.0, "bytes": 5 * _esz(x) * x.numel()}):
-            check(L.mri3d_norm_act_bwd(ctypes.byref(g), 1 if ctx.training_stats else 0, _ptr(x), _ptr(dy), _ptr(mean),
-                                       _ptr(invstd), _ptr(gamma), _ptr(beta), _ptr(alpha) if prelu else None, _ptr(dx),
-                                       _ptr(dgamma_k), _ptr(dbeta_k), _ptr(dalpha), _ptr(ws), ws.numel(), _stream()),
-                  "norm_act_bwd")
-        if sync is not None:
-            _sync_correct_dx(sync, g, x, mean, invstd, gamma, dbeta_k, dgamma_k, ctx.sync_count, dx)
-        return (dx, *_grad_slots_done(ctx, grads, sinks), None, None, None, None, None, None, None, None, None, None)
+        dx, grads = _norm_act_backward(ctx, "norm_act", dy)
+        return (dx, *grads, None, None, None, None, None, None, None, None, None, None)
+
+
+def _norm_act_backward(ctx, who, dy):
+    L = _lib.lib()
+    x, mean, invstd, gamma, beta, alpha = ctx.saved_tensors
+    g0 = ctx.geom
+    dy, dy_ld = _nd(dy)
+    x = _backward_x(who, x, g0, dy)
+    dx = _new(x.shape, x)
+    g = _repitched(g0, g0.c, dy_ld)
+    prelu = g.act == ACT_PRELU
+    sinks, grads = _grad_slots(ctx, (gamma, beta, alpha if prelu else None))
+    dgamma_k, dbeta_k, dalpha = grads
+    sync = ctx.sync
+    if sync is not None:
+        dbeta_k = dbeta_k if dbeta_k is not None else torch.empty(g.c, dtype=torch.float32, device=x.device)
+        dgamma_k = dgamma_k if dgamma_k is not None else torch.empty(g.c, dtype=torch.float32, device=x.device)
+    ws = _workspace(L.mri3d_norm_workspace_bytes(ctypes.byref(g)), x.device)
+    with _timed(lambda: "norm_act_bwd c%d vox%d n%d" % (g.c, g.vox, g.n), lambda: {"flops": 0.0, "bytes": 5 * _esz(x) * x.numel()}):
+        check(L.mri3d_norm_act_bwd(ctypes.byref(g), 1 if ctx.training_stats else 0, _ptr(x), _ptr(dy), _ptr(mean),
+                                   _ptr(invstd), _ptr(gamma), _ptr(beta), _ptr(alpha) if prelu else None, _ptr(dx),
+                                   _ptr(dgamma_k), _ptr(dbeta_k), _ptr(dalpha), _ptr(ws), ws.numel(), _stream()),
+              "norm_act_bwd")
+    if sync is not None:
+        _sync_correct_dx(sync, g, x, mean, invstd, gamma, dbeta_k, dgamma_k, ctx.sync_count, dx)
+    return dx, _grad_slots_done(ctx, grads, sinks)
 
 
 def norm_act(x, gamma=None, beta=None, alpha=None, running_mean=None, running_var=None, stats_mode="batch",
@@ -1276,6 +1357,63 @@
     return _NormActPoolFn.apply(x, gamma, beta, alpha, running_mean, running_var, stats_mode, momentum, eps, act, slope, fused)
 
 
+def _up2x_geom(x, x_ld, y_ld):
+    n, c, d, h, w = x.shape
+    return UpGeom(n, d, h, w, 2 * d, 2 * h, 2 * w, c, x_ld, y_ld, UP_TRILINEAR, 0, 0.5, 0.5, 0.5, _dt(x))
+
+
+def norm_act_upsample_supported(x, stats_mode="batch", act=None, alpha=None):
+    x_ld = _fusable_x_ld(x, stats_mode, act)
+    if x_ld is None or x.dtype != torch.float32:
+        return False
+    c = x.shape[1]
+    g = _norm_geom(x, x_ld, c, _ACT_CODES[act], alpha, 0.0, 0.0)
+    ug = _up2x_geom(x, x_ld, c)
+    return bool(_lib.lib().mri3d_norm_act_upsample_supported(ctypes.byref(g), ctypes.byref(ug)))
+
+
+class _NormActUpsampleFn(torch.autograd.Function):
+
+    @staticmethod
+    def forward(ctx, x, gamma, beta, alpha, running_mean, running_var, stats_mode, momentum, eps, act, slope, fused_stats=None):
+        _require_device(x)
+        _require_param(gamma, beta, alpha)
+        ctx.params = (gamma, beta, alpha)
+        L = _lib.lib()
+        x, x_ld = _nd(x)
+        n, c, d, h, w = x.shape
+        act_code = _ACT_CODES[act]
+        g = _norm_geom(x, x_ld, c, act_code, alpha, slope, eps)
+        ug = _up2x_geom(x, x_ld, c)
+        if not L.mri3d_norm_act_upsample_supported(ctypes.byref(g), ctypes.byref(ug)):
+            raise RuntimeError("norm_act_upsample: c=%d pitch %d extents %s is not served (ask norm_act_upsample_supported first)"
+                               % (c, x_ld, (d, h, w)))
+        mean, invstd = _norm_statistics("norm_act_upsample", g, x, 1, stats_mode, running_mean, running_var, momentum, eps,
+                                        fused_stats)
+        y = _new((n, c, 2 * d, 2 * h, 2 * w), x)
+        with _timed(lambda: "norm_act_upsample_fwd c%d" % c, lambda: {"flops": 0.0, "bytes": _esz(x) * (x.numel() + y.numel())}):
+            check(L.mri3d_norm_act_upsample_fwd(ctypes.byref(g), ctypes.byref(ug), _ptr(x), _ptr(mean), _ptr(invstd), _ptr(gamma),
+                                                _ptr(beta), _ptr(alpha) if act_code == ACT_PRELU else None, _ptr(y), _stream()),
+                  "norm_act_upsample_fwd")
+        ctx.save_for_backward(x, mean, invstd, gamma, beta, alpha)
+        ctx.geom, ctx.up_geom = g, ug
+        ctx.training_stats = stats_mode == "batch"
+        ctx.sync = None
+        return y
+
+    @staticmethod
+    def backward(ctx, dy):
+        da = _upsample_backward(ctx.up_geom, tuple(ctx.saved_tensors[0].shape), dy)
+        dx, grads = _norm_act_backward(ctx, "norm_act_upsample", da)
+        return (dx, *grads, None, None, None, None, None, None, None, None)
+
+
+def norm_act_upsample(x, gamma=None, beta=None, alpha=None, running_mean=None, running_var=None, stats_mode="batch",
+                      momentum=0.1, eps=1e-5, act=None, slope=0.01):
+    fused = _fused_stats_of(x, stats_mode, momentum)
+    return _NormActUpsampleFn.apply(x, gamma, beta, alpha, running_mean, running_var, stats_mode, momentum, eps, act, slope, fused)
+
+
 def activation(x, act, alpha=None, slope=0.01):
     return norm_act(x, None, None, alpha, None, None, "none", 0.1, 0.0, act, slope)
 
@@ -1400,6 +1538,16 @@
     return _MaxPool3dFn.apply(x, k, s, _triple(padding))
 
 
+
+
+def _upsample_backward(g0, xshape, dy):
+    L = _lib.lib()
+    dy, dy_ld = _nd(dy)
+    dx = _new(xshape, dy)
+    g = _repitched(g0, g0.c, dy_ld, _dt(dy))
+    _launch(L.mri3d_upsample3d_bwd, lambda: "upsample_bwd c%d" % g.c, lambda: {"flops": 0.0, "bytes": _esz(dy) * (dx.numel() + dy.numel())},
+            L.mri3d_upsample3d_workspace_bytes(ctypes.byref(g)), dy.device, g, dy, dx)
+    return dx
 
 
 class _Upsample3dFn(torch.autograd.Function):
@@ -1429,13 +1577,7 @@
 
     @staticmethod
     def backward(ctx, dy):
-        L = _lib.lib()
-        dy, dy_ld = _nd(dy)
-        dx = _new(ctx.xshape, dy)
-        g = _repitched(ctx.geom, ctx.geom.c, dy_ld, _dt(dy))
-        _launch(L.mri3d_upsample3d_bwd, lambda: "upsample_bwd c%d" % g.c, lambda: {"flops": 0.0, "bytes": _esz(dy) * (dx.numel() + dy.numel())},
-                L.mri3d_upsample3d_workspace_bytes(ctypes.byref(g)), dy.device, g, dy, dx)
-        return dx, None, None, None, None, None
+        return _upsample_backward(ctx.geom, ctx.xshape, dy), None, None, None, None, None
 
 
 def upsample3d(x, size=None, scale_factor=None, mode="nearest", align_corners=None, out=None):
diff --git a/mri_epilepsy_diagnosis_amd/unet/unet.py b/mri_epilepsy_diagnosis_amd/unet/unet.py
--- a/mri_epilepsy_diagnosis_amd/unet/unet.py
+++ b/mri_epilepsy_diagnosis_amd/unet/unet.py
@@ -32,8 +32,8 @@
         self.dropout_layer = None
         self.block = tnn.Sequential(*[m for m in (conv, norm, act) if m is not None])
 
-    def forward(self, x, out=None, head=None, pool=None):
-        return mnn.conv_norm_act(self.conv_layer, self.norm_layer, self.activation_layer, x, out, head, pool)
+    def forward(self, x, out=None, head=None, pool=None, upsample=None, fused_act=False):
+        return mnn.conv_norm_act(self.conv_layer, self.norm_layer, self.activation_layer, x, out, head, pool, upsample, fused_act)
 
 
 class EncodingBlock(tnn.Module):
@@ -55,12 +55,12 @@
                 raise NotImplementedError("only max pooling is used by the reference")
             self.downsample = mnn.MaxPool3d(kernel_size=2)
 
-    def forward(self, x, skip_out=None, head=None, fused_pool=True):
+    def forward(self, x, skip_out=None, head=None, fused_pool=True, upsample=None, fused_first=False):
         if self.downsample is None:
-            return self.conv2(self.conv1(x), skip_out, head)
+            return self.conv2(self.conv1(x, fused_act=fused_first), skip_out, head, upsample=upsample)
         if fused_pool and skip_out is None and isinstance(self.downsample, mnn.MaxPool3d):
-            return self.conv2(self.conv1(x), pool=self.downsample)
-        x = self.conv2(self.conv1(x), skip_out)
+            return self.conv2(self.conv1(x, fused_act=fused_first), pool=self.downsample)
+        x = self.conv2(self.conv1(x, fused_act=fused_first), skip_out)
         return self.downsample.forward_with_skip(x)
 
     @property
@@ -85,10 +85,10 @@
             if self.dilation is not None:
                 self.dilation *= 2
 
-    def forward(self, x, cat_bufs=None, fused_pool=True):
+    def forward(self, x, cat_bufs=None, fused_pool=True, fused_first=False):
         skips = []
         for i, blk in enumerate(self.encoding_blocks):
-            x, skip = blk(x, None if cat_bufs is None else (cat_bufs[i], 0), fused_pool=fused_pool)
+            x, skip = blk(x, None if cat_bufs is None else (cat_bufs[i], 0), fused_pool=fused_pool, fused_first=fused_first and i == 0)
             skips.append(skip)
         return skips, x
 
@@ -114,7 +114,11 @@
                                         normalization=normalization, padding=padding, activation=activation,
                                         dilation=dilation)
 
-    def forward(self, skip, x, cat_buf=None, head=None):
+    def forward(self, skip, x, cat_buf=None, head=None, upsampled=False, next_upsample=None):
+        if upsampled:
+            if skip.shape[2:] != x.shape[2:]:
+                raise NotImplementedError("padding=False (centre-cropped skips) is not used by the reference")
+            return self.conv2(self.conv1((skip, x)), head=head, upsample=next_upsample)
         if cat_buf is not None and isinstance(self.upsample, mnn.Upsample):
             up = ops.upsample3d(x, self.upsample.size, self.upsample.scale_factor, self.upsample.mode,
                                 self.upsample.align_corners, out=(cat_buf, skip.shape[1]))
@@ -139,10 +143,11 @@
             if self.dilation is not None:
                 self.dilation //= 2
 
-    def forward(self, skips, x, cat_bufs=None, head=None):
+    def forward(self, skips, x, cat_bufs=None, head=None, upsampled=False):
         last = min(len(skips), len(self.decoding_blocks)) - 1
         for j, (skip, blk) in enumerate(zip(reversed(skips), self.decoding_blocks)):
-            x = blk(skip, x, None if cat_bufs is None else cat_bufs[len(skips) - 1 - j], head if j == last else None)
+            nxt = self.decoding_blocks[j + 1].upsample if upsampled and j < last else None
+            x = blk(skip, x, None if cat_bufs is None else cat_bufs[len(skips) - 1 - j], head if j == last else None, upsampled, nxt)
         return x
 
 
@@ -173,6 +178,8 @@
         self.shared_concat_buffers = False
         self.fused_head = True
         self.fused_pool = True
+        self.fused_upsample = True
+        self.fused_first_layer = False
         self.classifier = ConvolutionalBlock(dimensions, 2 * out_channels_first_layer, out_classes, kernel_size=1,
                                              activation=None)
 
@@ -193,9 +200,11 @@
         mc = mc if (mc is not None and mc.training and mc.p > 0) else None
         head = clf.conv_layer if (self.fused_head and mc is None and x.is_cuda and clf.norm_layer is None
                                   and clf.activation_layer is None and clf.dropout_layer is None) else None
-        skips, enc = self.encoder(x, cat_bufs, self.fused_pool)
+        skips, enc = self.encoder(x, cat_bufs, self.fused_pool, self.fused_first_layer)
         if not skips:
-            x = self.bottom_block(enc, head=head)
+            x = self.bottom_block(enc, head=head, fused_first=self.fused_first_layer)
+        elif self.fused_upsample and cat_bufs is None:
+            x = self.decoder(skips, self.bottom_block(enc, upsample=self.decoder.decoding_blocks[0].upsample), None, head, True)
         else:
             x = self.decoder(skips, self.bottom_block(enc), cat_bufs, head)
         if head is not None:
```

Result: no change. 69.09 volumes/s, median of 6 (+0.3%).
